# elizabethfong/SparkSmithWaterman

Hardware: AMD Instinct MI355X
Metric: GCUPS (higher is better)
Workload: dtype int32

## Files before the change

### include/swmi.h

```cpp
#ifndef SWMI_H
#define SWMI_H

#include <stddef.h>
#include <stdint.h>

#ifdef __cplusplus
extern "C" {
#endif

#define SWMI_ABI_VERSION 3

typedef enum swmi_status {
    SWMI_OK               =  0,
    SWMI_ERR_INVALID      = -1,
    SWMI_ERR_NO_DEVICE    = -2,
    SWMI_ERR_HIP          = -3,
    SWMI_ERR_NOMEM        = -4,
    SWMI_ERR_UNSUPPORTED  = -5,
    SWMI_ERR_RANGE        = -6
} swmi_status;

#define SWMI_ALIGN_LOCAL  0
#define SWMI_ALIGN_FIT    1
#define SWMI_ALIGN_GLOBAL 2

#define SWMI_TIE_SERIAL 0
#define SWMI_TIE_STRICT 1

typedef struct swmi_params {
    int32_t match;
    int32_t mismatch;
    int32_t gap;
    int32_t tie_mode;
    char    types[4];
} swmi_params;

typedef struct swmi_ctx    swmi_ctx;
typedef struct swmi_batch  swmi_batch;

int         swmi_abi_version(void);
const char *swmi_last_error(void);
int         swmi_device_count(int *count);
int         swmi_create(int device, swmi_ctx **out);
void        swmi_destroy(swmi_ctx *ctx);
void        swmi_default_params(swmi_params *p);

int         swmi_set_option(swmi_ctx *ctx, const char *name, int64_t value);

int         swmi_set_score_matrix(swmi_ctx *ctx, const uint8_t *alphabet, uint32_t n, const int32_t *scores);

int  swmi_batch_upload(swmi_ctx *ctx,
                       const uint8_t *ref_bytes, const uint64_t *ref_off, uint32_t n_refs,
                       const uint8_t *read_bytes, const uint64_t *read_off, uint32_t n_reads,
                       swmi_batch **out);
int  swmi_batch_run(swmi_ctx *ctx, swmi_batch *b, const swmi_params *p);
void swmi_batch_free(swmi_ctx *ctx, swmi_batch *b);
int  swmi_batch_run_async(swmi_ctx *ctx, swmi_batch *b, const swmi_params *p);
int  swmi_batch_wait(swmi_ctx *ctx);

typedef struct swmi_timing {
    float    fill_ms, traceback_ms, d2h_ms, total_ms;
    uint32_t fill_launches, rerun_pairs;
    uint64_t cells;
    uint64_t dir_bytes;
    uint32_t strip_fallbacks;
    uint32_t col_chunks;
    uint32_t resident_pairs;
    uint32_t tfused_pairs;
} swmi_timing;
int  swmi_batch_timing(const swmi_batch *b, swmi_timing *t);
int  swmi_batch_mode(const swmi_batch *b, int *mode);

#define SWMI_PAIR_DEGENERATE 0x1u
uint64_t swmi_batch_n_pairs(const swmi_batch *b);
int      swmi_pair_score(const swmi_batch *b, uint64_t pair, int32_t *score);
int      swmi_pair_n_alignments(const swmi_batch *b, uint64_t pair, uint64_t *n, uint32_t *flags);
int      swmi_pair_rows_swept(const swmi_batch *b, uint64_t pair, uint32_t *rows);
int      swmi_batch_pair_results(const swmi_batch *b, int32_t *scores, uint64_t *n_alignments, uint64_t n);
int      swmi_pair_alignment(swmi_batch *b, uint64_t pair, uint64_t k,
                             int32_t *begin, int32_t *end_i, int32_t *end_j,
                             const char **ref_aln, const char **read_aln, uint32_t *len);

int      swmi_batch_materialise_all(swmi_batch *b, uint64_t *n_alignments, uint64_t *n_chars);

int      swmi_ref_total(const swmi_batch *b, uint32_t ref, int32_t *total);
int      swmi_ref_totals(const swmi_batch *b, int32_t *totals, uint32_t n);
int      swmi_ref_n_match_sites(swmi_batch *b, uint32_t ref, uint64_t *n);
int      swmi_ref_match_site(swmi_batch *b, uint32_t ref, uint64_t k, int32_t *begin,
                             const char **ref_aln, const char **read_aln, uint32_t *len);

int      swmi_ref_sites_packed(swmi_batch *b, uint32_t ref_lo, uint32_t ref_hi,
                               int32_t *totals, uint64_t *degenerate, uint64_t *site_first,
                               int32_t *begins, uint32_t *lens, uint64_t *str_off, uint64_t sites_cap,
                               uint8_t *blob, uint64_t blob_cap, uint64_t *n_sites, uint64_t *blob_bytes);

int  swmi_align_batch(swmi_ctx *ctx, const swmi_params *p,
                      const uint8_t *ref_bytes, const uint64_t *ref_off, uint32_t n_refs,
                      const uint8_t *read_bytes, const uint64_t *read_off, uint32_t n_reads,
                      swmi_batch **out);

typedef struct swmi_stream swmi_stream;
typedef struct swmi_stream_stats {
    double   push_ms;
    double   parse_ms;
    double   upload_ms, run_ms;
    double   gpu_sweep_ms, gpu_traceback_ms;
    uint64_t bytes, cells;
    uint32_t chunks, pad;
} swmi_stream_stats;
int      swmi_stream_open(swmi_ctx *ctx, const swmi_params *p, const uint8_t *read_bytes, const uint64_t *read_off,
                          uint32_t n_reads, uint32_t slots, uint64_t chunk_bytes, swmi_stream **out);
int      swmi_stream_push(swmi_stream *s, const uint8_t *ref_bytes, const uint64_t *ref_off, uint32_t n_refs);
int      swmi_stream_push_file(swmi_stream *s, const char *path, const char *delimiter, uint32_t parse_threads);
int      swmi_stream_push_file_shard(swmi_stream *s, const char *path, const char *delimiter, uint32_t parse_threads,
                                     uint32_t shard, uint32_t n_shards);
int      swmi_stream_finish(swmi_stream *s);
uint64_t swmi_stream_n_refs(const swmi_stream *s);
uint32_t swmi_stream_n_chunks(const swmi_stream *s);
int      swmi_stream_chunk(swmi_stream *s, uint32_t k, swmi_batch **batch, uint64_t *first_ref);
int      swmi_stream_totals(const swmi_stream *s, int32_t *totals, uint64_t n);
int      swmi_stream_metadata(const swmi_stream *s, uint64_t ref, char *buf, size_t cap);
int      swmi_stream_ref_pos(const swmi_stream *s, uint64_t ref, uint64_t *pos);
int      swmi_stream_ref_sequence(const swmi_stream *s, uint64_t ref, uint8_t *buf, uint64_t cap, uint64_t *len);
int      swmi_stream_get_stats(const swmi_stream *s, swmi_stream_stats *st);
void     swmi_stream_close(swmi_stream *s);

#ifdef __cplusplus
}
#endif
#endif
```

### sparksmithwaterman_amd/_capi.py

```python
import ctypes as C
import os

_HERE = os.path.dirname(os.path.abspath(__file__))
LIB_PATH = os.environ.get("SWMI_LIB") or os.path.join(_HERE, "lib", "libswmi.so")

TIE_SERIAL = 0
TIE_STRICT = 1
ALIGN_LOCAL = 0
ALIGN_FIT = 1
ALIGN_GLOBAL = 2
BAND_MAX = 1 << 20
XDROP_MAX = (1 << 31) - 1
PAIR_DEGENERATE = 0x1


class SwmiError(RuntimeError):
    def __init__(self, code, msg):
        super().__init__("swmi error %d: %s" % (code, msg))
        self.code = code


class Params(C.Structure):
    _fields_ = [("match", C.c_int32), ("mismatch", C.c_int32), ("gap", C.c_int32),
                ("tie_mode", C.c_int32), ("types", C.c_char * 4)]


class Timing(C.Structure):
    _fields_ = [("fill_ms", C.c_float), ("traceback_ms", C.c_float), ("d2h_ms", C.c_float),
                ("total_ms", C.c_float), ("fill_launches", C.c_uint32), ("rerun_pairs", C.c_uint32),
                ("cells", C.c_uint64), ("dir_bytes", C.c_uint64),
                ("strip_fallbacks", C.c_uint32), ("col_chunks", C.c_uint32),
                ("resident_pairs", C.c_uint32), ("tfused_pairs", C.c_uint32)]


class StreamStats(C.Structure):
    _fields_ = [("push_ms", C.c_double), ("parse_ms", C.c_double), ("upload_ms", C.c_double), ("run_ms", C.c_double),
                ("gpu_sweep_ms", C.c_double), ("gpu_traceback_ms", C.c_double), ("bytes", C.c_uint64), ("cells", C.c_uint64),
                ("chunks", C.c_uint32), ("pad", C.c_uint32)]


_P = C.c_void_p
_u8p = C.POINTER(C.c_uint8)
_u64p = C.POINTER(C.c_uint64)
SYMBOLS = [
    ("swmi_abi_version", C.c_int, []),
    ("swmi_last_error", C.c_char_p, []),
    ("swmi_device_count", C.c_int, [C.POINTER(C.c_int)]),
    ("swmi_create", C.c_int, [C.c_int, C.POINTER(_P)]),
    ("swmi_destroy", None, [_P]),
    ("swmi_default_params", None, [C.POINTER(Params)]),
    ("swmi_set_option", C.c_int, [_P, C.c_char_p, C.c_int64]),
    ("swmi_set_score_matrix", C.c_int, [_P, C.c_char_p, C.c_uint32, C.POINTER(C.c_int32)]),
    ("swmi_batch_upload", C.c_int, [_P, C.c_char_p, _u64p, C.c_uint32, C.c_char_p, _u64p, C.c_uint32, C.POINTER(_P)]),
    ("swmi_batch_run", C.c_int, [_P, _P, C.POINTER(Params)]),
    ("swmi_batch_run_async", C.c_int, [_P, _P, C.POINTER(Params)]),
    ("swmi_batch_wait", C.c_int, [_P]),
    ("swmi_batch_free", None, [_P, _P]),
    ("swmi_batch_timing", C.c_int, [_P, C.POINTER(Timing)]),
    ("swmi_batch_mode", C.c_int, [_P, C.POINTER(C.c_int)]),
    ("swmi_batch_n_pairs", C.c_uint64, [_P]),
    ("swmi_pair_score", C.c_int, [_P, C.c_uint64, C.POINTER(C.c_int32)]),
    ("swmi_pair_n_alignments", C.c_int, [_P, C.c_uint64, _u64p, C.POINTER(C.c_uint32)]),
    ("swmi_pair_alignment", C.c_int, [_P, C.c_uint64, C.c_uint64, C.POINTER(C.c_int32), C.POINTER(C.c_int32),
                                      C.POINTER(C.c_int32), C.POINTER(C.c_char_p), C.POINTER(C.c_char_p),
                                      C.POINTER(C.c_uint32)]),
    ("swmi_pair_rows_swept", C.c_int, [_P, C.c_uint64, C.POINTER(C.c_uint32)]),
    ("swmi_batch_pair_results", C.c_int, [_P, C.POINTER(C.c_int32), _u64p, C.c_uint64]),
    ("swmi_batch_materialise_all", C.c_int, [_P, _u64p, _u64p]),
    ("swmi_ref_total", C.c_int, [_P, C.c_uint32, C.POINTER(C.c_int32)]),
    ("swmi_ref_totals", C.c_int, [_P, C.POINTER(C.c_int32), C.c_uint32]),
    ("swmi_ref_n_match_sites", C.c_int, [_P, C.c_uint32, _u64p]),
    ("swmi_ref_match_site", C.c_int, [_P, C.c_uint32, C.c_uint64, C.POINTER(C.c_int32), C.POINTER(C.c_char_p),
                                      C.POINTER(C.c_char_p), C.POINTER(C.c_uint32)]),
    ("swmi_ref_sites_packed", C.c_int, [_P, C.c_uint32, C.c_uint32, C.POINTER(C.c_int32), _u64p, _u64p, C.POINTER(C.c_int32),
                                        C.POINTER(C.c_uint32), _u64p, C.c_uint64, C.c_void_p, C.c_uint64, _u64p, _u64p]),
    ("swmi_stream_open", C.c_int, [_P, C.POINTER(Params), C.c_char_p, _u64p, C.c_uint32, C.c_uint32, C.c_uint64, C.POINTER(_P)]),
    ("swmi_stream_push", C.c_int, [_P, C.c_char_p, _u64p, C.c_uint32]),
    ("swmi_stream_push_file", C.c_int, [_P, C.c_char_p, C.c_char_p, C.c_uint32]),
    ("swmi_stream_push_file_shard", C.c_int, [_P, C.c_char_p, C.c_char_p, C.c_uint32, C.c_uint32, C.c_uint32]),
    ("swmi_stream_finish", C.c_int, [_P]),
    ("swmi_stream_n_refs", C.c_uint64, [_P]),
    ("swmi_stream_n_chunks", C.c_uint32, [_P]),
    ("swmi_stream_chunk", C.c_int, [_P, C.c_uint32, C.POINTER(_P), _u64p]),
    ("swmi_stream_totals", C.c_int, [_P, C.POINTER(C.c_int32), C.c_uint64]),
    ("swmi_stream_metadata", C.c_int, [_P, C.c_uint64, C.c_char_p, C.c_size_t]),
    ("swmi_stream_ref_pos", C.c_int, [_P, C.c_uint64, _u64p]),
    ("swmi_stream_ref_sequence", C.c_int, [_P, C.c_uint64, C.c_void_p, C.c_uint64, _u64p]),
    ("swmi_stream_get_stats", C.c_int, [_P, C.POINTER(StreamStats)]),
    ("swmi_stream_close", None, [_P]),
    ("swmi_align_batch", C.c_int, [_P, C.POINTER(Params), C.c_char_p, _u64p, C.c_uint32, C.c_char_p, _u64p,
                                   C.c_uint32, C.POINTER(_P)]),
]

_lib = None


def load():
    global _lib
    if _lib is None:
        if not os.path.exists(LIB_PATH):
            raise ImportError(
                "%s is missing: build it with `python -c 'import __graft_entry__ as g; g.build()'` "
                "(hipcc, gfx950).  There is no CPU fallback." % LIB_PATH)
        lib = C.CDLL(LIB_PATH)
        for name, res, args in SYMBOLS:
            f = getattr(lib, name)
            f.restype = res
            f.argtypes = args
        _lib = lib
    return _lib


def check(rc):
    if rc != 0:
        raise SwmiError(rc, load().swmi_last_error().decode("utf-8", "replace"))


def as_bytes(s):
    return bytes(s) if isinstance(s, (bytes, bytearray, memoryview)) else s.encode("latin-1")


def pack(seqs):
    bs = [as_bytes(s) for s in seqs]
    off = (C.c_uint64 * (len(bs) + 1))()
    t = 0
    for k, b in enumerate(bs):
        off[k] = t
        t += len(b)
    off[len(bs)] = t
    return b"".join(bs), off
```

### sparksmithwaterman_amd/csrc/swmi_ctx.cpp

```cpp
#include <cstdarg>
#include <cstdio>
#include <cstdlib>

#include "swmi_host.h"
#include "swmi_launch.h"

static thread_local std::string g_err;

int swmi_host::fail(int code, const char *fmt, ...) {
    char buf[512];
    va_list ap;
    va_start(ap, fmt);
    vsnprintf(buf, sizeof buf, fmt, ap);
    va_end(ap);
    g_err = buf;
    return code;
}

int swmi_io_fail(int code, const std::string &msg) { return fail(code, "%s", msg.c_str()); }

static const uint8_t *code_table();

extern "C" int swmi_abi_version(void) { return SWMI_ABI_VERSION; }

extern "C" const char *swmi_last_error(void) { return g_err.c_str(); }

extern "C" int swmi_device_count(int *count) {
    if (!count) return fail(SWMI_ERR_INVALID, "count is null");
    int n = 0;
    hipError_t e = hipGetDeviceCount(&n);
    if (e != hipSuccess) { *count = 0; return fail(SWMI_ERR_NO_DEVICE, "hipGetDeviceCount: %s", hipGetErrorString(e)); }
    *count = n;
    return SWMI_OK;
}

extern "C" void swmi_default_params(swmi_params *p) {
    if (!p) return;
    p->match = 5; p->mismatch = -3; p->gap = -4;
    p->tie_mode = SWMI_TIE_SERIAL;
    p->types[0] = 'a'; p->types[1] = 'i'; p->types[2] = 'd'; p->types[3] = '-';
}

static void ctx_release(swmi_ctx *c) {
    for (auto &ev : c->ev) if (ev) (void)hipEventDestroy(ev);
    if (c->stream) (void)hipStreamDestroy(c->stream);
    c->h_err.release();
    c->d_lut.release();
    c->d_hdr_ring.release();
    delete c;
}

extern "C" int swmi_create(int device, swmi_ctx **out) {
    if (!out) return fail(SWMI_ERR_INVALID, "out is null");
    *out = nullptr;
    int n = 0;
    hipError_t e = hipGetDeviceCount(&n);
    if (e != hipSuccess || n <= 0)
        return fail(SWMI_ERR_NO_DEVICE, "no HIP device available (%s); this library has no CPU fallback",
                    e != hipSuccess ? hipGetErrorString(e) : "device count 0");
    if (device < 0 || device >= n) return fail(SWMI_ERR_INVALID, "device %d out of range [0,%d)", device, n);
    hipDeviceProp_t prop;
    e = hipGetDeviceProperties(&prop, device);
    if (e != hipSuccess) return fail(SWMI_ERR_NO_DEVICE, "hipGetDeviceProperties: %s", hipGetErrorString(e));
    if (strncmp(prop.gcnArchName, "gfx950", 6) != 0)
        return fail(SWMI_ERR_NO_DEVICE, "device %d is %s; the kernels are built for gfx950 (MI355X) only",
                    device, prop.gcnArchName);
    e = hipSetDevice(device);
    if (e != hipSuccess) return fail(SWMI_ERR_NO_DEVICE, "hipSetDevice: %s", hipGetErrorString(e));
    swmi_ctx *c = new swmi_ctx;
    c->device = device;
    e = hipStreamCreateWithFlags(&c->stream, hipStreamNonBlocking);
    if (e != hipSuccess) { c->stream = nullptr; ctx_release(c); return fail(SWMI_ERR_HIP, "hipStreamCreate: %s", hipGetErrorString(e)); }
    for (auto &ev : c->ev) {
        e = hipEventCreate(&ev);
        if (e != hipSuccess) { ev = nullptr; ctx_release(c); return fail(SWMI_ERR_HIP, "hipEventCreate: %s", hipGetErrorString(e)); }
    }
    { int r = c->h_err.reserve(64); if (r) { ctx_release(c); return r; } }
    { static const char *ee = getenv("SWMI_EXT_EVENTS"); if (ee) c->ext_events = atoi(ee) != 0; }
    *(volatile uint32_t *)c->h_err.p = 0u;
    { int r = c->d_lut.reserve(256); if (r) { ctx_release(c); return r; } }
    e = hipMemcpy(c->d_lut.p, code_table(), 256, hipMemcpyHostToDevice);
    if (e != hipSuccess) { ctx_release(c); return fail(SWMI_ERR_HIP, "code table upload: %s", hipGetErrorString(e)); }
    *out = c;
    return SWMI_OK;
}

extern "C" void swmi_destroy(swmi_ctx *ctx) {
    if (!ctx) return;
    (void)hipSetDevice(ctx->device);
    if (ctx->worker.joinable()) {
        {
            std::unique_lock<std::mutex> lk(ctx->job_mu);
            ctx->job_cv.wait(lk, [&] { return ctx->job_state.load() != 1; });
            ctx->job_state.store(3);
        }
        ctx->job_cv.notify_all();
        ctx->worker.join();
    }
    ctx_release(ctx);
}

extern "C" int swmi_set_option(swmi_ctx *ctx, const char *name, int64_t value) {
    if (!ctx || !name) return fail(SWMI_ERR_INVALID, "null argument");
    std::lock_guard<std::mutex> g(ctx->mu);
    if (!strcmp(name, "cell_cap")) {
        if (value < 1 || value > (1 << 20)) return fail(SWMI_ERR_INVALID, "cell_cap out of range");
        ctx->cell_cap = (uint32_t)value;
        ctx->cell_cap_set = true;
    } else if (!strcmp(name, "max_workspace_bytes")) {
        if (value < (1 << 20)) return fail(SWMI_ERR_INVALID, "max_workspace_bytes too small");
        ctx->max_workspace_bytes = (uint64_t)value;
    } else if (!strcmp(name, "mode")) {
        if (value < -1 || value > 2) return fail(SWMI_ERR_INVALID, "mode must be -1 (automatic), 0, 1 or 2");
        ctx->mode = value < 0 ? 1u : (uint32_t)value;
    } else if (!strcmp(name, "auto_ties_x100")) {
        if (value < 100) return fail(SWMI_ERR_INVALID, "auto_ties_x100 out of range");
        ctx->auto_ties_x100 = (uint32_t)value;
    } else if (!strcmp(name, "spin_us")) {
        if (value < 0) return fail(SWMI_ERR_INVALID, "spin_us out of range");
        ctx->spin_us = value;
    } else if (!strcmp(name, "debug_strip_spins")) {
        ctx->dbg_strip_spins = (uint32_t)value;
    } else if (!strcmp(name, "debug_reverse_strips")) {
        ctx->dbg_reverse_strips = value != 0;
    } else if (!strcmp(name, "debug_async_delay_us")) {
        if (value < 0 || value > 10000000) return fail(SWMI_ERR_INVALID, "debug_async_delay_us out of range");
        ctx->dbg_async_delay_us = (uint32_t)value;
    } else if (!strcmp(name, "tfused")) {
        if (value < -1 || value > 1) return fail(SWMI_ERR_INVALID, "tfused must be -1 (automatic), 0 or 1");
        ctx->tfused = (int)value;
    } else if (!strcmp(name, "resident")) {
        if (value < -1 || value > 1) return fail(SWMI_ERR_INVALID, "resident must be -1 (automatic), 0 or 1");
        ctx->resident = (int)value;
    } else if (!strcmp(name, "scores_only")) {
        ctx->scores_only = value != 0;
    } else if (!strcmp(name, "stream_keep_records")) {
        ctx->stream_keep_records = value != 0;
    } else if (!strcmp(name, "device_strings")) {
        ctx->device_strings = value != 0;
    } else if (!strcmp(name, "tb_split")) {
        if (value < -1 || value > 1) return fail(SWMI_ERR_INVALID, "tb_split must be -1 (automatic), 0 or 1");
        ctx->tb_split = (int)value;
    } else if (!strcmp(name, "col_chunks")) {
        if (value < 0 || value > 4096) return fail(SWMI_ERR_INVALID, "col_chunks out of range");
        ctx->col_chunks = (uint32_t)value;
    } else if (!strcmp(name, "zero_copy")) {
        ctx->zero_copy = value != 0;
    } else if (!strcmp(name, "profiling")) {
        if (value < 0 || value > 2) return fail(SWMI_ERR_INVALID, "profiling must be 0, 1 (every stage) or 2 (the sweep only)");
        ctx->profiling = (int)value;
    } else if (!strcmp(name, "gap_open")) {
        if (value > 0) return fail(SWMI_ERR_INVALID, "gap_open must be <= 0 (a penalty), got %lld", (long long)value);
        if (value < INT32_MIN) return fail(SWMI_ERR_INVALID, "gap_open out of range");
        ctx->gap_open = (int32_t)value;
    } else if (!strcmp(name, "affine")) {
        if (value != -1 && value != 1) return fail(SWMI_ERR_INVALID, "affine must be -1 (when gap_open != 0) or 1 (always)");
        ctx->affine = (int)value;
    } else if (!strcmp(name, "align_mode")) {
        if (value != SWMI_ALIGN_LOCAL && value != SWMI_ALIGN_FIT && value != SWMI_ALIGN_GLOBAL)
            return fail(SWMI_ERR_INVALID, "align_mode must be 0 (local), 1 (fit) or 2 (global), got %lld", (long long)value);
        ctx->modes.align_mode = (int)value;
    } else if (!strcmp(name, "long_reads")) {
        if (value != 0 && value != 1) return fail(SWMI_ERR_INVALID, "long_reads must be 0 or 1, got %lld", (long long)value);
        ctx->modes.long_reads = (int)value;
    } else if (!strcmp(name, "band")) {
        if (value < 0 || value > (int64_t)SWMI_AFF_BAND_MAX)
            return fail(SWMI_ERR_INVALID, "band must be 0 (none) or a half-width of 1 .. %u columns, got %lld", SWMI_AFF_BAND_MAX, (long long)value);
        ctx->modes.band = (int)value;
    } else if (!strcmp(name, "extend")) {
        if (value != 0 && value != 1) return fail(SWMI_ERR_INVALID, "extend must be 0 or 1, got %lld", (long long)value);
        ctx->modes.extend = (int)value;
    } else if (!strcmp(name, "xdrop")) {
        if (value < 0 || value > 0x7FFFFFFFll)
            return fail(SWMI_ERR_INVALID, "xdrop must be 0 (off) or a threshold of 1 .. 2^31 - 1, got %lld", (long long)value);
        ctx->modes.xdrop = (int)value;
    } else if (!strcmp(name, "arena_words_per_pair")) {
        if (value < 1) return fail(SWMI_ERR_INVALID, "arena_words_per_pair out of range");
        ctx->arena_words_per_pair = (uint64_t)value;
    } else {
        return fail(SWMI_ERR_INVALID, "unknown option '%s'", name);
    }
    return SWMI_OK;
}

extern "C" int swmi_set_score_matrix(swmi_ctx *ctx, const uint8_t *alphabet, uint32_t n, const int32_t *scores) {
    if (!ctx) return fail(SWMI_ERR_INVALID, "null context");
    if (n == 0) {
        std::lock_guard<std::mutex> g(ctx->mat_mu);
        ctx->matrix.reset();
        return SWMI_OK;
    }
    if (n > SWMI_MAT_MAX_SYMBOLS) return fail(SWMI_ERR_INVALID, "a score matrix has at most %u symbols, got %u", SWMI_MAT_MAX_SYMBOLS, n);
    if (!alphabet || !scores) return fail(SWMI_ERR_INVALID, "alphabet or scores is null");
    const uint8_t *T = code_table();
    uint32_t cls[256];
    for (uint32_t c = 0; c < 256; c++) cls[c] = n;
    for (uint32_t i = 0; i < n; i++) {
        const uint8_t c = T[alphabet[i]];
        if (cls[c] != n)
            return fail(SWMI_ERR_INVALID, "score matrix symbols %u and %u are the same symbol (0x%02x, 0x%02x)", cls[c], i,
                        alphabet[cls[c]], alphabet[i]);
        cls[c] = i;
    }
    auto M = std::make_shared<ScoreMatrix>();
    M->n = n;
    M->max_entry = INT32_MIN;
    const uint32_t nn = n + 1;
    M->image.assign(swmi_aff_mat_words(nn), 0u);
    for (uint64_t x = 0; x < (uint64_t)n * n; x++) {
        if (std::llabs((int64_t)scores[x]) > (1 << 20))
            return fail(SWMI_ERR_INVALID, "score matrix entry [%u][%u] = %d: |entries| must be <= 2^20", (uint32_t)(x / n),
                        (uint32_t)(x % n), scores[x]);
        M->max_entry = std::max(M->max_entry, scores[x]);
        M->image[256 + (x / n) * nn + x % n] = (uint32_t)scores[x];
    }
    for (uint32_t c = 0; c < 256; c++) M->image[c] = cls[c] * 4u | ((cls[c] == n ? c : 0x1FFu) << 16);
    static std::atomic<uint64_t> gens{0};
    M->gen = ++gens;
    std::lock_guard<std::mutex> g(ctx->mat_mu);
    ctx->matrix = std::move(M);
    return SWMI_OK;
}

static const uint8_t *code_table() {
    static uint8_t T[256];
    static std::once_flag once;
    std::call_once(once, [] {
        uint8_t perm[256];
        for (int i = 0; i < 256; i++) perm[i] = (uint8_t)i;
        const uint8_t fast[8] = {'A', 'C', 'G', 'T', 'N', 'U', 'R', 'Y'};
        for (int k = 0; k < 8; k++) std::swap(perm[fast[k]], perm[4 * k]);
        for (int i = 0; i < 256; i++) {
            int u = i;
            if ((i >= 'a' && i <= 'z') || (i >= 0xE0 && i <= 0xFE && i != 0xF7)) u = i - 32;
            T[i] = perm[u];
        }
    });
    return T;
}

static uint64_t layout_sequences(const uint64_t *off, uint32_t n, uint64_t word0, std::vector<SeqDesc> &desc) {
    desc.resize(n);
    uint64_t at = word0;
    for (uint32_t s = 0; s < n; s++) {
        const uint64_t len = off[s + 1] - off[s];
        at = (at + 3) & ~(uint64_t)3;
        SeqDesc d{};
        d.len = (uint32_t)len;
        d.boff = (uint32_t)at;
        d.acgt = 0;
        desc[s] = d;
        at += (len + 3) / 4 + SWMI_SEQ_PAD_WORDS;
    }
    return at;
}

int swmi_host::check_offsets(const uint64_t *off, uint32_t n, const char *what) {
    if (!off) return fail(SWMI_ERR_INVALID, "%s offsets are null", what);
    if (off[0] != 0) return fail(SWMI_ERR_INVALID, "%s offsets must start at 0", what);
    for (uint32_t k = 0; k < n; k++) {
        if (off[k + 1] < off[k]) return fail(SWMI_ERR_INVALID, "%s offsets decrease at %u", what, k);
        if (off[k + 1] - off[k] >= (1ull << 30))
            return fail(SWMI_ERR_UNSUPPORTED, "%s %u is longer than 2^30-1 bases", what, k);
    }
    return SWMI_OK;
}

extern "C" void swmi_batch_free(swmi_ctx *ctx, swmi_batch *b) {
    if (!b) return;
    if (ctx) (void)hipSetDevice(ctx->device);
    b->d_raw.release(); b->d_raw_off.release();
    b->d_seqw.release(); b->d_refs.release(); b->d_reads.release(); b->d_pairs.release();
    b->d_dir.release(); b->d_seam.release(); b->d_result.release(); b->d_cells.release();
    b->d_cells_off.release(); b->d_cells_cap.release(); b->d_dbg.release(); b->d_dbg2.release();
    b->d_strip_items.release(); b->d_progress.release(); b->d_col_items.release(); b->d_win_off.release(); b->d_queue.release(); b->d_res_items.release();
    b->d_tf_items.release(); b->d_mat.release();
    b->h_result.release();
    delete b;
}

int swmi_host::upload_device(swmi_ctx *ctx, swmi_batch *b, hipStream_t st, const uint8_t *ref_src, const uint8_t *read_src) {
    const uint32_t n_refs = b->n_refs, n_reads = b->n_reads;
    const uint64_t ref_total = b->ref_off[n_refs], read_total = b->read_off[n_reads];
// ... 58 lines not shown
```

### sparksmithwaterman_amd/csrc/swmi_host.h

```cpp
#pragma once
#include <hip/hip_runtime.h>

#include <algorithm>
#include <atomic>
#include <condition_variable>
#include <cstdint>
#include <cstring>
#include <memory>
#include <mutex>
#include <string>
#include <thread>
#include <type_traits>
#include <unordered_map>
#include <vector>

#include "../../include/swmi.h"
#include "swmi_device.h"
#include "swmi_io_internal.h"

namespace swmi_host __attribute__((visibility("hidden"))) {
int fail(int code, const char *fmt, ...);
int check_offsets(const uint64_t *off, uint32_t n, const char *what);
int upload_device(swmi_ctx *ctx, swmi_batch *b, hipStream_t st, const uint8_t *ref_src, const uint8_t *read_src);
int settle_raw(swmi_batch *b);
int dump_traceback_diagnostics(swmi_batch *b, const TraceArgs &ta, size_t np, size_t n_tf);
int dump_fill_diagnostics(swmi_batch *b, const FillArgs &fa, size_t np);
void watchdog_wait(hipStream_t st, const swmi_batch *b, const char *limit_s);
}
using namespace swmi_host;

#define HIP_TRY(expr)                                                                         \
    do {                                                                                      \
        hipError_t e_ = (expr);                                                               \
        if (e_ != hipSuccess)                                                                 \
            return fail(e_ == hipErrorOutOfMemory ? SWMI_ERR_NOMEM : SWMI_ERR_HIP,            \
                        "%s failed: %s", #expr, hipGetErrorString(e_));                       \
    } while (0)

struct DevBuf {
    void *p = nullptr;
    size_t cap = 0;
    int reserve(size_t bytes) {
        if (bytes <= cap) return SWMI_OK;
        size_t want = bytes >= (256u << 20) ? bytes + bytes / 2 : bytes;
        if (p) { want = std::max(want, cap + cap / 4); (void)hipFree(p); p = nullptr; cap = 0; }
        hipError_t e = hipMalloc(&p, want);
        if (e != hipSuccess && want > bytes) { want = bytes; e = hipMalloc(&p, want); }
        if (e != hipSuccess) { p = nullptr; return fail(SWMI_ERR_NOMEM, "hipMalloc(%zu) failed: %s", bytes, hipGetErrorString(e)); }
        cap = want;
        return SWMI_OK;
    }
    void release() { if (p) (void)hipFree(p); p = nullptr; cap = 0; }
    template <class T> T *as() const { return (T *)p; }
    DevBuf() = default;
    DevBuf(const DevBuf &) = delete;
    DevBuf &operator=(const DevBuf &) = delete;
    ~DevBuf() { release(); }
};

struct PinnedBuf {
    void *p = nullptr;
    void *dp = nullptr;
    size_t cap = 0;
    int reserve(size_t bytes) {
        if (bytes <= cap) return SWMI_OK;
        if (p) { bytes = std::max(bytes, cap + cap / 4); (void)hipHostFree(p); p = nullptr; dp = nullptr; cap = 0; }
        hipError_t e = hipHostMalloc(&p, bytes, hipHostMallocMapped);
        if (e != hipSuccess) { p = nullptr; return fail(SWMI_ERR_NOMEM, "hipHostMalloc(%zu) failed: %s", bytes, hipGetErrorString(e)); }
        e = hipHostGetDevicePointer(&dp, p, 0);
        if (e != hipSuccess) { (void)hipHostFree(p); p = nullptr; return fail(SWMI_ERR_HIP, "hipHostGetDevicePointer: %s", hipGetErrorString(e)); }
        cap = bytes;
        return SWMI_OK;
    }
    void release() { if (p) (void)hipHostFree(p); p = nullptr; dp = nullptr; cap = 0; }
    PinnedBuf() = default;
    PinnedBuf(const PinnedBuf &) = delete;
    PinnedBuf &operator=(const PinnedBuf &) = delete;
    ~PinnedBuf() { release(); }
};

struct ScoreMatrix {
    uint64_t gen = 0;
    uint32_t n = 0;
    int32_t max_entry = 0;
    std::vector<uint32_t> image;
};

struct __attribute__((visibility("hidden"))) RunModes {
    int align_mode = SWMI_ALIGN_LOCAL;
    int long_reads = 0;
    int band = 0;
    int extend = 0;
    int xdrop = 0;
    uint32_t kernel_mode() const { return extend && align_mode == SWMI_ALIGN_GLOBAL ? 3u : (uint32_t)align_mode; }
    bool operator==(const RunModes &o) const { return memcmp(this, &o, sizeof(RunModes)) == 0; }
};
static_assert(std::has_unique_object_representations_v<RunModes>, "RunModes is compared bytewise: no padding, no floating point");
struct __attribute__((visibility("hidden"))) RunOptions {
    RunModes modes;
    std::shared_ptr<const ScoreMatrix> mat;
};

struct swmi_ctx {
    int device = 0;
    hipStream_t stream = nullptr;
    std::mutex mu;
    uint32_t cell_cap = 64;
    uint64_t max_workspace_bytes = 32ull << 30;
    int profiling = 0;
    uint32_t mode = 1;
    int zero_copy = 1;
    uint64_t arena_words_per_pair = 160;
    uint64_t arena_copy_wpp = 160;
    uint64_t recs_per_pair_x16 = 32;
    hipEvent_t ev[6] = {nullptr, nullptr, nullptr, nullptr, nullptr, nullptr};
    PinnedBuf h_err;
    DevBuf d_hdr_ring;
    uint32_t hdr_next = 0;
    DevBuf d_lut;
    int64_t spin_us = 2000;
    uint32_t dbg_strip_spins = 0;
    uint32_t dbg_reverse_strips = 0;
    uint32_t dbg_async_delay_us = 0;
    uint32_t auto_ties_x100 = 300;
    uint32_t col_chunks = 0;
    int tb_split = -1;
    bool ext_events = false;
    int tfused = -1;
    int resident = -1;
    int scores_only = 0;
    int stream_keep_records = 1;
    int device_strings = 1;
    bool cell_cap_set = false;
    int32_t gap_open = 0;
    int affine = -1;
    RunModes modes;
    std::mutex mat_mu;
    std::shared_ptr<const ScoreMatrix> matrix;
    std::thread worker;
    std::mutex job_mu;
    std::condition_variable job_cv;
    std::atomic<int> job_state{0};
    swmi_batch *job_batch = nullptr;
    swmi_params job_params{};
    RunOptions job_opt;
    uint32_t job_delay_us = 0;
    int job_rc = 0;
    std::string job_err;
};

static inline RunOptions run_options(swmi_ctx *ctx) {
    std::lock_guard<std::mutex> g(ctx->mat_mu);
    return RunOptions{ctx->modes, ctx->matrix};
}

struct HostAln {
    uint32_t rank;
    int32_t begin, end_i, end_j;
    uint32_t n_ops;
    const uint32_t *rec = nullptr;
    int64_t str_id = -1;
};

struct PairRes {
    int32_t score = 0;
    uint32_t flags = 0;
    uint64_t n_cells = 0;
    uint32_t strips = 0;
    uint64_t first = 0;
    uint64_t count = 0;
};

struct SiteRef { uint64_t pair; uint64_t k; int32_t begin; };

struct Work {
    uint32_t pair;
    uint64_t cells;
    uint64_t dir_words;
    uint64_t seam_words;
};

struct __attribute__((visibility("hidden"))) PlanKey {
    bool valid = false;
    size_t lo = 0, hi = 0;
    const void *work = nullptr;
    swmi_params params{};
    uint32_t eff_mode = 0;
    uint32_t col_chunks = 0;
    bool reverse_strips = false;
    int resident = -1, tfused = -1;
    bool exact = false;
    bool scores_only = false;
    uint64_t mat_gen = 0;
    RunModes modes;
    const void *d_pairs = nullptr;
    size_t pairs_bytes = 0;
    bool operator==(const PlanKey &o) const {
        return valid == o.valid && lo == o.lo && hi == o.hi && work == o.work && memcmp(&params, &o.params, sizeof(swmi_params)) == 0 &&
               eff_mode == o.eff_mode && col_chunks == o.col_chunks && reverse_strips == o.reverse_strips && resident == o.resident &&
               tfused == o.tfused && exact == o.exact && scores_only == o.scores_only && mat_gen == o.mat_gen &&
               modes == o.modes && d_pairs == o.d_pairs && pairs_bytes == o.pairs_bytes;
    }
};

struct __attribute__((visibility("hidden"))) ChunkPlan {
    uint64_t dir_words = 0, seam_words = 0;
    uint64_t seam_priv_words = 0;
    uint32_t max_path = 0, max_read = 0;
    size_t n_strip_items = 0;
    size_t n_strip_chunks = 0;
    size_t n_col_items = 0;
    uint64_t n_windows = 0;
    size_t n_res = 0;
    uint32_t res_lds_words = 0, res_ops_words = 0;
    size_t n_tf = 0;
    uint32_t tf_max_m = 0, tf_max_n = 0, tf_max_path = 0;
    uint32_t aff_r_min = 0xFFFFFFFFu, aff_r_max = 0;
    size_t aff_n_long = 0;
};

struct swmi_batch {
    uint32_t n_refs = 0, n_reads = 0;
    std::vector<uint8_t> ref_bytes, read_bytes;
    const uint8_t *src_map = nullptr;
    std::vector<swmi_io_recpos> src_recs;
    std::unordered_map<uint32_t, std::vector<uint8_t>> src_cache;
    std::vector<uint64_t> ref_off, read_off;
    std::vector<SeqDesc> ref_desc, read_desc;
    DevBuf d_raw, d_raw_off;
    DevBuf d_seqw, d_refs, d_reads, d_pairs, d_dir, d_seam, d_result, d_cells, d_cells_off, d_cells_cap, d_dbg, d_dbg2;
    DevBuf d_strip_items, d_progress;
    DevBuf d_col_items;
    DevBuf d_win_off, d_queue;
    DevBuf d_tf_items;
    DevBuf d_res_items;
    bool views_built = false;
    bool tb_split_used = false;
    bool acgt_known = false;
    PinnedBuf h_result;
    swmi_params params{};
    bool has_run = false;
    int auto_choice = -1;
    swmi_params auto_params{};
    std::vector<Work> work;
    int work_mode = -1;
    int work_band = 0;
    bool work_tfused = false;
    uint32_t eff_mode = 1;
    int32_t gap_open = 0;
    RunOptions opt;
    DevBuf d_mat;
    uint64_t d_mat_gen = 0;
    uint64_t work_cells = 0;
    std::vector<uint8_t> pairs_on_device;
    const void *pairs_dev_ptr = nullptr;
    PlanKey plan_key;
    ChunkPlan plan;
    std::vector<PairRes> pairs;
    struct RawChunk { size_t at, words; size_t tab_at, n_rec; size_t lo; std::vector<uint32_t> wpos; };
    std::vector<uint32_t> raw;
    std::vector<AlnRec> rtab;
    const uint32_t *raw_ext = nullptr;
    const AlnRec *rtab_ext = nullptr;
    uint64_t raw_ext_records = 0, raw_ext_cap = 0;
    std::vector<RawChunk> raw_chunks;
    bool indexed = false;
    bool rec_strings = false;
    bool scores_only = false;
    bool records_dropped = false;
    std::vector<HostAln> alns;
    std::vector<char> str_buf;
    std::vector<uint64_t> str_at;
    std::vector<int8_t> ref_view_ready;
    std::vector<std::vector<SiteRef>> ref_sites;
    std::vector<uint64_t> ref_degenerate;
    swmi_timing timing{};
};

struct RunState {
    swmi_ctx *ctx;
    swmi_batch *b;
    FillArgs fa{};
    TraceArgs ta{};
    float fill_ms = 0, tb_ms = 0, d2h_ms = 0;
    uint32_t launches = 0;
    double enqueue_us = 0, wait_us = 0, copyout_us = 0, prep_us = 0, prep_upload_us = 0;
    bool one_wave_sweep = false;
    bool tb_split = false;
    bool defer_copy = false;
    bool keep = true;
};

static inline size_t result_out_off() { return 64; }
static inline size_t result_tab_off(size_t np) { return (64 + np * sizeof(PairOut) + 255) & ~(size_t)255; }
static inline size_t result_arena_off(size_t np, uint64_t tab_cap) { return (result_tab_off(np) + tab_cap * sizeof(AlnRec) + 255) & ~(size_t)255; }
static inline uint64_t rec_words(uint32_t n_ops, bool strings) {
    return strings ? 2 * ((uint64_t)n_ops / 4 + 1) : ((uint64_t)n_ops + 15) / 16;
}
```

### sparksmithwaterman_amd/csrc/swmi_launch.h

```cpp
#pragma once
#include <hip/hip_runtime.h>
#include <stdint.h>
#include "swmi_device.h"

template <class K>
static inline void swmi_allow_big_lds(K kernel) {
    (void)hipFuncSetAttribute(reinterpret_cast<const void *>(kernel), hipFuncAttributeMaxDynamicSharedMemorySize, 160 * 1024);
}

extern "C" hipError_t swmi_launch_fill(const FillArgs *a, hipStream_t st, hipEvent_t ev_start, hipEvent_t ev_stop);
extern "C" hipError_t swmi_launch_traceback(const TraceArgs *a, hipStream_t st, hipEvent_t ev_start, hipEvent_t ev_stop);
extern "C" hipError_t swmi_launch_traceback_split(const TraceArgs *a, uint32_t n_windows, hipStream_t st);
extern "C" hipError_t swmi_launch_resident(const TraceArgs *a, const ResidentArgs *x, hipStream_t st);
extern "C" hipError_t swmi_launch_tfused(const TraceArgs *a, const TFusedArgs *x, hipStream_t st);
extern "C" hipError_t swmi_launch_affine_sweep(const FillArgs *a, int32_t gap_open, uint32_t align_mode, const uint32_t *mat, uint32_t nn,
                                               uint32_t r_min, uint32_t r_max, uint32_t long_reads, uint32_t band, uint32_t xdrop, hipStream_t st);
extern "C" hipError_t swmi_launch_affine_traceback(const TraceArgs *a, uint32_t align_mode, uint32_t long_reads, uint32_t band, uint32_t tile_words,
                                                   uint32_t ops_words, hipStream_t st);
extern "C" hipError_t swmi_launch_encode(const uint8_t *raw, const uint64_t *raw_off, SeqDesc *desc, uint32_t *seqw,
                                         const uint8_t *lut, uint32_t n_seq, hipStream_t st);
```

### sparksmithwaterman_amd/csrc/swmi_plan.h

```cpp
#pragma once
#include <chrono>
#include <cstdlib>

#include "swmi_host.h"

using Clock = std::chrono::steady_clock;
static inline double us_between(Clock::time_point a, Clock::time_point c) { return std::chrono::duration<double, std::micro>(c - a).count(); }

static uint64_t path_bound(uint64_t n_, uint64_t m_, const swmi_params &p, int32_t smax, int align_mode = 0) {
    uint64_t path = n_ + m_;
    if (align_mode != 0) return path;
    if (smax > 0 && p.gap < 0 && p.mismatch <= smax) {
        const uint64_t g = (uint64_t)(-(int64_t)p.gap), mt = (uint64_t)smax;
        path = std::min(path, std::min(m_ + std::min(n_, mt * m_ / g), n_ + std::min(m_, mt * n_ / g)));
    }
    return path;
}

static uint64_t traceback_lds_bytes(uint32_t mode, uint64_t max_path, uint64_t max_read) {
    const uint64_t lds_words = (max_path + 3) / 4 + 1, lds_read_words = (max_read + 3) / 4 + 1;
    const uint64_t win = (uint64_t)SWMI_RMAX * 64;
    const uint64_t tile_words = mode == 0 ? 4ull * SWMI_TB_BLOCKS * win : (mode == 1 ? 32 + 8ull * SWMI_CK_BLOCKS * win : 4ull * SWMI_CK_BLOCKS * win);
    return 4ull * (tile_words + 4ull * (lds_words + lds_read_words + SWMI_TB_REFWIN_WORDS));
}

static void longest_sequences(const swmi_batch *b, uint64_t &max_m, uint64_t &max_n) {
    max_m = max_n = 0;
    for (const auto &d : b->read_desc) max_m = std::max<uint64_t>(max_m, d.len);
    for (const auto &d : b->ref_desc) max_n = std::max<uint64_t>(max_n, d.len);
}


namespace {

struct PlanItems {
    std::vector<PairDesc> pd;
    std::vector<StripItem> strip_items;
    std::vector<ColItem> col_items;
    std::vector<uint32_t> win_off;
    std::vector<uint32_t> res_items, tf_items;
};

static const uint32_t CK_STEP_W = 16u * SWMI_CK_BLOCKS;
static inline uint32_t ck_windows(uint32_t n) {
    const uint64_t wblocks = ((uint64_t)n + 63u + 15u) / 16u;
    return (uint32_t)((wblocks + SWMI_CK_BLOCKS - 1u) / SWMI_CK_BLOCKS);
}
static inline uint64_t path_span(uint32_t m, const swmi_params &P) {
    return (uint64_t)m + (uint64_t)(P.match > 0 ? P.match : 0) * m / (uint64_t)(P.gap < 0 ? -(int64_t)P.gap : 1) + 1;
}

struct ColChunk { uint32_t g_lo, g_hi, col0; };
static ColChunk col_chunk(uint32_t g_lo, uint32_t wpc, uint32_t n_ck, uint32_t n, uint64_t span) {
    ColChunk c;
    c.g_lo = g_lo;
    c.g_hi = std::min(g_lo + wpc, n_ck);
    if (c.g_hi < n_ck && (uint64_t)c.g_hi * CK_STEP_W > n) c.g_hi = n_ck;
    const int64_t c0 = (int64_t)g_lo * CK_STEP_W - 64 - (int64_t)span - 1;
    c.col0 = g_lo == 0 || c0 <= 0 ? 0u : (uint32_t)(c0 / CK_STEP_W * CK_STEP_W);
    return c;
}

struct Planner {
    const swmi_ctx *ctx;
    const swmi_batch *b;
    const swmi_params &P;
    size_t np;
    ChunkPlan &plan;
    PlanItems &it;
    bool cols_possible = false;
    uint64_t chunk_budget = 1;
    bool res_possible = false, res_maybe = false;
    bool tf_possible = false;

    Planner(const swmi_ctx *ctx_, const swmi_batch *b_, size_t np_, bool exact, ChunkPlan &plan_, PlanItems &it_)
        : ctx(ctx_), b(b_), P(b_->params), np(np_), plan(plan_), it(it_) {
        const bool mode1 = b->eff_mode == 1, whole = mode1 && !exact && !ctx->scores_only;
        cols_possible = mode1 && P.match > 0 && P.gap < 0 && P.mismatch <= 0 && P.match <= 7 && P.mismatch >= -8 &&
                        (np <= 512 || ctx->col_chunks > 1) && ctx->col_chunks != 1;
        chunk_budget = ctx->col_chunks > 1 ? ctx->col_chunks : std::max<uint64_t>(1, 1024 / std::max<size_t>(np, 1));
        res_possible = whole && ctx->resident != 0 && (ctx->resident == 1 || np >= 256) &&
                       P.match <= 7 && P.match >= -8 && P.mismatch >= -8 && P.mismatch <= 0 && P.gap <= 0;
        tf_possible = whole && ctx->tfused == 1 &&
                      P.match > 0 && P.match <= 7 && P.mismatch >= -8 && P.mismatch <= P.match && P.gap < 0 && P.gap >= -64;
    }
    bool fast_symbols(const PairDesc &d) const { return b->read_desc[d.read_id].acgt && b->ref_desc[d.ref_id].acgt; }

    uint64_t res_need_words(uint32_t m, uint32_t n, uint32_t &opw) const {
        const uint32_t R_ = swmi_rows_per_lane(m), lact = (m + R_ - 1) / R_;
        const uint64_t nblk = ((uint64_t)n + lact - 1 + 15) / 16, n_ck = (nblk + SWMI_CK_BLOCKS - 1) / SWMI_CK_BLOCKS;
        opw = (uint32_t)((path_bound(n, m, P, P.match) + 15) / 16 + 1);
        return nblk * R_ * 64 + ((n_ck + 1) & ~1ull) + 2ull * SWMI_RES_CELL_CAP + 64ull * opw + (n + 3) / 4 + 1 + (m + 3) / 4 + 1 + 8 +
               SWMI_EMIT_SCRATCH_WORDS;
    }
    bool res_size_fits(uint32_t m, uint32_t n) const {
        uint32_t opw;
        return m <= 64u * SWMI_RMAX && (ctx->resident == 1 || (uint64_t)n <= 8ull * m) &&
               res_need_words(m, n, opw) * 4 <= (ctx->resident == 1 ? 40u : 20u) * 1024u;
    }
    bool tf_fits(const PairDesc &d, const Work &w, uint32_t m, uint32_t n) const {
        return tf_possible && m <= SWMI_TF_MAX_M && n <= 64u * SWMI_TF_BMAX && fast_symbols(d) && w.dir_words >= swmi_tf_ck_words(m);
    }
    bool cols_fit(const PairDesc &d, uint32_t m) const {
        return cols_possible && chunk_budget > 1 && m <= 64u * SWMI_RMAX && fast_symbols(d);
    }

    void take_tfused(size_t k, PairDesc &d, uint32_t m, uint32_t n) {
        d.pad = SWMI_PAD_RESIDENT;
        it.tf_items.push_back((uint32_t)k);
        plan.tf_max_m = std::max(plan.tf_max_m, m); plan.tf_max_n = std::max(plan.tf_max_n, n);
        plan.tf_max_path = std::max<uint32_t>(plan.tf_max_path, (uint32_t)path_bound(n, m, P, P.match));
    }
    void take_resident(size_t k, PairDesc &d, uint32_t m, uint32_t n) {
        d.pad = SWMI_PAD_RESIDENT;
        it.res_items.push_back((uint32_t)k);
        uint32_t opw;
        (void)res_need_words(m, n, opw);
        plan.res_ops_words = std::max(plan.res_ops_words, opw);
    }
    void take_strips(size_t k, PairDesc &d, uint32_t m, uint32_t n) {
        const uint32_t strips = (m + 64u * SWMI_RMAX - 1u) / (64u * SWMI_RMAX);
        d.pad = (uint32_t)it.strip_items.size();
        auto push_strips = [&](StripItem si) {
            si.pair = (uint32_t)k;
            si.prog = (uint32_t)it.strip_items.size();
            si.pad = 0;
            if (ctx->dbg_reverse_strips) for (uint32_t st = strips; st-- > 0;) { si.strip = st; it.strip_items.push_back(si); }
            else                         for (uint32_t st = 0; st < strips; st++) { si.strip = st; it.strip_items.push_back(si); }
        };
        uint64_t chunks = 1;
        const uint32_t n_ck = ck_windows(n);
        const uint64_t span = path_span(m, P);
        if (cols_possible) {
            const uint64_t budget = ctx->col_chunks > 1 ? ctx->col_chunks : chunk_budget / strips;
            chunks = std::min<uint64_t>(budget, n / std::max<uint64_t>((span + 64) / 4, 256));
            chunks = std::min<uint64_t>(chunks, n_ck);
            if (chunks < 2) chunks = 1;
        }
        if (chunks == 1) {
            StripItem si{};
            si.col0 = 0; si.g_lo = 0; si.g_hi = 0xFFFFFFFFu; si.priv_stride = 0; si.priv_off = 0;
            push_strips(si);
            return;
        }
        const uint32_t wpc = (uint32_t)((n_ck + chunks - 1) / chunks);
        for (uint32_t g_lo = 0; g_lo < n_ck; g_lo += wpc) {
            const ColChunk c = col_chunk(g_lo, wpc, n_ck, n, span);
            StripItem si{};
            si.g_lo = c.g_lo; si.g_hi = c.g_hi; si.col0 = c.col0;
            const uint64_t ext0 = (uint64_t)c.g_hi * CK_STEP_W - c.col0 + 64ull * (strips - 1u);
            const uint64_t n0 = c.g_hi < n_ck ? std::min<uint64_t>(n - c.col0, ext0) : n - c.col0;
            si.priv_stride = (uint32_t)((n0 + 1 + 15) & ~15ull);
            si.priv_off = plan.seam_priv_words;
            plan.seam_priv_words += (uint64_t)(strips - 1u) * si.priv_stride;
            if (c.g_hi == n_ck) si.g_hi = 0xFFFFFFFFu;
            push_strips(si);
            plan.n_strip_chunks++;
            if (c.g_hi == n_ck) break;
        }
    }
    void take_cols(size_t k, PairDesc &d, uint32_t m, uint32_t n) {
        const uint64_t span = path_span(m, P);
        const uint32_t n_ck = ck_windows(n);
        uint64_t chunks = std::min<uint64_t>(chunk_budget, n / std::max<uint64_t>(span + 64, 256));
        chunks = std::min<uint64_t>(chunks, n_ck);
        static const bool dbg_one = getenv("SWMI_DEBUG_ONE_CHUNK") != nullptr;
        if (dbg_one) chunks = 1;
        if (chunks < 2 && !dbg_one) return;
        const uint32_t wpc = (uint32_t)((n_ck + chunks - 1) / chunks);
        const size_t first = it.col_items.size();
        for (uint32_t g_lo = 0; g_lo < n_ck; g_lo += wpc) {
            const ColChunk c = col_chunk(g_lo, wpc, n_ck, n, span);
            ColItem ci;
            ci.pair = (uint32_t)k; ci.g_lo = c.g_lo; ci.g_hi = c.g_hi; ci.col0 = c.col0;
            it.col_items.push_back(ci);
            if (c.g_hi == n_ck) break;
        }
        d.pad = SWMI_PAD_COLS | (uint32_t)(it.col_items.size() - first);
    }

    void finish(const std::vector<Work> &work, size_t lo) {
        for (uint32_t k : it.res_items) {
            uint32_t opw;
            const uint64_t own = res_need_words(b->read_desc[it.pd[k].read_id].len, b->ref_desc[it.pd[k].ref_id].len, opw);
            plan.res_lds_words = std::max<uint32_t>(plan.res_lds_words, (uint32_t)(own + 64ull * (plan.res_ops_words - opw)));
        }
        if (16ull * plan.res_lds_words > SWMI_LDS_BYTES) {
            for (uint32_t k : it.res_items) it.pd[k].pad = 0;
            it.res_items.clear();
            plan.res_lds_words = 0; plan.res_ops_words = 0;
        }
        plan.n_strip_items = it.strip_items.size();
        plan.n_col_items = it.col_items.size();
        plan.n_res = it.res_items.size();
        plan.n_tf = it.tf_items.size();
        std::vector<uint8_t> is_res(np, 0);
        for (uint32_t k : it.res_items) is_res[k] = 1;
        for (size_t k = 0; k < np; k++) {
            it.pd[k].dir_off = plan.dir_words;
            it.pd[k].seam_off = plan.seam_words;
            if (!is_res[k]) { plan.dir_words += work[lo + k].dir_words; plan.seam_words += work[lo + k].seam_words; }
        }
        if (b->eff_mode == 1) it.win_off[np] = (uint32_t)std::min<uint64_t>(plan.n_windows, 0xFFFFFFFFu);
        for (StripItem &si : it.strip_items)
            if (si.priv_stride) si.priv_off += plan.seam_words;
    }
};

}

static int plan_chunk(swmi_ctx *ctx, swmi_batch *b, const std::vector<Work> &work, size_t lo, size_t np, bool exact, ChunkPlan &plan,
                      PlanItems &it) {
    const uint32_t n_reads = b->n_reads;
    plan = ChunkPlan{};
    Planner pl(ctx, b, np, exact, plan, it);
    if (pl.res_possible)
        for (size_t k = 0; k < np && !pl.res_maybe; k++)
            pl.res_maybe = pl.res_size_fits(b->read_desc[work[lo + k].pair % n_reads].len, b->ref_desc[work[lo + k].pair / n_reads].len);
    if ((pl.cols_possible || pl.res_maybe || pl.tf_possible) && !b->acgt_known) {
        if (b->n_refs) HIP_TRY(hipMemcpy(b->ref_desc.data(), b->d_refs.p, b->n_refs * sizeof(SeqDesc), hipMemcpyDeviceToHost));
        if (b->n_reads) HIP_TRY(hipMemcpy(b->read_desc.data(), b->d_reads.p, b->n_reads * sizeof(SeqDesc), hipMemcpyDeviceToHost));
        b->acgt_known = true;
    }
    it.pd.resize(np);
    if (b->eff_mode == 1) it.win_off.resize(np + 1);
    uint32_t pb_m = 0xFFFFFFFFu, pb_n = 0xFFFFFFFFu, pb_val = 0;
    const int32_t smax = b->opt.mat ? std::max(b->params.match, b->opt.mat->max_entry) : b->params.match;
    for (size_t k = 0; k < np; k++) {
        const Work &w = work[lo + k];
        PairDesc d{};
        d.ref_id = w.pair / n_reads;
        d.read_id = w.pair % n_reads;
        d.out_id = (uint32_t)k;
        const uint32_t m_ = b->read_desc[d.read_id].len, n_ = b->ref_desc[d.ref_id].len;
        if (b->eff_mode == 1) {
            const uint64_t rps = 64ull * swmi_rows_per_lane(m_);
            it.win_off[k] = (uint32_t)std::min<uint64_t>(plan.n_windows, 0xFFFFFFFFu);
            plan.n_windows += ((m_ + rps - 1) / rps) * ck_windows(n_);
        }
        const bool res_fit = pl.res_maybe && pl.fast_symbols(d) && pl.res_size_fits(m_, n_);
        if (!res_fit && pl.tf_fits(d, w, m_, n_)) pl.take_tfused(k, d, m_, n_);
        else if (res_fit) pl.take_resident(k, d, m_, n_);
        else if (b->eff_mode == 1 && m_ > 64u * SWMI_RMAX && it.strip_items.size() < (1u << 30)) pl.take_strips(k, d, m_, n_);
        else if (pl.cols_fit(d, m_)) pl.take_cols(k, d, m_, n_);
        it.pd[k] = d;
        if (m_ != pb_m || n_ != pb_n) { pb_m = m_; pb_n = n_; pb_val = (uint32_t)path_bound(n_, m_, b->params, smax, b->opt.modes.align_mode); }
        plan.max_path = std::max<uint32_t>(plan.max_path, pb_val);
        plan.max_read = std::max(plan.max_read, m_);
        if (m_ > SWMI_AFF_MAX_READ) { plan.aff_n_long++; continue; }
        plan.aff_r_min = std::min(plan.aff_r_min, swmi_aff_rows_per_lane(m_));
        plan.aff_r_max = std::max(plan.aff_r_max, swmi_aff_rows_per_lane(m_));
    }
    pl.finish(work, lo);
    if (b->eff_mode == 3 && plan.aff_n_long) {
        std::stable_partition(it.pd.begin(), it.pd.end(), [&](const PairDesc &d) { return b->read_desc[d.read_id].len <= SWMI_AFF_MAX_READ; });
    }
    return SWMI_OK;
}

template <class T>
static int upload_items(hipStream_t st, DevBuf &dst, const std::vector<T> &v) {
    int rc;
    if ((rc = dst.reserve(v.size() * sizeof(T)))) return rc;
    HIP_TRY(hipMemcpyAsync(dst.p, v.data(), v.size() * sizeof(T), hipMemcpyHostToDevice, st));
    HIP_TRY(hipStreamSynchronize(st));
    return SWMI_OK;
}

static int upload_plan(swmi_ctx *ctx, swmi_batch *b, size_t np, const ChunkPlan &plan, const PlanItems &it) {
    int rc;
    if (b->eff_mode == 1 && (rc = upload_items(ctx->stream, b->d_win_off, it.win_off))) return rc;
    if ((rc = b->d_pairs.reserve(np * sizeof(PairDesc)))) return rc;
    if (!it.strip_items.empty()) {
        if ((rc = b->d_progress.reserve(it.strip_items.size() * sizeof(uint32_t)))) return rc;
        if ((rc = upload_items(ctx->stream, b->d_strip_items, it.strip_items))) return rc;
    }
    if (!it.res_items.empty() && (rc = upload_items(ctx->stream, b->d_res_items, it.res_items))) return rc;
    if (!it.tf_items.empty() && (rc = upload_items(ctx->stream, b->d_tf_items, it.tf_items))) return rc;
    if (!it.col_items.empty() && (rc = upload_items(ctx->stream, b->d_col_items, it.col_items))) return rc;
    if ((rc = b->d_dir.reserve(std::max<uint64_t>(plan.dir_words, 1) * 4))) return rc;
    if ((rc = b->d_seam.reserve(std::max<uint64_t>(plan.seam_words + plan.seam_priv_words, 1) * 4))) return rc;
    const size_t bytes = np * sizeof(PairDesc);
    if (b->pairs_dev_ptr != b->d_pairs.p || b->pairs_on_device.size() != bytes || memcmp(b->pairs_on_device.data(), it.pd.data(), bytes) != 0) {
        HIP_TRY(hipMemcpyAsync(b->d_pairs.p, it.pd.data(), bytes, hipMemcpyHostToDevice, ctx->stream));
        HIP_TRY(hipStreamSynchronize(ctx->stream));
        b->pairs_on_device.assign((const uint8_t *)it.pd.data(), (const uint8_t *)it.pd.data() + bytes);
        b->pairs_dev_ptr = b->d_pairs.p;
    }
    return SWMI_OK;
}

static int prepare_chunk(RunState &rs, const std::vector<Work> &work, size_t lo, size_t hi, const std::vector<uint64_t> *cells_exact) {
    swmi_ctx *ctx = rs.ctx;
    swmi_batch *b = rs.b;
    const size_t np = hi - lo;
    const auto p0 = Clock::now();
    PlanKey key;
    key.valid = true;
    key.lo = lo; key.hi = hi; key.work = (const void *)work.data();
    key.params = b->params; key.eff_mode = b->eff_mode;
    key.col_chunks = ctx->col_chunks; key.reverse_strips = ctx->dbg_reverse_strips != 0;
    key.resident = ctx->resident; key.tfused = ctx->tfused;
    key.exact = cells_exact != nullptr; key.scores_only = ctx->scores_only != 0;
    key.mat_gen = b->opt.mat ? b->opt.mat->gen : 0u; key.modes = b->opt.modes;
    key.d_pairs = b->d_pairs.p; key.pairs_bytes = np * sizeof(PairDesc);
    auto p1 = p0;
    if (key == b->plan_key) {
        p1 = Clock::now();
    } else {
        b->plan_key = PlanKey{};
        PlanItems items;
        int rc;
        if ((rc = plan_chunk(ctx, b, work, lo, np, key.exact, b->plan, items))) return rc;
        p1 = Clock::now();
        if ((rc = upload_plan(ctx, b, np, b->plan, items))) return rc;
        key.d_pairs = b->pairs_dev_ptr;
        b->plan_key = key;
    }
    rs.prep_us += us_between(p0, p1);
    rs.prep_upload_us += us_between(p1, Clock::now());
    return SWMI_OK;
}
```

### sparksmithwaterman_amd/csrc/swmi_run.cpp

```cpp
#include <chrono>
#include <cstdio>
#include <cstdlib>
#include <functional>
#include <numeric>

#include "swmi_host.h"
#include "swmi_launch.h"
#include "swmi_plan.h"

static int keep_chunk_records(RunState &rs, const AlnRec *tab, uint64_t n_rec, const uint32_t *arena, uint64_t arena_cap, size_t lo) {
    swmi_batch *b = rs.b;
    if (rs.defer_copy && b->raw_chunks.empty()) {
        b->raw_ext = arena; b->rtab_ext = tab; b->raw_ext_records = n_rec; b->raw_ext_cap = arena_cap;
        b->raw_chunks.push_back(swmi_batch::RawChunk{0, 0, 0, (size_t)n_rec, lo, {}});
        return SWMI_OK;
    }
    uint64_t used = 0;
    for (uint64_t k = 0; k < n_rec; k++) {
        const uint64_t end = (((uint64_t)tab[k].off_hi << 32) | tab[k].off_lo) + rec_words(tab[k].n_ops, b->rec_strings);
        used = std::max(used, end);
    }
    if (used > arena_cap) return fail(SWMI_ERR_HIP, "record payloads overrun the arena");
    b->raw_chunks.push_back(swmi_batch::RawChunk{b->raw.size(), (size_t)used, b->rtab.size(), (size_t)n_rec, lo, {}});
    b->raw.insert(b->raw.end(), arena, arena + used);
// ... 91 lines not shown
    fa.err_host = (uint32_t *)ctx->h_err.dp;
    fa.pad3 = 0;
    if (L.attempt == 0) b->timing.col_chunks += (uint32_t)plan.n_col_items + (pipe ? (uint32_t)plan.n_strip_chunks : 0u);
    fa.col_items = plan.n_col_items ? b->d_col_items.as<ColItem>() : nullptr;
    fa.n_col_items = (uint32_t)plan.n_col_items;
    fa.strip_spins = ctx->dbg_strip_spins;
    L.q_cap = std::min<uint64_t>(std::max<uint64_t>(L.cells_total, 1), 1ull << 24);
    if (L.split && (rc = b->d_queue.reserve(256 + L.q_cap * sizeof(uint4)))) return rc;
    fa.q_reset = L.split ? b->d_queue.as<uint32_t>() : nullptr;
    return SWMI_OK;
}

static int build_trace_args(RunState &rs, Launch &L) {
    swmi_ctx *ctx = rs.ctx;
    swmi_batch *b = rs.b;
    const ChunkPlan &plan = b->plan;
    const FillArgs &fa = rs.fa;
    int rc;
    TraceArgs &ta = rs.ta;
    ta.seqw = fa.seqw; ta.refs = fa.refs; ta.reads = fa.reads; ta.pairs = fa.pairs;
    ta.dir = fa.dir; ta.out = fa.out; ta.cells = fa.cells;
    ta.cells_off = fa.cells_off; ta.cells_cap = fa.cells_cap;
    ta.hdr = (ArenaHdr *)L.res;
    ta.arena = (uint32_t *)(L.res + L.a_off);
    ta.arena_cap_words = L.arena_cap;
    ta.rec_tab = (AlnRec *)(L.res + L.t_off);
    ta.rec_tab_cap = (uint32_t)std::min<uint64_t>(L.tab_cap, 0xFFFFFFFFu);
    ta.n_pairs = fa.n_pairs; ta.cell_cap = fa.cell_cap;
    ta.match = fa.match; ta.mismatch = fa.mismatch; ta.gap = fa.gap; ta.strict = fa.strict;
    ta.lds_words = (plan.max_path + 3) / 4 + 1;
    ta.seam = fa.seam;
    ta.mode = b->eff_mode;
    ta.pad2 = 0;
    ta.lds_read_words = (plan.max_read + 3) / 4 + 1;
    ta.out_host = nullptr;
    ta.ovf_host = (uint32_t *)ctx->h_err.dp + 4;
    ((volatile uint32_t *)ctx->h_err.p)[4] = 0u; ((volatile uint32_t *)ctx->h_err.p)[5] = 0u;
    ta.win_off = nullptr; ta.q_count = nullptr; ta.q_items = nullptr; ta.q_cap = 0; ta.pad4 = 0;
    const bool strings = ctx->device_strings != 0 && b->d_raw.p != nullptr;
    ta.raw = strings ? b->d_raw.as<uint8_t>() : nullptr;
    ta.raw_off = strings ? b->d_raw_off.as<uint64_t>() : nullptr;
    ta.raw_reads_at = b->n_refs + 1u;
    b->rec_strings = strings;
    if (L.zc) {
        if ((rc = b->h_result.reserve(L.a_off + L.arena_cap * 4))) return rc;
        uint8_t *hd = (uint8_t *)b->h_result.dp;
        *(volatile uint32_t *)b->h_result.p = 0u;
        ((volatile uint32_t *)b->h_result.p)[1] = 0u;
        ta.ovf_host = (uint32_t *)hd;
        ta.out_host = (PairOut *)(hd + result_out_off());
        ta.arena = (uint32_t *)(hd + L.a_off);
        ta.rec_tab = (AlnRec *)(hd + L.t_off);
    }
    ta.dbg = nullptr;
    if (dbg_fill_on()) {
        if ((rc = b->d_dbg2.reserve(L.np * 32))) return rc;
        HIP_TRY(hipMemsetAsync(b->d_dbg2.p, 0, L.np * 32, ctx->stream));
        ta.dbg = b->d_dbg2.as<unsigned long long>();
    }
    L.whole_only = L.zc && plan.n_tf + plan.n_res == L.np;
    if (L.whole_only) {
        const uint32_t slots = 1024;
        if (!ctx->d_hdr_ring.p || ctx->hdr_next >= slots) {
            if ((rc = ctx->d_hdr_ring.reserve((size_t)slots * 64))) return rc;
            HIP_TRY(hipMemsetAsync(ctx->d_hdr_ring.p, 0, (size_t)slots * 64, ctx->stream));
            ctx->hdr_next = 0;
        }
        ta.hdr = (ArenaHdr *)(ctx->d_hdr_ring.as<uint8_t>() + (size_t)ctx->hdr_next++ * 64);
    }
    return SWMI_OK;
}

static ResidentArgs resident_args(const swmi_batch *b) {
    const ChunkPlan &plan = b->plan;
    ResidentArgs xa;
    xa.res_items = plan.n_res ? b->d_res_items.as<uint32_t>() : nullptr;
    xa.n_res = (uint32_t)plan.n_res; xa.res_lds_words = plan.res_lds_words; xa.res_cell_cap = SWMI_RES_CELL_CAP; xa.res_ops_words = plan.res_ops_words;
    return xa;
}

static TFusedArgs tfused_args(const swmi_batch *b) {
    const ChunkPlan &plan = b->plan;
    TFusedArgs xt{};
    xt.items = plan.n_tf ? b->d_tf_items.as<uint32_t>() : nullptr;
    xt.n_items = (uint32_t)plan.n_tf;
    xt.cell_cap = 16;
    xt.tile_words = ((plan.tf_max_m + 63u + 15u) / 16u) * 64u * SWMI_TF_BR;
    xt.ref_words = (plan.tf_max_n + 3u) / 4u + 1u;
    xt.read_words = (plan.tf_max_m + 3u) / 4u + 1u;
    xt.stage_words = (plan.tf_max_path + 3u) / 4u + 1u + SWMI_EMIT_SCRATCH_WORDS;
    static const bool tf_marks = getenv("SWMI_DEBUG_MARKS") != nullptr;
    xt.debug_marks = tf_marks ? 1u : 0u;
    xt.lds_words = (xt.tile_words + 2u * xt.cell_cap + xt.stage_words + xt.ref_words + xt.read_words + 3u) & ~3u;
    static const int tf_helpers = getenv("SWMI_TF_HELPERS") ? atoi(getenv("SWMI_TF_HELPERS")) : 2;
    const uint64_t region = 4ull * xt.lds_words, budget = SWMI_LDS_BYTES - 4ull * 1024;
    const uint64_t left = budget > 4 * region ? budget - 4 * region : 0;
    xt.n_helpers = (uint32_t)std::min<uint64_t>((uint64_t)std::max(0, std::min(tf_helpers, (int)SWMI_TF_HELPERS)), region ? left / region : 0);
    return xt;
}

static int enqueue_launches(RunState &rs, Launch &L, const ResidentArgs &xa, const TFusedArgs &xt) {
    swmi_ctx *ctx = rs.ctx;
    swmi_batch *b = rs.b;
    const ChunkPlan &plan = b->plan;
    FillArgs &fa = rs.fa;
    TraceArgs &ta = rs.ta;
    const size_t np = L.np, n_res = plan.n_res, n_tf = plan.n_tf;
    const bool first = L.attempt == 0;
    int rc;
    L.ext_timing = ctx->profiling == 1 && first && !L.whole_only && !n_res && !n_tf && !L.split && b->eff_mode == 1 &&
                   !fa.n_strip_items && !fa.n_col_items && ctx->ext_events;
    const bool ext = L.ext_timing;
    if (ctx->profiling && !ext) HIP_TRY(hipEventRecord(ctx->ev[0], ctx->stream));
    if (first && !L.whole_only) {
        if (fa.n_strip_items) HIP_TRY(hipMemsetAsync(fa.progress, 0, (size_t)fa.n_strip_items * sizeof(uint32_t), ctx->stream));
        if (b->eff_mode == 3) {
            FillArgs fs = fa, fl = fa;
            fs.n_pairs = (uint32_t)(np - plan.aff_n_long);
            fl.n_pairs = (uint32_t)plan.aff_n_long; fl.pairs = fa.pairs + fs.n_pairs;
            const uint32_t *mat = b->opt.mat ? b->d_mat.as<uint32_t>() : nullptr;
            const uint32_t nn = b->opt.mat ? b->opt.mat->n + 1u : 0u;
            HIP_TRY(swmi_launch_affine_sweep(&fs, b->gap_open, b->opt.modes.kernel_mode(), mat, nn, plan.aff_r_min, plan.aff_r_max, 0u, 0u, 0u, ctx->stream));
            HIP_TRY(swmi_launch_affine_sweep(&fl, b->gap_open, b->opt.modes.kernel_mode(), mat, nn, 0u, 0u, 1u, (uint32_t)b->opt.modes.band,
                                             (uint32_t)b->opt.modes.xdrop, ctx->stream));
        }
        else HIP_TRY(swmi_launch_fill(&fa, ctx->stream, ext ? ctx->ev[0] : nullptr, ext ? ctx->ev[1] : nullptr));
        rs.launches++;
    }
    if (n_tf) HIP_TRY(swmi_launch_tfused(&ta, &xt, ctx->stream));
    if (L.whole_only && n_tf) rs.launches++;
    if (ctx->profiling && !ext) HIP_TRY(hipEventRecord(ctx->ev[1], ctx->stream));
    if (n_res) HIP_TRY(swmi_launch_resident(&ta, &xa, ctx->stream));
    if (first) b->timing.resident_pairs += (uint32_t)n_res;
    if (first) b->timing.tfused_pairs += (uint32_t)n_tf;
    if (L.sweep_only) {
        if ((rc = b->h_result.reserve(L.a_off + L.arena_cap * 4))) return rc;
        HIP_TRY(hipMemcpyAsync((uint8_t *)b->h_result.p + result_out_off(), L.res + result_out_off(), np * sizeof(PairOut),
                               hipMemcpyDeviceToHost, ctx->stream));
    } else if (L.split) {
        ta.win_off = b->d_win_off.as<uint32_t>();
        ta.q_count = b->d_queue.as<uint32_t>();
        ta.q_items = (uint4 *)(b->d_queue.as<uint8_t>() + 256);
        ta.q_cap = (uint32_t)L.q_cap;
        if (!first || L.whole_only) HIP_TRY(hipMemsetAsync(ta.q_count, 0, 4, ctx->stream));
        HIP_TRY(swmi_launch_traceback_split(&ta, (uint32_t)plan.n_windows, ctx->stream));
    } else if (b->eff_mode == 3) {
        TraceArgs ts = ta, tl = ta;
        ts.n_pairs = (uint32_t)(np - plan.aff_n_long);
        tl.n_pairs = (uint32_t)plan.aff_n_long; tl.pairs = ta.pairs + ts.n_pairs;
        const uint32_t ops_words = (uint32_t)(((uint64_t)plan.max_path + 15) / 16 + 1);
        HIP_TRY(swmi_launch_affine_traceback(&ts, b->opt.modes.kernel_mode(), 0u, 0u, SWMI_AFF_TILE_WORDS, ops_words, ctx->stream));
        HIP_TRY(swmi_launch_affine_traceback(&tl, b->opt.modes.kernel_mode(), 1u, (uint32_t)b->opt.modes.band, SWMI_AFF_TILE_WORDS, ops_words, ctx->stream));
    } else if (n_res + n_tf < np) {
        HIP_TRY(swmi_launch_traceback(&ta, ctx->stream, ext ? ctx->ev[2] : nullptr, ext ? ctx->ev[3] : nullptr));
    }
    if (L.time_all && !ext) HIP_TRY(hipEventRecord(ctx->ev[3], ctx->stream));

    L.copy_words = std::min<uint64_t>(L.arena_cap, std::max<uint64_t>(256, np * ctx->arena_copy_wpp));
    L.copy_recs = std::min<uint64_t>(L.tab_cap, np * ctx->recs_per_pair_x16 / 16 + 64);
    if (!L.zc && !L.sweep_only) {
        if ((rc = b->h_result.reserve(L.a_off + L.arena_cap * 4))) return rc;
        HIP_TRY(hipMemcpyAsync(b->h_result.p, L.res, L.t_off + L.copy_recs * sizeof(AlnRec), hipMemcpyDeviceToHost, ctx->stream));
        HIP_TRY(hipMemcpyAsync((uint8_t *)b->h_result.p + L.a_off, L.res + L.a_off, L.copy_words * 4, hipMemcpyDeviceToHost, ctx->stream));
        if (L.time_all) HIP_TRY(hipEventRecord(ctx->ev[4], ctx->stream));
    }
    return SWMI_OK;
}

static int wait_for_stream(swmi_ctx *ctx) {
    const auto t0 = Clock::now();
    hipError_t q = hipErrorNotReady;
    while (ctx->spin_us > 0 && (q = hipStreamQuery(ctx->stream)) == hipErrorNotReady && us_between(t0, Clock::now()) < (double)ctx->spin_us)
        __builtin_ia32_pause();
    if (q != hipSuccess && q != hipErrorNotReady) return fail(SWMI_ERR_HIP, "hipStreamQuery: %s", hipGetErrorString(q));
    if (q != hipSuccess) HIP_TRY(hipStreamSynchronize(ctx->stream));
    return SWMI_OK;
}

static void collect_scores(const swmi_batch *b, const std::vector<Work> &work, const Launch &L, std::vector<PairOut> &outs) {
    const uint8_t *h = (const uint8_t *)b->h_result.p;
    outs.assign((const PairOut *)(h + result_out_off()), (const PairOut *)(h + result_out_off()) + L.np);
    for (size_t k = 0; k < L.np; k++) {
        PairOut &o = outs[k];
        if (o.score <= 0 && !(o.flags & SWMI_F_DEGENERATE) && b->opt.modes.align_mode == 0) {
            const uint32_t pair = work[L.lo + k].pair;
            o.score = 0; o.flags = SWMI_F_DEGENERATE;
            o.n_cells = (uint64_t)b->read_desc[pair % b->n_reads].len * b->ref_desc[pair / b->n_reads].len;
        }
        o.flags &= SWMI_F_DEGENERATE | SWMI_F_STRIPS_MASK;
    }
}

static int collect_launch(RunState &rs, Launch &L, Clock::time_point t_done, std::vector<uint8_t> &saved_outs, std::vector<PairOut> &outs,
                          bool &retry) {
    swmi_ctx *ctx = rs.ctx;
    swmi_batch *b = rs.b;
    const size_t np = L.np;
    const bool zc = L.zc;
    int rc;
    retry = false;
    const uint8_t *h = (const uint8_t *)b->h_result.p;
    ArenaHdr hdr_copy{};
    const ArenaHdr *hdr = (const ArenaHdr *)h;
    bool overflow = false;
    if (zc) {
        overflow = *(const volatile uint32_t *)h != 0u;
        if (overflow) {
            HIP_TRY(hipMemcpy(&hdr_copy, rs.ta.hdr, sizeof hdr_copy, hipMemcpyDeviceToHost));
            hdr = &hdr_copy;
        }
    }
    const uint64_t hdr_words = zc && !overflow ? 0 : hdr->reserved & SWMI_HDR_WORD_MASK;
    const uint64_t hdr_recs = zc && !overflow ? 0 : hdr->reserved >> SWMI_HDR_WORD_BITS;
    if (!zc) overflow = hdr_words > L.arena_cap || hdr_recs > L.tab_cap;
    if (overflow) {
        if (zc) {
            saved_outs.resize(np * sizeof(PairOut));
            HIP_TRY(hipMemcpy(saved_outs.data(), L.res + result_out_off(), saved_outs.size(), hipMemcpyDeviceToHost));
        } else {
            saved_outs.assign(h + result_out_off(), h + result_out_off() + np * sizeof(PairOut));
        }
        for (size_t k = 0; k < np; k++) {
            PairOut &so = ((PairOut *)saved_outs.data())[k];
            so.flags &= ~SWMI_F_ARENA_OVF;
            if (L.split && !(so.flags & SWMI_F_DEGENERATE)) { so.n_cells = 0; so.flags &= ~SWMI_F_CELL_OVF; }
        }
        L.arena_cap = std::max<uint64_t>(L.arena_cap, hdr_words + 1024);
        L.tab_cap = std::max<uint64_t>(L.tab_cap, hdr_recs + 64);
        if (L.arena_cap >= SWMI_HDR_WORD_MASK || L.tab_cap >= (1ull << (64u - SWMI_HDR_WORD_BITS)) - 1ull)
            return fail(SWMI_ERR_UNSUPPORTED, "one launch would hold %llu alignment records in %llu arena dwords: lower max_workspace_bytes so that the batch runs in smaller launches",
                        (unsigned long long)L.tab_cap, (unsigned long long)L.arena_cap);
        ctx->arena_words_per_pair = std::max<uint64_t>(ctx->arena_words_per_pair, L.arena_cap / np + 1);
        ctx->recs_per_pair_x16 = std::max<uint64_t>(ctx->recs_per_pair_x16, L.tab_cap * 16 / np + 1);
        retry = true;
        return SWMI_OK;
    }
    outs.assign((const PairOut *)(h + result_out_off()), (const PairOut *)(h + result_out_off()) + np);
    for (auto &o : outs) o.flags &= ~SWMI_F_ARENA_OVF;
    uint64_t n_rec = 0;
    if (zc) {
        for (auto &o : outs)
            if (!(o.flags & (SWMI_F_DEGENERATE | SWMI_F_CELL_OVF))) n_rec += o.n_cells;
    } else {
        n_rec = hdr_recs;
    }
    if (n_rec > L.tab_cap) return fail(SWMI_ERR_HIP, "more records than the table holds");
    const AlnRec *tab = (const AlnRec *)(h + L.t_off);
    const uint32_t *aw = (const uint32_t *)(h + L.a_off);
    if (!zc) {
        if (n_rec > L.copy_recs)
            HIP_TRY(hipMemcpy((uint8_t *)b->h_result.p + L.t_off + L.copy_recs * sizeof(AlnRec), L.res + L.t_off + L.copy_recs * sizeof(AlnRec),
                              (n_rec - L.copy_recs) * sizeof(AlnRec), hipMemcpyDeviceToHost));
        if (hdr_words > L.copy_words)
            HIP_TRY(hipMemcpy((uint8_t *)b->h_result.p + L.a_off + L.copy_words * 4, L.res + L.a_off + L.copy_words * 4,
                              (hdr_words - L.copy_words) * 4, hipMemcpyDeviceToHost));
        ctx->arena_copy_wpp = hdr_words * 5 / (4 * np) + 2;
        ctx->recs_per_pair_x16 = std::max<uint64_t>(ctx->recs_per_pair_x16, n_rec * 20 / np + 1);
    }
    if (rs.keep) {
        if ((rc = keep_chunk_records(rs, tab, n_rec, aw, L.arena_cap, L.lo))) return rc;
        rs.copyout_us += us_between(t_done, Clock::now());
    }
    return SWMI_OK;
}

static int run_chunk(RunState &rs, const std::vector<Work> &work, size_t lo, size_t hi,
                     const std::vector<uint64_t> *cells_exact, std::vector<PairOut> &outs) {
    swmi_ctx *ctx = rs.ctx;
    swmi_batch *b = rs.b;
    const size_t np = hi - lo;
    int rc;
    if ((rc = prepare_chunk(rs, work, lo, hi, cells_exact))) return rc;
    const ChunkPlan &plan = b->plan;
    if (plan.seam_words) HIP_TRY(hipMemsetAsync(b->d_seam.p, 0, plan.seam_words * 4, ctx->stream));

    Launch L;
    L.np = np; L.lo = lo; L.cells_exact = cells_exact;
    if ((rc = size_cell_lists(rs, L))) return rc;
    {
        const uint64_t need = b->eff_mode == 3 ? 4ull * (SWMI_AFF_TILE_WORDS + ((uint64_t)plan.max_path + 15) / 16 + 1 + SWMI_EMIT_SCRATCH_WORDS)
                                               : traceback_lds_bytes(b->eff_mode, plan.max_path, plan.max_read);
        if (need > SWMI_LDS_BYTES)
            return fail(SWMI_ERR_UNSUPPORTED, "a pair of %u bases in total needs %llu bytes of LDS for the traceback (limit %u)",
                        plan.max_path, (unsigned long long)need, SWMI_LDS_BYTES);
    }
    L.split = rs.tb_split && !cells_exact && b->eff_mode == 1 && plan.n_windows < 0xFFFFFFFFull;
    L.zc = ctx->zero_copy != 0;
    L.sweep_only = ctx->scores_only != 0 && !cells_exact;
    L.time_all = ctx->profiling == 1;

    const auto c0 = Clock::now();
    L.arena_cap = std::max<uint64_t>(np * ctx->arena_words_per_pair, 1024);
    L.tab_cap = std::max<uint64_t>(np * ctx->recs_per_pair_x16 / 16 + 64, 256);
    std::vector<uint8_t> saved_outs;
    for (L.attempt = 0;; L.attempt++) {
        if (L.attempt > 4) return fail(SWMI_ERR_HIP, "the record arena overflowed %d times in a row; results discarded", L.attempt);
        L.t_off = result_tab_off(np); L.a_off = result_arena_off(np, L.tab_cap);
        if ((rc = b->d_result.reserve(L.a_off + L.arena_cap * 4))) return rc;
        L.res = b->d_result.as<uint8_t>();
        if (L.attempt > 0) {
            HIP_TRY(hipMemsetAsync(L.res, 0, 64, ctx->stream));
            HIP_TRY(hipMemcpyAsync(L.res + result_out_off(), saved_outs.data(), saved_outs.size(), hipMemcpyHostToDevice, ctx->stream));
        }
        if ((rc = build_fill_args(rs, L))) return rc;
        if ((rc = build_trace_args(rs, L))) return rc;
        if ((rc = enqueue_launches(rs, L, resident_args(b), tfused_args(b)))) return rc;
        static const char *watchdog = getenv("SWMI_DEBUG_WATCHDOG");
// ... 440 lines not shown
```

### sparksmithwaterman_amd/csrc/swmi_stream.cpp

```cpp
#include <chrono>
#include <cstdio>
#include <cstdlib>
#include <deque>

#include "swmi_host.h"

struct StreamChunk {
    uint32_t id = 0;
    PinnedBuf *buf = nullptr;
    std::vector<uint64_t> off;
    std::vector<swmi_io_recpos> recs;
    std::vector<uint8_t> keep;
};

struct swmi_stream {
    swmi_ctx *owner = nullptr;
    swmi_params params{};
    std::vector<uint8_t> read_bytes;
    std::vector<uint64_t> read_off;
    uint32_t n_reads = 0;
    uint64_t chunk_bytes = 32ull << 20;
    bool keep_records = true;
    struct Slot { swmi_ctx *ctx = nullptr; swmi_batch *shell = nullptr; std::thread th; };
    std::vector<Slot> slots;
    std::vector<std::unique_ptr<PinnedBuf>> bufs;
    std::deque<PinnedBuf *> free_bufs;
    std::deque<StreamChunk *> ready;
    std::mutex mu;
    std::condition_variable cv_free, cv_ready;
    bool closing = false;
    std::atomic<int> err{0};
    std::string err_msg;
    uint32_t next_id = 0;
    uint32_t in_flight = 0;
    std::vector<swmi_batch *> results;
    std::vector<uint64_t> first_ref;
    bool finished = false;
    const uint8_t *map_p = nullptr; size_t map_n = 0; int map_fd = -1;
    swmi_stream_stats stats{};
};

static void stream_fail(swmi_stream *s, int rc, const std::string &msg) {
    std::lock_guard<std::mutex> g(s->mu);
    if (!s->err.load()) { s->err_msg = msg; s->err.store(rc); }
    s->cv_free.notify_all(); s->cv_ready.notify_all();
}

static int stream_process(swmi_stream *s, swmi_stream::Slot &sl, StreamChunk *c) {
    swmi_batch *b = sl.shell;
    const uint32_t n_refs = (uint32_t)(c->off.size() - 1);
    int rc;
    {
        std::lock_guard<std::mutex> g(sl.ctx->mu);
        HIP_TRY(hipSetDevice(sl.ctx->device));
        b->n_refs = n_refs; b->n_reads = s->n_reads;
        b->ref_off = c->off;
        b->read_off = s->read_off;
        if ((uint64_t)n_refs * s->n_reads >= (1ull << 32)) return fail(SWMI_ERR_UNSUPPORTED, "more than 2^32-1 pairs in one chunk");
        const auto t0 = std::chrono::steady_clock::now();
        if ((rc = upload_device(sl.ctx, b, sl.ctx->stream, (const uint8_t *)c->buf->p, s->read_bytes.data()))) return rc;
        const double up = std::chrono::duration<double, std::milli>(std::chrono::steady_clock::now() - t0).count();
        std::lock_guard<std::mutex> g2(s->mu);
        s->stats.upload_ms += up;
    }
    const auto t1 = std::chrono::steady_clock::now();
    if ((rc = swmi_batch_run(sl.ctx, b, &s->params))) return rc;
    const double run = std::chrono::duration<double, std::milli>(std::chrono::steady_clock::now() - t1).count();
    const auto t2 = std::chrono::steady_clock::now();
    std::unique_ptr<swmi_batch> r(new swmi_batch);
    r->n_refs = n_refs; r->n_reads = s->n_reads;
    r->ref_off = std::move(b->ref_off);
    r->read_off = s->read_off;
    r->read_bytes = s->read_bytes;
    r->ref_desc = b->ref_desc; r->read_desc = b->read_desc;
    r->params = b->params; r->has_run = true; r->eff_mode = b->eff_mode;
    r->work = std::move(b->work); b->work.clear(); b->work_mode = -1;
    r->work_mode = (int)r->eff_mode;
    r->pairs = std::move(b->pairs);
    if (s->keep_records) {
        (void)settle_raw(b);
        r->raw = std::move(b->raw);
        r->rtab = std::move(b->rtab);
        r->raw_chunks = std::move(b->raw_chunks);
    } else {
        r->records_dropped = true;
        b->raw_ext = nullptr; b->rtab_ext = nullptr;
    }
    r->rec_strings = b->rec_strings;
    r->scores_only = b->scores_only;
    r->indexed = false;
    r->ref_view_ready.assign(n_refs, 0);
    r->ref_sites.assign(n_refs, {});
    r->ref_degenerate.assign(n_refs, 0);
    r->timing = b->timing;
    if (!c->recs.empty()) { r->src_map = s->map_p; r->src_recs = std::move(c->recs); }
    else r->ref_bytes = std::move(c->keep);
    b->pairs.clear(); b->raw.clear(); b->rtab.clear(); b->raw_chunks.clear(); b->has_run = false;
    std::lock_guard<std::mutex> g(s->mu);
    {
        static const bool host_dbg = getenv("SWMI_DEBUG_HOST") != nullptr;
        if (host_dbg) fprintf(stderr, "[swmi stream] chunk %u: %u refs, run %.1f ms, results moved out of the slot in %.1f ms\n", c->id, n_refs, run,
                              std::chrono::duration<double, std::milli>(std::chrono::steady_clock::now() - t2).count());
    }
    if (s->results.size() <= c->id) s->results.resize(c->id + 1, nullptr);
    s->results[c->id] = r.release();
    s->stats.run_ms += run;
    s->stats.gpu_sweep_ms += b->timing.fill_ms;
    s->stats.gpu_traceback_ms += b->timing.traceback_ms;
    s->stats.cells += b->timing.cells;
    s->stats.chunks++;
    return SWMI_OK;
}

static void stream_worker(swmi_stream *s, size_t slot) {
    swmi_stream::Slot &sl = s->slots[slot];
    for (;;) {
        StreamChunk *c = nullptr;
        {
            std::unique_lock<std::mutex> lk(s->mu);
            s->cv_ready.wait(lk, [&] { return !s->ready.empty() || s->closing; });
            if (s->ready.empty()) return;
            c = s->ready.front();
            s->ready.pop_front();
        }
        int rc = s->err.load() ? s->err.load() : stream_process(s, sl, c);
        if (rc && !s->err.load()) stream_fail(s, rc, swmi_last_error());
        {
            std::lock_guard<std::mutex> g(s->mu);
            s->free_bufs.push_back(c->buf);
            s->in_flight--;
        }
        s->cv_free.notify_all();
        delete c;
    }
}

extern "C" int swmi_stream_open(swmi_ctx *ctx, const swmi_params *p, const uint8_t *read_bytes, const uint64_t *read_off,
                                uint32_t n_reads, uint32_t slots, uint64_t chunk_bytes, swmi_stream **out) {
    if (!ctx || !p || !out) return fail(SWMI_ERR_INVALID, "null argument");
    *out = nullptr;
    int rc;
    if ((rc = check_offsets(read_off, n_reads, "read"))) return rc;
    if (n_reads && read_off[n_reads] && !read_bytes) return fail(SWMI_ERR_INVALID, "sequence bytes are null");
    if (slots == 0) slots = 3;
    if (slots > 8) return fail(SWMI_ERR_INVALID, "at most 8 slots");
    std::unique_ptr<swmi_stream> s(new swmi_stream);
    s->owner = ctx;
    s->params = *p;
    s->n_reads = n_reads;
    s->read_off.assign(read_off, read_off + n_reads + 1);
    s->read_bytes.assign(read_bytes, read_bytes + read_off[n_reads]);
    if (chunk_bytes) s->chunk_bytes = std::max<uint64_t>(chunk_bytes, 1 << 16);
    s->keep_records = ctx->stream_keep_records != 0;
    s->slots.resize(slots);
    for (auto &sl : s->slots) {
        if ((rc = swmi_create(ctx->device, &sl.ctx))) { swmi_stream_close(s.release()); return rc; }
        sl.ctx->cell_cap = ctx->cell_cap; sl.ctx->cell_cap_set = ctx->cell_cap_set; sl.ctx->max_workspace_bytes = ctx->max_workspace_bytes;
        sl.ctx->profiling = ctx->profiling; sl.ctx->mode = ctx->mode; sl.ctx->zero_copy = ctx->zero_copy;
        sl.ctx->tb_split = ctx->tb_split; sl.ctx->col_chunks = ctx->col_chunks; sl.ctx->resident = ctx->resident; sl.ctx->tfused = ctx->tfused;
        sl.ctx->auto_ties_x100 = ctx->auto_ties_x100; sl.ctx->arena_words_per_pair = ctx->arena_words_per_pair;
        sl.ctx->device_strings = ctx->device_strings; sl.ctx->scores_only = ctx->scores_only;
        sl.ctx->gap_open = ctx->gap_open; sl.ctx->affine = ctx->affine;
        sl.ctx->modes = ctx->modes; sl.ctx->matrix = run_options(ctx).mat;
        sl.ctx->spin_us = 50;
        sl.shell = new swmi_batch;
    }
    const size_t n_bufs = slots + 8;
    for (size_t k = 0; k < n_bufs; k++) {
        std::unique_ptr<PinnedBuf> pb(new PinnedBuf);
        if ((rc = pb->reserve(s->chunk_bytes + (1 << 20)))) { swmi_stream_close(s.release()); return rc; }
        s->free_bufs.push_back(pb.get());
        s->bufs.push_back(std::move(pb));
    }
    for (size_t k = 0; k < s->slots.size(); k++) s->slots[k].th = std::thread(stream_worker, s.get(), k);
    *out = s.release();
    return SWMI_OK;
}

static PinnedBuf *stream_take_buf(swmi_stream *s, uint64_t bytes) {
    PinnedBuf *pb = nullptr;
    {
        std::unique_lock<std::mutex> lk(s->mu);
        s->cv_free.wait(lk, [&] { return !s->free_bufs.empty() || s->err; });
        if (s->err) return nullptr;
        pb = s->free_bufs.front();
        s->free_bufs.pop_front();
    }
    if (pb->reserve(bytes)) {
        stream_fail(s, SWMI_ERR_NOMEM, swmi_last_error());
        std::lock_guard<std::mutex> g(s->mu);
        s->free_bufs.push_back(pb);
        return nullptr;
    }
    return pb;
}

static void stream_submit(swmi_stream *s, StreamChunk *c) {
    {
        std::lock_guard<std::mutex> g(s->mu);
        auto it = s->ready.begin();
        while (it != s->ready.end() && (*it)->id < c->id) ++it;
        s->ready.insert(it, c);
        s->in_flight++;
    }
    s->cv_ready.notify_one();
}

extern "C" int swmi_stream_push(swmi_stream *s, const uint8_t *ref_bytes, const uint64_t *ref_off, uint32_t n_refs) {
    if (!s) return fail(SWMI_ERR_INVALID, "stream is null");
    if (s->finished) return fail(SWMI_ERR_INVALID, "the stream is finished");
    int rc;
    if ((rc = check_offsets(ref_off, n_refs, "reference"))) return rc;
    if (n_refs && ref_off[n_refs] && !ref_bytes) return fail(SWMI_ERR_INVALID, "sequence bytes are null");
    uint32_t lo = 0;
    while (lo < n_refs) {
        uint32_t hi = lo;
        while (hi < n_refs && (hi == lo || ref_off[hi + 1] - ref_off[lo] <= s->chunk_bytes)) hi++;
        const uint64_t bytes = ref_off[hi] - ref_off[lo];
        PinnedBuf *pb = stream_take_buf(s, std::max<uint64_t>(bytes, 16));
        if (!pb) return fail(s->err.load() ? s->err.load() : SWMI_ERR_NOMEM, "%s", s->err_msg.c_str());
        StreamChunk *c = new StreamChunk;
        c->buf = pb;
        c->off.resize(hi - lo + 1);
        for (uint32_t k = lo; k <= hi; k++) c->off[k - lo] = ref_off[k] - ref_off[lo];
        memcpy(pb->p, ref_bytes + ref_off[lo], bytes);
        c->keep.assign(ref_bytes + ref_off[lo], ref_bytes + ref_off[hi]);
        { std::lock_guard<std::mutex> g(s->mu); c->id = s->next_id++; }
        stream_submit(s, c);
        lo = hi;
    }
    return s->err ? fail(s->err, "%s", s->err_msg.c_str()) : SWMI_OK;
}

extern "C" int swmi_stream_push_file(swmi_stream *s, const char *path, const char *delimiter, uint32_t parse_threads) {
    return swmi_stream_push_file_shard(s, path, delimiter, parse_threads, 0, 1);
}

extern "C" int swmi_stream_push_file_shard(swmi_stream *s, const char *path, const char *delimiter, uint32_t parse_threads,
                                           uint32_t shard, uint32_t n_shards) {
    if (!s || !path || !delimiter) return fail(SWMI_ERR_INVALID, "null argument");
    if (s->finished) return fail(SWMI_ERR_INVALID, "the stream is finished");
    if (s->map_p) return fail(SWMI_ERR_UNSUPPORTED, "one file per stream");
    const auto t0 = std::chrono::steady_clock::now();
    int rc = swmi_io_map(path, &s->map_p, &s->map_n, &s->map_fd);
    if (rc) return rc;
    const uint8_t *p = s->map_p;
    const size_t n = s->map_n;
    size_t lo = 0, hi = 0;
    if ((rc = swmi_io_shard_range(p, n, delimiter, shard, n_shards, path, &lo, &hi))) return rc;
    std::vector<size_t> cut{lo};
    while (cut.back() < hi) {
        const size_t want = cut.back() + s->chunk_bytes;
        size_t nxt = want >= hi ? hi : swmi_io_next_record(p, n, want, delimiter);
        if (nxt <= cut.back() || nxt > hi) nxt = hi;
        cut.push_back(nxt);
    }
    const uint32_t n_seg = (uint32_t)(cut.size() - 1);
    uint32_t id0;
    { std::lock_guard<std::mutex> g(s->mu); id0 = s->next_id; s->next_id += n_seg; }
    if (parse_threads == 0) parse_threads = 6;
    parse_threads = std::min<uint32_t>(parse_threads, std::max<uint32_t>(1, n_seg));
    std::atomic<uint32_t> next{0};
    std::string delim(delimiter);
    auto parser = [&]() {
        for (;;) {
            const uint32_t k = next.fetch_add(1);
            if (k >= n_seg || s->err) return;
            const auto p0 = std::chrono::steady_clock::now();
            PinnedBuf *pb = stream_take_buf(s, std::max<uint64_t>(cut[k + 1] - cut[k], 16));
            if (!pb) return;
            StreamChunk *c = new StreamChunk;
            c->id = id0 + k;
            c->buf = pb;
            int prc = swmi_io_parse_segment(p, cut[k], cut[k + 1], delim.c_str(), (uint8_t *)pb->p, c->off, c->recs);
            if (prc) {
                stream_fail(s, prc, swmi_last_error());
                std::lock_guard<std::mutex> g(s->mu);
                s->free_bufs.push_back(pb);
                delete c;
                return;
            }
            const double ms = std::chrono::duration<double, std::milli>(std::chrono::steady_clock::now() - p0).count();
            { std::lock_guard<std::mutex> g(s->mu); s->stats.parse_ms += ms; s->stats.bytes += c->off.back(); }
            stream_submit(s, c);
        }
    };
    std::vector<std::thread> th;
    for (uint32_t k = 0; k < parse_threads; k++) th.emplace_back(parser);
    for (auto &t : th) t.join();
    s->stats.push_ms += std::chrono::duration<double, std::milli>(std::chrono::steady_clock::now() - t0).count();
    return s->err ? fail(s->err, "%s", s->err_msg.c_str()) : SWMI_OK;
}

extern "C" int swmi_stream_finish(swmi_stream *s) {
    if (!s) return fail(SWMI_ERR_INVALID, "stream is null");
    {
        std::unique_lock<std::mutex> lk(s->mu);
        s->cv_free.wait(lk, [&] { return s->in_flight == 0 || s->err; });
    }
    if (s->err) return fail(s->err, "%s", s->err_msg.c_str());
    if (!s->finished) {
        s->first_ref.assign(s->results.size() + 1, 0);
        for (size_t k = 0; k < s->results.size(); k++) {
            if (!s->results[k]) return fail(SWMI_ERR_HIP, "chunk %zu has no results", k);
            s->first_ref[k + 1] = s->first_ref[k] + s->results[k]->n_refs;
        }
        s->finished = true;
    }
    return SWMI_OK;
}

extern "C" uint64_t swmi_stream_n_refs(const swmi_stream *s) { return s && s->finished ? s->first_ref.back() : 0; }
// ... 106 lines not shown
```

### sparksmithwaterman_amd/csrc/swmi_traceback.hip

```cpp
#include <hip/hip_runtime.h>
#include <hip/hip_ext.h>
#include <stdint.h>
#include <stdlib.h>
#include "swmi_device.h"
#include "swmi_emit.h"
#include "swmi_launch.h"
#include "swmi_walk.h"

template <int R>
__device__ __forceinline__ void coop_helper(const TraceArgs &A, const PairDesc pd, const uint32_t lane, const uint32_t wave,
                                            const uint32_t nw, const uint32_t ts, const uint32_t n_waves_all,
                                            uint32_t *__restrict__ tiles, volatile uint32_t *__restrict__ shared) {
    const SeqDesc rd = A.refs[pd.ref_id];
    const SeqDesc qd = A.reads[pd.read_id];
    const uint32_t n = rd.len, m = qd.len;
    const uint32_t *__restrict__ refw = A.seqw + rd.boff;
    const uint32_t *__restrict__ readw = A.seqw + qd.boff;
    const StripGeom G = strip_geom<R>(m, n, 1u);
    const bool acgt = rd.acgt && qd.acgt && SWMI_SCORES_FIT(A);
    const uint32_t team = (wave - nw) % nw, q = 1u + (wave - nw) / nw;
    uint32_t last = 0;
    for (;;) {
        uint32_t seq;
        while ((seq = __hip_atomic_load(const_cast<uint32_t *>(&shared[7u + 4u * team]), __ATOMIC_RELAXED, __HIP_MEMORY_SCOPE_WORKGROUP)) == last)
            __builtin_amdgcn_s_sleep(SWMI_HELPER_SLEEP);
        if (seq == 0xFFFFFFFFu) break;
        last = seq;
        __builtin_amdgcn_fence(__ATOMIC_ACQUIRE, "workgroup");
        const uint32_t flags = shared[4u + 4u * team], wlo = shared[5u + 4u * team], nq = shared[6u + 4u * team];
        const uint32_t s = flags >> 2;
        const uint32_t win = (flags & 2u) ? q - 1u : q;
        if (q < ts && win < nq) {
            uint32_t *__restrict__ base = ((flags & 1u) ? tiles + n_waves_all * (SWMI_CK_BLOCKS * SWMI_RMAX * WAVE) : tiles) +
                                          team * ts * (SWMI_CK_BLOCKS * SWMI_RMAX * WAVE);
            (void)replay_any<R, false, false>(A, pd, n, m, acgt, refw, readw, G, s, wlo + win * SWMI_CK_BLOCKS, lane,
                                       base + win * SWMI_CK_BLOCKS * R * WAVE, 0, 0u, nullptr, 0u);
            __builtin_amdgcn_fence(__ATOMIC_RELEASE, "workgroup");
            if (lane == 0) atomicAdd(const_cast<uint32_t *>(&shared[20u + team]), 1u);
        }
    }
}

template <int TMODE>
__device__ __forceinline__ void traceback_entry(const TraceArgs &A, uint32_t *lds_all) {
    const uint32_t wave = threadIdx.x >> 6;
    const uint32_t pair = blockIdx.x * FILL_WAVES + wave;
    if (pair >= A.n_pairs) return;
    const uint32_t lane = threadIdx.x & 63u;
    const uint32_t slot = blockIdx.y;
    uint32_t *tb_lds = lds_all + wave * (A.lds_words + A.lds_read_words + SWMI_TB_REFWIN_WORDS +
                                         (TMODE == 0 ? SWMI_TB_BLOCKS : SWMI_CK_BLOCKS) * SWMI_RMAX * WAVE);
    uint32_t *tile = tb_lds + A.lds_words + A.lds_read_words + SWMI_TB_REFWIN_WORDS;
    const PairDesc pd = A.pairs[pair];
    const PairOut po = A.out[pd.out_id];
    if (A.out_host && slot == 0 && lane == 0) A.out_host[pd.out_id] = po;
    if (po.flags & (SWMI_F_DEGENERATE | SWMI_F_CELL_OVF)) return;
    if (po.n_cells <= slot) return;
    const uint32_t R = swmi_rows_per_lane(A.reads[pd.read_id].len);
    if (R == 1)      traceback_pair<1, TMODE, false>(A, pd, po, lane, slot, SWMI_TB_SLOTS, tb_lds, tile, nullptr, 1u);
    else if (R == 2) traceback_pair<2, TMODE, false>(A, pd, po, lane, slot, SWMI_TB_SLOTS, tb_lds, tile, nullptr, 1u);
    else if (R == 3) traceback_pair<3, TMODE, false>(A, pd, po, lane, slot, SWMI_TB_SLOTS, tb_lds, tile, nullptr, 1u);
    else             traceback_pair<4, TMODE, false>(A, pd, po, lane, slot, SWMI_TB_SLOTS, tb_lds, tile, nullptr, 1u);
}

template <int R>
__device__ __forceinline__ uint32_t winmax_detect(const TraceArgs &A, const PairDesc pd, PairOut &po, const uint32_t lane,
                                                  const uint32_t wave, const uint32_t n_waves, const uint32_t ccap,
                                                  uint32_t *__restrict__ tiles, uint32_t *__restrict__ walker_lds,
                                                  const uint32_t per_walker, volatile uint32_t *__restrict__ shared) {
    const SeqDesc rd = A.refs[pd.ref_id];
    const SeqDesc qd = A.reads[pd.read_id];
    const uint32_t n = rd.len, m = qd.len;
    const uint32_t *__restrict__ refw = A.seqw + rd.boff;
    const uint32_t *__restrict__ readw = A.seqw + qd.boff;
    const bool acgt = rd.acgt && qd.acgt && SWMI_SCORES_FIT(A);
    const StripGeom G = strip_geom<R>(m, n, 1u);
    constexpr uint32_t WIN_WORDS = SWMI_CK_BLOCKS * SWMI_RMAX * WAVE;
    uint32_t ncand = 0, gc[SWMI_TB_SLOTS] = {0u, 0u, 0u, 0u};
    if (G.n_strips == 1u) {
        const uint32_t *__restrict__ wm = A.dir + pd.dir_off + G.wmax_off;
        for (uint32_t g0 = 0; g0 < G.n_ck; g0 += WAVE) {
            const uint32_t g = g0 + lane;
            const int wv = g < G.n_ck ? (int)wm[g] : -1;
            uint64_t cand = BALLOT(wv == po.score);
            while (cand) {
                const uint32_t gg = g0 + (uint32_t)__builtin_ctzll(cand);
                cand &= cand - 1ull;
                if (ncand == 0u) gc[0] = gg; else if (ncand == 1u) gc[1] = gg; else if (ncand == 2u) gc[2] = gg; else if (ncand == 3u) gc[3] = gg;
                ++ncand;
            }
        }
    }
    auto stage_ref = [&](uint32_t *__restrict__ dst, uint32_t wlo, uint32_t nwin) {
        const int clo = (int)(16u * wlo) - 63;
        const uint32_t cw0 = clo > 0 ? (uint32_t)clo >> 2 : 0u;
        const uint32_t cw1 = (16u * (wlo + nwin * SWMI_CK_BLOCKS) - 1u) >> 2;
        for (uint32_t x = cw0 + lane; x <= cw1 && x < (n + 3u) / 4u; x += WAVE) dst[x - cw0] = refw[x];
    };
    auto publish = [&](uint32_t cnt, uint32_t staged) {
        if (lane == 0) {
            po.n_cells = cnt;
            if (cnt > ccap) po.flags |= SWMI_F_CELL_OVF;
            A.out[pd.out_id] = po;
            if (A.out_host) A.out_host[pd.out_id] = po;
            shared[0] = cnt;
            shared[3] = staged;
        }
        if (lane < SWMI_TB_SLOTS) { shared[7u + 4u * lane] = 0u; shared[20u + lane] = 0u; }
        asm volatile("s_waitcnt vmcnt(0)" ::: "memory");
    };
    const uint64_t cbase = A.cells_off ? A.cells_off[pd.out_id] : (uint64_t)pd.out_id * A.cell_cap;
    uint2 *__restrict__ cells = const_cast<uint2 *>(A.cells) + cbase;

    const uint32_t seg = ccap / SWMI_TB_SLOTS;
    if (ncand >= 2u && ncand <= SWMI_TB_SLOTS && ncand <= n_waves && seg >= 1u) {
        const uint32_t nw = ncand, ts = n_waves / nw;
        if (wave < nw) {
            const uint32_t g = wave == 0u ? gc[0] : wave == 1u ? gc[1] : wave == 2u ? gc[2] : gc[3];
            const uint32_t nq0 = g + 1u < ts ? g + 1u : ts;
            const uint32_t wlo0 = (g + 1u - nq0) * SWMI_CK_BLOCKS;
            uint32_t *my = walker_lds + wave * per_walker;
            for (uint32_t w = lane; w < (m + 3u) / 4u; w += WAVE) my[A.lds_words + w] = readw[w];
            stage_ref(my + A.lds_words + A.lds_read_words, wlo0, nq0);
            const uint32_t c = replay_any<R, true, false>(A, pd, n, m, acgt, refw, readw, G, 0u, g * SWMI_CK_BLOCKS, lane,
                                                   tiles + wave * ts * WIN_WORDS + (nq0 - 1u) * SWMI_CK_BLOCKS * R * WAVE,
                                                   po.score, 0u, cells + wave * seg, seg);
            if (lane == 0) { shared[24u + wave] = c; shared[28u + wave] = wlo0; }
            asm volatile("s_waitcnt vmcnt(0)" ::: "memory");
        } else {
            const uint32_t team = (wave - nw) % nw, q = 1u + (wave - nw) / nw;
            const uint32_t g = team == 0u ? gc[0] : team == 1u ? gc[1] : team == 2u ? gc[2] : gc[3];
            const uint32_t nq0 = g + 1u < ts ? g + 1u : ts;
            if (q < nq0)
                (void)replay_any<R, false, false>(A, pd, n, m, acgt, refw, readw, G, 0u, (g - q) * SWMI_CK_BLOCKS, lane,
                                           tiles + team * ts * WIN_WORDS + (nq0 - 1u - q) * SWMI_CK_BLOCKS * R * WAVE,
                                           0, 0u, nullptr, 0u);
        }
        __syncthreads();
        bool one_each = true;
        for (uint32_t w = 0; w < nw; ++w) one_each = one_each && shared[24u + w] == 1u;
        if (one_each) {
            if (wave == 0) {
                uint2 c = make_uint2(0, 0);
                if (lane < nw) { c.x = ld_l2(&cells[lane * seg].x); c.y = ld_l2(&cells[lane * seg].y); }
                if (lane < nw) cells[lane] = c;
                publish(nw, 1u);
            }
            __syncthreads();
            return wave < nw ? shared[28u + wave] : 0xFFFFFFFFu;
        }
        __syncthreads();
    }

    const bool pre = ncand == 1u;
    const uint32_t nq0 = gc[0] + 1u < n_waves ? gc[0] + 1u : n_waves;
    const uint32_t wlo0 = (gc[0] + 1u - nq0) * SWMI_CK_BLOCKS;
    if (wave == 0) {
        if (n_waves == 1u) {
            for (uint32_t w = lane; w < (m + 3u) / 4u; w += WAVE) walker_lds[A.lds_words + w] = readw[w];
            if (pre) stage_ref(walker_lds + A.lds_words + A.lds_read_words, wlo0, nq0);
        }
        const uint32_t cnt = detect_cells<R, false>(A, pd, po, lane, pre ? tiles + (nq0 - 1u) * SWMI_CK_BLOCKS * R * WAVE : tiles);
        publish(cnt, (pre && cnt == 1u) ? 1u : 0u);
    } else {
        if (wave < SWMI_TB_SLOTS)
            for (uint32_t w = lane; w < (m + 3u) / 4u; w += WAVE) walker_lds[wave * per_walker + A.lds_words + w] = readw[w];
        if (wave == n_waves - 1u)
            for (uint32_t w = lane; w < (m + 3u) / 4u; w += WAVE) walker_lds[A.lds_words + w] = readw[w];
        if (pre) {
            if (wave < nq0)
                (void)replay_any<R, false, false>(A, pd, n, m, acgt, refw, readw, G, 0u, wlo0 + (wave - 1u) * SWMI_CK_BLOCKS, lane,
                                           tiles + (wave - 1u) * SWMI_CK_BLOCKS * R * WAVE, 0, 0u, nullptr, 0u);
            if (wave == n_waves - 1u) stage_ref(walker_lds + A.lds_words + A.lds_read_words, wlo0, nq0);
        }
    }
    __syncthreads();
    return (pre && wave == 0) ? wlo0 : 0xFFFFFFFFu;
}

extern "C" __global__ void __launch_bounds__(WAVE * SWMI_TB_WAVES) __attribute__((amdgpu_waves_per_eu(4, 4)))
sw_traceback_winmax_kernel(const TraceArgs A) {
    extern __shared__ uint32_t wm_lds[];
    const uint32_t pair = blockIdx.x;
    if (pair >= A.n_pairs) return;
    const uint32_t wave = threadIdx.x >> 6, lane = threadIdx.x & 63u;
    const PairDesc pd = A.pairs[pair];
    PairOut po = A.out[pd.out_id];
    if (finish_pair(A, pd, po) && wave == 0 && lane == 0) A.out[pd.out_id] = po;
    if (po.flags & (SWMI_F_DEGENERATE | SWMI_F_DONE)) {
        if (A.out_host && wave == 0 && lane == 0) A.out_host[pd.out_id] = po;
        return;
    }
    const uint32_t n_waves = blockDim.x >> 6;
    const uint32_t per_walker = A.lds_words + A.lds_read_words + SWMI_TB_REFWIN_WORDS;
    constexpr uint32_t WIN_WORDS = SWMI_CK_BLOCKS * SWMI_RMAX * WAVE;
    uint32_t *shared = wm_lds;
    uint32_t *tiles = wm_lds + 32;
    const uint32_t R = swmi_rows_per_lane(A.reads[pd.read_id].len);
    const uint32_t ccap = A.cells_cap ? A.cells_cap[pd.out_id] : A.cell_cap;
    const uint32_t tile_sets = A.pad2 ? 2u : 1u;
    uint32_t *tiles2 = A.pad2 ? tiles + n_waves * WIN_WORDS : nullptr;
    uint32_t *walker_lds0 = tiles + tile_sets * n_waves * WIN_WORDS;
    if (!swmi_common_pair(A, A.refs[pd.ref_id], A.reads[pd.read_id])) {
        if (wave == 0) {
            uint32_t c;
            if (R == 1)      c = detect_cells<1>(A, pd, po, lane, tiles);
            else if (R == 2) c = detect_cells<2>(A, pd, po, lane, tiles);
            else if (R == 3) c = detect_cells<3>(A, pd, po, lane, tiles);
            else             c = detect_cells<4>(A, pd, po, lane, tiles);
            if (lane == 0) {
                po.n_cells = c;
                if (c > ccap) po.flags |= SWMI_F_CELL_OVF;
                A.out[pd.out_id] = po;
                if (A.out_host) A.out_host[pd.out_id] = po;
                shared[0] = c;
            }
            asm volatile("s_waitcnt vmcnt(0)" ::: "memory");
        }
        __syncthreads();
        const uint32_t c = shared[0];
        uint32_t nwr = c < SWMI_TB_SLOTS ? c : SWMI_TB_SLOTS;
        if (nwr > n_waves) nwr = n_waves;
        if (c > ccap || wave >= nwr) return;
        po.n_cells = c;
        uint32_t *lds = walker_lds0 + wave * per_walker;
        uint32_t *tile = tiles + wave * WIN_WORDS;
        if (R == 1)      traceback_pair<1, 1, false>(A, pd, po, lane, wave, nwr, lds, tile, nullptr, 1u);
        else if (R == 2) traceback_pair<2, 1, false>(A, pd, po, lane, wave, nwr, lds, tile, nullptr, 1u);
        else if (R == 3) traceback_pair<3, 1, false>(A, pd, po, lane, wave, nwr, lds, tile, nullptr, 1u);
        else             traceback_pair<4, 1, false>(A, pd, po, lane, wave, nwr, lds, tile, nullptr, 1u);
        return;
    }
    uint32_t pre_wlo;
    if (R == 1)      pre_wlo = winmax_detect<1>(A, pd, po, lane, wave, n_waves, ccap, tiles, walker_lds0, per_walker, shared);
    else if (R == 2) pre_wlo = winmax_detect<2>(A, pd, po, lane, wave, n_waves, ccap, tiles, walker_lds0, per_walker, shared);
    else if (R == 3) pre_wlo = winmax_detect<3>(A, pd, po, lane, wave, n_waves, ccap, tiles, walker_lds0, per_walker, shared);
    else             pre_wlo = winmax_detect<4>(A, pd, po, lane, wave, n_waves, ccap, tiles, walker_lds0, per_walker, shared);
    const uint32_t cnt = shared[0];
    if (shared[3] != 1u) pre_wlo = 0xFFFFFFFFu;
    if (cnt > ccap || cnt == 0u) return;
    po.n_cells = cnt;
    uint32_t nw = cnt < SWMI_TB_SLOTS ? cnt : SWMI_TB_SLOTS;
    if (nw > n_waves) nw = n_waves;
    const uint32_t ts = n_waves / nw;
    if (ts == 1u) {
        if (wave >= nw) return;
        uint32_t *lds = walker_lds0 + wave * per_walker;
        uint32_t *tile = tiles + wave * WIN_WORDS;
        if (R == 1)      traceback_pair<1, 1, false, false>(A, pd, po, lane, wave, nw, lds, tile, nullptr, 1u, pre_wlo, true);
        else if (R == 2) traceback_pair<2, 1, false, false>(A, pd, po, lane, wave, nw, lds, tile, nullptr, 1u, pre_wlo, true);
        else if (R == 3) traceback_pair<3, 1, false, false>(A, pd, po, lane, wave, nw, lds, tile, nullptr, 1u, pre_wlo, true);
        else             traceback_pair<4, 1, false, false>(A, pd, po, lane, wave, nw, lds, tile, nullptr, 1u, pre_wlo, true);
        return;
    }
    if (wave < nw) {
        uint32_t *lds = walker_lds0 + wave * per_walker;
        uint32_t *tile = tiles + wave * ts * WIN_WORDS;
        uint32_t *tile2 = tiles2 ? tiles2 + wave * ts * WIN_WORDS : nullptr;
        if (R == 1)      traceback_pair<1, 1, true, false>(A, pd, po, lane, wave, nw, lds, tile, shared, ts, pre_wlo, true, nullptr, tile2);
        else if (R == 2) traceback_pair<2, 1, true, false>(A, pd, po, lane, wave, nw, lds, tile, shared, ts, pre_wlo, true, nullptr, tile2);
        else if (R == 3) traceback_pair<3, 1, true, false>(A, pd, po, lane, wave, nw, lds, tile, shared, ts, pre_wlo, true, nullptr, tile2);
        else             traceback_pair<4, 1, true, false>(A, pd, po, lane, wave, nw, lds, tile, shared, ts, pre_wlo, true, nullptr, tile2);
    } else {
        if (R == 1)      coop_helper<1>(A, pd, lane, wave, nw, ts, n_waves, tiles, shared);
        else if (R == 2) coop_helper<2>(A, pd, lane, wave, nw, ts, n_waves, tiles, shared);
        else if (R == 3) coop_helper<3>(A, pd, lane, wave, nw, ts, n_waves, tiles, shared);
        else             coop_helper<4>(A, pd, lane, wave, nw, ts, n_waves, tiles, shared);
    }
}

extern "C" __global__ void __launch_bounds__(WAVE * FILL_WAVES)
sw_traceback_kernel(const TraceArgs A) {
    extern __shared__ uint32_t tb_lds[];
    traceback_entry<0>(A, tb_lds);
}

extern "C" __global__ void __launch_bounds__(WAVE * FILL_WAVES)
sw_traceback_replay_kernel(const TraceArgs A) {
    extern __shared__ uint32_t tb_lds[];
    traceback_entry<1>(A, tb_lds);
}

#define SWMI_SPLIT_WAVES 4u

extern "C" __global__ void __launch_bounds__(WAVE * SWMI_SPLIT_WAVES)
sw_detect_windows_kernel(const TraceArgs A) {
    extern __shared__ uint32_t dw_lds[];
    const uint32_t wave = threadIdx.x >> 6, lane = threadIdx.x & 63u;
    const uint32_t item = blockIdx.x * SWMI_SPLIT_WAVES + wave;
    const uint32_t n_items = A.win_off[A.n_pairs];
    if (item >= n_items) return;
    uint32_t lo = 0, hi = A.n_pairs;
    while (hi - lo > 1u) {
        const uint32_t mid = (lo + hi) >> 1;
        if (A.win_off[mid] <= item) lo = mid; else hi = mid;
    }
    const uint32_t pair = lo, wloc = item - A.win_off[pair];
    const PairDesc pd = A.pairs[pair];
    PairOut po = A.out[pd.out_id];
    if (finish_pair(A, pd, po) && wloc == 0u && lane == 0) A.out[pd.out_id] = po;
    if (po.flags & (SWMI_F_DEGENERATE | SWMI_F_DONE)) return;
    const SeqDesc rd = A.refs[pd.ref_id];
    const SeqDesc qd = A.reads[pd.read_id];
    const uint32_t n = rd.len, m = qd.len;
    const uint32_t R = swmi_rows_per_lane(m);
    const uint64_t wblocks = ((uint64_t)n + 63u + 15u) / 16u;
    const uint32_t n_ck = (uint32_t)((wblocks + SWMI_CK_BLOCKS - 1u) / SWMI_CK_BLOCKS);
    const uint32_t strip = wloc / n_ck, g = wloc - strip * n_ck;
    const uint64_t wmax_off = (uint64_t)n_ck * (R + 2) * WAVE;
    const uint64_t strip_words = wmax_off + (uint64_t)((n_ck + 63u) & ~63u);
    if ((int)A.dir[pd.dir_off + strip * strip_words + wmax_off + g] != po.score) return;

    constexpr uint32_t WIN_WORDS = SWMI_CK_BLOCKS * SWMI_RMAX * WAVE;
    uint32_t *tile = dw_lds + wave * (WIN_WORDS + 2u * SWMI_DETECT_LCAP);
    uint2 *found = reinterpret_cast<uint2 *>(tile + WIN_WORDS);
    const uint32_t *__restrict__ refw = A.seqw + rd.boff;
    const uint32_t *__restrict__ readw = A.seqw + qd.boff;
    const bool acgt = rd.acgt && qd.acgt && SWMI_SCORES_FIT(A);
    uint32_t cnt;
    if (R == 1)      { const StripGeom G = strip_geom<1>(m, n, 1u); cnt = replay_any<1, true>(A, pd, n, m, acgt, refw, readw, G, strip, g * SWMI_CK_BLOCKS, lane, tile, po.score, 0u, found, SWMI_DETECT_LCAP); }
    else if (R == 2) { const StripGeom G = strip_geom<2>(m, n, 1u); cnt = replay_any<2, true>(A, pd, n, m, acgt, refw, readw, G, strip, g * SWMI_CK_BLOCKS, lane, tile, po.score, 0u, found, SWMI_DETECT_LCAP); }
    else if (R == 3) { const StripGeom G = strip_geom<3>(m, n, 1u); cnt = replay_any<3, true>(A, pd, n, m, acgt, refw, readw, G, strip, g * SWMI_CK_BLOCKS, lane, tile, po.score, 0u, found, SWMI_DETECT_LCAP); }
    else             { const StripGeom G = strip_geom<4>(m, n, 1u); cnt = replay_any<4, true>(A, pd, n, m, acgt, refw, readw, G, strip, g * SWMI_CK_BLOCKS, lane, tile, po.score, 0u, found, SWMI_DETECT_LCAP); }
    if (cnt == 0u) return;
    WAVE_SYNC();
    const uint64_t cbase = A.cells_off ? A.cells_off[pd.out_id] : (uint64_t)pd.out_id * A.cell_cap;
    const uint32_t ccap = A.cells_cap ? A.cells_cap[pd.out_id] : A.cell_cap;
    unsigned long long base = 0;
    uint32_t qbase = 0;
    const uint32_t have = cnt < SWMI_DETECT_LCAP ? cnt : SWMI_DETECT_LCAP;
// ... 115 lines not shown
#endif
            {
                sweep_tail_block<R>(S, w, wnext.x, t0, lane_eff, n, one, gm);
            }
        }
        const int wm = wave_max_i32(lane < lact ? S.lmax : -1);
        if (lane == 0) wmaxs[(nblk - 1u) / SWMI_CK_BLOCKS] = (uint32_t)wm;
        pair_max = pair_max > wm ? pair_max : wm;
    }
    PairOut po;
    if (pair_max <= 0) {
        po.score = 0; po.flags = SWMI_F_DEGENERATE | SWMI_F_DONE; po.n_cells = (uint64_t)m * n;
        if (lane == 0) { A.out[pd.out_id] = po; if (A.out_host) A.out_host[pd.out_id] = po; }
        return;
    }
    WAVE_SYNC();

    uint32_t ncell;
    {
        FillState<R> S;
        S.thr = pair_max; S.cnt = 0; S.ev_prev = 0; S.events = 0; S.dbg_skip = false; S.lmax = -1;
        setup_rows<R, true>(S, readw, lane * R, m, A.match, A.mismatch);
        uint4 wnext = refq[0];
        for (uint32_t tb = 0; tb < nblk; ++tb) {
            const uint4 w = wnext;
            wnext = refq[tb + 1];
            const uint32_t t0 = 16u * tb;
            const bool steady = (t0 + 1u >= lact) && (t0 + 15u < n);
            const bool hot = (int)wmaxs[tb / SWMI_CK_BLOCKS] == pair_max;
            if (hot) {
                if (steady) fill_block16<R, true, STRICT, false, false, SWMI_MODE_DETECT>(S, w, t0, lane, lane_eff, n, m, lane * R, A.gap, A.match, A.mismatch,
                                                                                          0, false, false, nullptr, cells, X.res_cell_cap);
                else        fill_block16<R, true, STRICT, false, true, SWMI_MODE_DETECT>(S, w, t0, lane, lane_eff, n, m, lane * R, A.gap, A.match, A.mismatch,
                                                                                         0, false, false, nullptr, cells, X.res_cell_cap);
            } else {
                if (steady) fill_block16<R, true, STRICT, false, false, SWMI_MODE_REPLAY>(S, w, t0, lane, lane_eff, n, m, lane * R, A.gap, A.match, A.mismatch,
                                                                                          0, false, false, nullptr, nullptr, 0u);
                else        fill_block16<R, true, STRICT, false, true, SWMI_MODE_REPLAY>(S, w, t0, lane, lane_eff, n, m, lane * R, A.gap, A.match, A.mismatch,
                                                                                         0, false, false, nullptr, nullptr, 0u);
            }
            const int miss = (int)(t0 + 15u) - ((int)(lane + n) - 1);
#pragma unroll
            for (int k = 0; k < R; ++k) {
                uint32_t v = S.acc[k];
                if (miss > 0 && miss < 16) v <<= 2 * miss;
                field[(tb * R + k) * WAVE + lane] = v;
            }
        }
        ncell = S.cnt;
    }
    po.score = pair_max; po.flags = SWMI_F_DONE | (ncell > X.res_cell_cap ? SWMI_F_CELL_OVF : 0u); po.n_cells = ncell;
    if (lane == 0) { A.out[pd.out_id] = po; if (A.out_host) A.out_host[pd.out_id] = po; }
    if (ncell > X.res_cell_cap || ncell == 0u) return;
    WAVE_SYNC();

    const uint8_t *ref_b = reinterpret_cast<const uint8_t *>(refc);
    const uint8_t *read_b = reinterpret_cast<const uint8_t *>(readc);
    const uint32_t umat = (uint32_t)A.match, umis = (uint32_t)A.mismatch, ugap = (uint32_t)A.gap;
    const uint32_t max_ops = 16u * X.res_ops_words;
    for (uint32_t base = 0; base < ncell; base += WAVE) {
        const bool mine = base + lane < ncell;
        const uint2 c0 = mine ? cells[base + lane] : make_uint2(0u, 0u);
        uint32_t i = c0.x, j = c0.y, score = (uint32_t)pair_max, nops = 0, cur = 0;
        int begin = 0;
        bool active = mine;
        uint32_t *my_ops = opsb + lane * X.res_ops_words;
        while (BALLOT(active)) {
            if (active) {
                const uint32_t rho = i - 1u, l = rho / R, k = rho - l * R;
                const uint32_t t = j - 1u + l;
                const uint32_t dw = field[((t >> 4) * R + k) * WAVE + l];
                const uint32_t rc = ref_b[j - 1u], qc = read_b[i - 1u];
                const uint32_t d = (dw >> (2u * (15u - (t & 15u)))) & 3u;
                const bool isA = (d & 1u) != 0u, isI = d == 2u;
                begin = (int)j;
                score -= isA ? (rc == qc ? umat : umis) : ugap;
                const uint32_t op = isA ? SWMI_DIR_A : (isI ? SWMI_DIR_I : SWMI_DIR_D);
                cur |= op << (2u * (nops & 15u));
                ++nops;
                if ((nops & 15u) == 0u) { if (nops <= max_ops) my_ops[(nops >> 4) - 1u] = cur; cur = 0; }
                i -= (isA || isI) ? 1u : 0u;
                j -= (isA || !isI) ? 1u : 0u;
                active = (int)score > 0 && i != 0u && j != 0u;
            }
        }
        if ((nops & 15u) != 0u && nops <= max_ops) my_ops[nops >> 4] = cur;
        WAVE_SYNC();
        const uint32_t opw = A.raw ? 0u : (nops + 15u) / 16u;
        const uint32_t words = mine ? swmi_payload_words(nops, A.raw != nullptr) : 0u;
        const uint32_t incl = wave_scan_add_u32(words);
        const uint32_t total = (uint32_t)__builtin_amdgcn_readlane((int)incl, 63);
        const uint32_t nhere = ncell - base < WAVE ? ncell - base : WAVE;
        unsigned long long off;
        uint32_t rslot;
        const bool fits = swmi_reserve(A, lane, total, nhere, off, rslot);
        const bool too_long = BALLOT(mine && nops > max_ops) != 0ull;
        if (fits && !too_long) {
            if (mine) {
                uint32_t *dst = A.arena + off + (incl - words);
                swmi_write_rec(A, rslot + lane, pd.out_id, SWMI_RANK_BY_CELL, begin, c0.x, c0.y, nops, off + (incl - words));
                for (uint32_t w = 0; w < opw; ++w) dst[w] = my_ops[w];
            }
            if (A.raw) {
                const uint8_t *__restrict__ raw_ref = A.raw + A.raw_off[pd.ref_id];
                const uint8_t *__restrict__ raw_read = A.raw + A.raw_off[A.raw_reads_at + pd.read_id];
                for (uint32_t a = 0; a < nhere; ++a) {
                    const uint32_t na = (uint32_t)__builtin_amdgcn_readlane((int)nops, (int)a);
                    const uint32_t at = (uint32_t)__builtin_amdgcn_readlane((int)(incl - words), (int)a);
                    const uint32_t ai = (uint32_t)__builtin_amdgcn_readlane((int)c0.x, (int)a);
                    const uint32_t aj = (uint32_t)__builtin_amdgcn_readlane((int)c0.y, (int)a);
                    swmi_emit_strings(A.arena + off + at, SwmiOpsPacked{opsb + a * X.res_ops_words},
                                      na, ai, aj, raw_ref, raw_read, lane, scratch);
                }
            }
        } else if (lane == 0) {
            atomicOr(&A.out[pd.out_id].flags, SWMI_F_ARENA_OVF);
            if (A.ovf_host) *A.ovf_host = 1u;
        }
        WAVE_SYNC();
    }
}

extern "C" __global__ void __launch_bounds__(WAVE * FILL_WAVES)
sw_resident_pairs_kernel(const TraceArgs A, const ResidentArgs X) {
    extern __shared__ uint32_t rp_lds[];
    const uint32_t wave = threadIdx.x >> 6, lane = threadIdx.x & 63u;
    const uint32_t item = blockIdx.x * FILL_WAVES + wave;
    if (item >= X.n_res) return;
    const PairDesc pd = A.pairs[X.res_items[item]];
    uint32_t *lds = rp_lds + wave * X.res_lds_words;
    const uint32_t R = swmi_rows_per_lane(A.reads[pd.read_id].len);
    if (A.strict) {
        if (R == 1)      resident_pair<1, true>(A, X, pd, lane, lds);
        else if (R == 2) resident_pair<2, true>(A, X, pd, lane, lds);
        else if (R == 3) resident_pair<3, true>(A, X, pd, lane, lds);
        else             resident_pair<4, true>(A, X, pd, lane, lds);
    } else {
        if (R == 1)      resident_pair<1, false>(A, X, pd, lane, lds);
        else if (R == 2) resident_pair<2, false>(A, X, pd, lane, lds);
        else if (R == 3) resident_pair<3, false>(A, X, pd, lane, lds);
        else             resident_pair<4, false>(A, X, pd, lane, lds);
    }
}

extern "C" hipError_t swmi_launch_resident(const TraceArgs *a, const ResidentArgs *x, hipStream_t st) {
    if (x->n_res == 0) return hipSuccess;
    static const bool attr = [] { swmi_allow_big_lds(sw_resident_pairs_kernel); return true; }();
    (void)attr;
    hipLaunchKernelGGL(sw_resident_pairs_kernel, dim3((x->n_res + FILL_WAVES - 1) / FILL_WAVES), dim3(WAVE * FILL_WAVES),
                       (size_t)FILL_WAVES * x->res_lds_words * sizeof(uint32_t), st, *a, *x);
    return hipGetLastError();
}

extern "C" hipError_t swmi_launch_traceback(const TraceArgs *a, hipStream_t st, hipEvent_t ev_start, hipEvent_t ev_stop) {
    if (a->n_pairs == 0) return hipSuccess;
    const size_t tile = (size_t)(a->mode == 0 ? SWMI_TB_BLOCKS : SWMI_CK_BLOCKS) * SWMI_RMAX * WAVE;
    const size_t per_wave = (size_t)a->lds_words + a->lds_read_words + SWMI_TB_REFWIN_WORDS + tile;
    const dim3 block(WAVE * FILL_WAVES);
    if (a->mode == 1) {
        static int forced = getenv("SWMI_TB_WAVES") ? atoi(getenv("SWMI_TB_WAVES")) : 0;
        static int big = getenv("SWMI_TB_BIG") ? atoi(getenv("SWMI_TB_BIG")) : 10000;
        const uint32_t n_waves = forced ? (uint32_t)forced : (a->n_pairs <= 512u ? SWMI_TB_WAVES : a->n_pairs <= (uint32_t)big ? 4u : 1u);
        const size_t n_walkers = n_waves < SWMI_TB_SLOTS ? n_waves : SWMI_TB_SLOTS;
        const size_t tiles = (size_t)n_waves * SWMI_CK_BLOCKS * SWMI_RMAX * WAVE;
        size_t words = 32 + tiles + n_walkers * ((size_t)a->lds_words + a->lds_read_words + SWMI_TB_REFWIN_WORDS);
        static const int spec_opt = getenv("SWMI_TB_SPEC") ? atoi(getenv("SWMI_TB_SPEC")) : 1;
        TraceArgs t = *a;
        t.pad2 = (spec_opt && (spec_opt == 2 || a->n_pairs <= 384u) && n_waves > 1u && (words + tiles) * sizeof(uint32_t) <= 160u * 1024u) ? 1u : 0u;
        if (t.pad2) words += tiles;
        if (ev_start && ev_stop)
            hipExtLaunchKernelGGL(sw_traceback_winmax_kernel, dim3(a->n_pairs), dim3(WAVE * n_waves), (uint32_t)(words * sizeof(uint32_t)), st, ev_start, ev_stop, 0u, t);
        else
            hipLaunchKernelGGL(sw_traceback_winmax_kernel, dim3(a->n_pairs), dim3(WAVE * n_waves), words * sizeof(uint32_t), st, t);
    } else {
        const dim3 grid((a->n_pairs + FILL_WAVES - 1) / FILL_WAVES, SWMI_TB_SLOTS);
        if (a->mode == 0) hipLaunchKernelGGL(sw_traceback_kernel, grid, block, per_wave * FILL_WAVES * sizeof(uint32_t), st, *a);
        else              hipLaunchKernelGGL(sw_traceback_replay_kernel, grid, block, per_wave * FILL_WAVES * sizeof(uint32_t), st, *a);
    }
    return hipGetLastError();
}
```

### sparksmithwaterman_amd/csrc/swmi_walk.h

```cpp
#pragma once
#include <hip/hip_runtime.h>
#include <stdint.h>
#include "swmi_device.h"
#include "swmi_emit.h"
#include "swmi_cells.h"

#ifndef SWMI_HELPER_SLEEP
#define SWMI_HELPER_SLEEP 8
#endif

#define SWMI_TB_SLOTS 4u
#if SWMI_CK_BLOCKS > 2
#define SWMI_TB_WAVES 4u
#else
#define SWMI_TB_WAVES 8u
#endif

template <int R, bool STRICT>
__device__ __forceinline__ void replay_window_fast(const TraceArgs &A, const PairDesc pd, const uint32_t n, const uint32_t m,
                                                   const uint32_t *__restrict__ refw, const uint32_t *__restrict__ readw,
                                                   const uint32_t wlo, const uint32_t lane, uint32_t *__restrict__ lds_tile) {
    const uint32_t gm = (uint32_t)(-(int64_t)A.gap);
    const int one = 1;
    int h[R], g[R], hp[R], q[R];
    uint32_t acc[R];
    const uint32_t *__restrict__ ck = A.dir + pd.dir_off + (uint64_t)(wlo / SWMI_CK_BLOCKS) * (R + 2) * WAVE + lane;
    build_profiles<R>(q, readw, lane * R, m, A.match, A.mismatch);
#pragma unroll
    for (int k = 0; k < R; ++k) {
        h[k] = (int)ld_l2(ck + k * WAVE);
        hp[k] = (uint32_t)h[k] > gm ? (int)((uint32_t)h[k] - gm) : 0;
        g[k] = 0;
        acc[k] = 0;
    }
    const int nprev = (int)ld_l2(ck + R * WAVE);
    g[R - 1] = __builtin_amdgcn_update_dpp(0, nprev, 0x130 , 0xf, 0xf, true);
    const int rb_ck = (int)ld_l2(ck + (R + 1) * WAVE);
    const uint32_t lact = m >= WAVE * R ? WAVE : (m + R - 1) / R;
    const uint32_t T = n + lact - 1, nblk = (T + 15u) / 16u;
    const uint4 *__restrict__ refq = reinterpret_cast<const uint4 *>(refw);
    uint4 wv[SWMI_CK_BLOCKS + 1];
#pragma unroll
    for (uint32_t b = 0; b <= SWMI_CK_BLOCKS; ++b) wv[b] = refq[wlo + b];
    int rbx = wave_shr1((int)(1u << (wv[0].x & 31u)), rb_ck), rby = rb_ck;
#pragma unroll
    for (uint32_t b = 0; b < SWMI_CK_BLOCKS; ++b) {
        if (wlo + b >= nblk) break;
        const uint4 w = wv[b];
        DirStep4Asm<R, STRICT>::run(h, g, hp, acc, q, rbx, rby, w.x, w.y, one, gm);
        DirStep4Asm<R, STRICT>::run(h, g, hp, acc, q, rbx, rby, w.y, w.z, one, gm);
        DirStep4Asm<R, STRICT>::run(h, g, hp, acc, q, rbx, rby, w.z, w.w, one, gm);
        DirStep4Asm<R, STRICT>::run(h, g, hp, acc, q, rbx, rby, w.w, wv[b + 1].x, one, gm);
#pragma unroll
        for (int k = 0; k < R; ++k) lds_tile[(b * R + k) * WAVE + lane] = acc[k];
    }
}

template <int R, bool ACGT, bool STRICT, bool MULTI, bool DETECT>
__device__ __forceinline__ uint32_t replay_window(const TraceArgs &A, const PairDesc pd, const uint32_t n, const uint32_t m,
                                                  const uint32_t *__restrict__ refw, const uint32_t *__restrict__ readw,
                                                  const StripGeom G, const uint32_t s, const uint32_t wlo,
                                                  const uint32_t lane, uint32_t *__restrict__ lds_tile,
                                                  const int maxv, const uint32_t cnt_in, uint2 *__restrict__ cells, const uint32_t ccap) {
#ifndef SWMI_NO_ASM
    if constexpr (ACGT && !MULTI && !DETECT) {
        if (A.gap <= 0 && s == 0u) {
            replay_window_fast<R, STRICT>(A, pd, n, m, refw, readw, wlo, lane, lds_tile);
            return cnt_in;
        }
    }
#endif
    constexpr int BM = DETECT ? SWMI_MODE_DETECT : SWMI_MODE_REPLAY;
    FillState<R> S;
    S.thr = DETECT ? maxv : 0x7FFFFFFF; S.cnt = cnt_in; S.ev_prev = 0; S.events = 0; S.dbg_skip = false; S.lmax = -1;
    const uint32_t row0 = s * G.rps + lane * R;
    const uint32_t rows_left = m - s * G.rps;
    const uint32_t lact = rows_left >= G.rps ? WAVE : (rows_left + R - 1) / R;
    const uint32_t T = n + lact - 1;
    const uint32_t lane_eff = lane < lact ? lane : 0x40000000u;
    setup_rows<R, ACGT>(S, readw, row0, m, A.match, A.mismatch);
    const uint32_t *__restrict__ ck = A.dir + pd.dir_off + s * G.strip_words +
                                      (uint64_t)(wlo / SWMI_CK_BLOCKS) * (R + 2) * WAVE + lane;
#pragma unroll
    for (int k = 0; k < R; ++k) S.h[k] = (int)ld_l2(ck + k * WAVE);
    S.nprev = (int)ld_l2(ck + R * WAVE);
    S.rb = (int)ld_l2(ck + (R + 1) * WAVE);
    const int32_t *seam_in = nullptr;
    if (MULTI) seam_in = A.seam + pd.seam_off + (uint64_t)(s > 0 ? s - 1 : 0) * (n + 1);
    const bool reads_seam = MULTI && (s > 0);
    const uint32_t nblk = (T + 15u) / 16u;
    const uint4 *__restrict__ refq = reinterpret_cast<const uint4 *>(refw);
    uint4 wv[SWMI_CK_BLOCKS];
#pragma unroll
    for (uint32_t b = 0; b < SWMI_CK_BLOCKS; ++b) wv[b] = refq[wlo + b];
#pragma unroll
    for (uint32_t b = 0; b < SWMI_CK_BLOCKS; ++b) {
        const uint32_t tb = wlo + b;
        if (tb >= nblk) break;
        const uint4 w = wv[b];
        const uint32_t t0 = 16u * tb;
        int seamv = 0;
        if (reads_seam) {
            const uint32_t col = t0 + 1u + (lane & 15u);
            seamv = col <= n ? (int)ld_l2((const uint32_t *)seam_in + col) : 0;
        }
        const bool steady = (t0 + 1u >= lact) && (t0 + 15u < n);
        if (steady)
            fill_block16<R, ACGT, STRICT, MULTI, false, BM>(S, w, t0, lane, lane_eff, n, m, row0, A.gap, A.match, A.mismatch,
                                                            seamv, reads_seam, false, nullptr, cells, ccap);
        else
            fill_block16<R, ACGT, STRICT, MULTI, true, BM>(S, w, t0, lane, lane_eff, n, m, row0, A.gap, A.match, A.mismatch,
                                                           seamv, reads_seam, false, nullptr, cells, ccap);
        const int miss = (int)(t0 + 15u) - ((int)(lane + n) - 1);
#pragma unroll
        for (int k = 0; k < R; ++k) {
            uint32_t v = S.acc[k];
            if (miss > 0 && miss < 16) v <<= 2 * miss;
            lds_tile[(b * R + k) * WAVE + lane] = v;
        }
    }
    return S.cnt;
}

template <int R, bool MULTI, bool DETECT>
__device__ __forceinline__ uint32_t replay_dispatch(const TraceArgs &A, const PairDesc pd, uint32_t n, uint32_t m, bool acgt,
                                                    const uint32_t *__restrict__ refw, const uint32_t *__restrict__ readw,
                                                    const StripGeom G, uint32_t s, uint32_t wlo, uint32_t lane, uint32_t *lds_tile,
                                                    int maxv, uint32_t cnt_in, uint2 *__restrict__ cells, uint32_t ccap) {
    if (acgt) {
        if (A.strict) return replay_window<R, true, true, MULTI, DETECT>(A, pd, n, m, refw, readw, G, s, wlo, lane, lds_tile, maxv, cnt_in, cells, ccap);
        else          return replay_window<R, true, false, MULTI, DETECT>(A, pd, n, m, refw, readw, G, s, wlo, lane, lds_tile, maxv, cnt_in, cells, ccap);
    } else {
        if (A.strict) return replay_window<R, false, true, MULTI, DETECT>(A, pd, n, m, refw, readw, G, s, wlo, lane, lds_tile, maxv, cnt_in, cells, ccap);
        else          return replay_window<R, false, false, MULTI, DETECT>(A, pd, n, m, refw, readw, G, s, wlo, lane, lds_tile, maxv, cnt_in, cells, ccap);
    }
}

__device__ __forceinline__ bool finish_pair(const TraceArgs &A, const PairDesc pd, PairOut &po) {
    if (po.score > 0 || (po.flags & SWMI_F_DEGENERATE)) return false;
    po.score = 0;
    po.flags = SWMI_F_DEGENERATE;
    po.n_cells = (uint64_t)A.reads[pd.read_id].len * A.refs[pd.ref_id].len;
    return true;
}

__device__ __forceinline__ bool swmi_common_pair(const TraceArgs &A, const SeqDesc rd, const SeqDesc qd) {
    return rd.acgt && qd.acgt && SWMI_SCORES_FIT(A) && !A.strict;
}

template <int R, bool DETECT, bool FULL = true>
__device__ __forceinline__ uint32_t replay_any(const TraceArgs &A, const PairDesc pd, uint32_t n, uint32_t m, bool acgt,
                                               const uint32_t *__restrict__ refw, const uint32_t *__restrict__ readw,
                                               const StripGeom G, uint32_t s, uint32_t wlo, uint32_t lane, uint32_t *lds_tile,
                                               int maxv, uint32_t cnt_in, uint2 *__restrict__ cells, uint32_t ccap) {
    if constexpr (!FULL) {
        if constexpr (R == SWMI_RMAX) {
            if (m > WAVE * SWMI_RMAX)
                return replay_window<R, true, false, true, DETECT>(A, pd, n, m, refw, readw, G, s, wlo, lane, lds_tile, maxv, cnt_in, cells, ccap);
        }
        return replay_window<R, true, false, false, DETECT>(A, pd, n, m, refw, readw, G, s, wlo, lane, lds_tile, maxv, cnt_in, cells, ccap);
    }
    if constexpr (R == SWMI_RMAX) {
        if (m > WAVE * SWMI_RMAX)
            return replay_dispatch<R, true, DETECT>(A, pd, n, m, acgt, refw, readw, G, s, wlo, lane, lds_tile, maxv, cnt_in, cells, ccap);
    }
    return replay_dispatch<R, false, DETECT>(A, pd, n, m, acgt, refw, readw, G, s, wlo, lane, lds_tile, maxv, cnt_in, cells, ccap);
}

template <int R, bool FULL = true>
__device__ __forceinline__ uint32_t detect_cells(const TraceArgs &A, const PairDesc pd, const PairOut po,
                                                 const uint32_t lane, uint32_t *__restrict__ lds_tile) {
    const SeqDesc rd = A.refs[pd.ref_id];
    const SeqDesc qd = A.reads[pd.read_id];
    const uint32_t n = rd.len, m = qd.len;
    const uint32_t *__restrict__ refw = A.seqw + rd.boff;
    const uint32_t *__restrict__ readw = A.seqw + qd.boff;
    const StripGeom G = strip_geom<R>(m, n, 1u);
    const bool acgt = rd.acgt && qd.acgt && SWMI_SCORES_FIT(A);
    const uint64_t cbase = A.cells_off ? A.cells_off[pd.out_id] : (uint64_t)pd.out_id * A.cell_cap;
    const uint32_t ccap = A.cells_cap ? A.cells_cap[pd.out_id] : A.cell_cap;
    uint2 *__restrict__ cells = const_cast<uint2 *>(A.cells) + cbase;
    uint32_t cnt = 0;
    for (uint32_t s = 0; s < G.n_strips; ++s) {
        const uint32_t *__restrict__ wm = A.dir + pd.dir_off + s * G.strip_words + G.wmax_off;
        for (uint32_t g0 = 0; g0 < G.n_ck; g0 += WAVE) {
            const uint32_t g = g0 + lane;
            const int wv = g < G.n_ck ? (int)wm[g] : -1;
            uint64_t cand = BALLOT(wv == po.score);
            while (cand) {
                const uint32_t gg = g0 + (uint32_t)__builtin_ctzll(cand);
                cand &= cand - 1ull;
                cnt = replay_any<R, true, FULL>(A, pd, n, m, acgt, refw, readw, G, s, gg * SWMI_CK_BLOCKS, lane, lds_tile,
                                          po.score, cnt, cells, ccap);
            }
        }
    }
    return cnt;
}

#ifdef SWMI_TB_DIAG
#define TB_DBG (A.dbg != nullptr)
#else
#define TB_DBG false
#endif
template <int R, int TMODE, bool COOP, bool FULL = true>
__device__ __forceinline__ void traceback_pair(const TraceArgs &A, const PairDesc pd, const PairOut po,
                                               const uint32_t lane, const uint32_t slot, const uint32_t nslots,
                                               uint32_t *__restrict__ lds, uint32_t *__restrict__ lds_tile,
                                               volatile uint32_t *__restrict__ shared, const uint32_t ts,
                                               uint32_t pre_wlo = 0xFFFFFFFFu, const bool read_staged = false,
                                               const uint4 *__restrict__ one = nullptr, uint32_t *__restrict__ lds_tile_alt = nullptr) {
    const SeqDesc rd = A.refs[pd.ref_id];
    const SeqDesc qd = A.reads[pd.read_id];
    const uint32_t n = rd.len, m = qd.len;
    const uint32_t *__restrict__ refw = A.seqw + rd.boff;
    const uint32_t *__restrict__ readw = A.seqw + qd.boff;
    const StripGeom G = strip_geom<R>(m, n, A.mode);
    const uint32_t rps = G.rps;
    const uint32_t *__restrict__ dirp = A.dir + pd.dir_off;
    const uint32_t umat = (uint32_t)A.match, umis = (uint32_t)A.mismatch, ugap = (uint32_t)A.gap;
    const int dec0 = A.match > A.mismatch ? A.match : A.mismatch;
    const bool dec_fits = dec0 <= 0x7FFFFFFF / 23 && A.gap <= 0x7FFFFFFF / 23;
    const uint32_t udec = !dec_fits ? 0xFFFFFFFFu : dec0 > 0 ? (uint32_t)dec0 : 0u;
    const uint32_t ugdec = !dec_fits ? 0xFFFFFFFFu : A.gap > 0 ? (uint32_t)A.gap : 0u;
    (void)udec; (void)ugdec;
    const bool acgt = rd.acgt && qd.acgt && SWMI_SCORES_FIT(A);
    const uint8_t *__restrict__ raw_ref = A.raw ? A.raw + A.raw_off[pd.ref_id] : nullptr;
    const uint8_t *__restrict__ raw_read = A.raw ? A.raw + A.raw_off[A.raw_reads_at + pd.read_id] : nullptr;

    uint32_t *lds_ops = lds;
    uint32_t *lds_read = lds_ops + A.lds_words;
    uint32_t *lds_ref = lds_read + A.lds_read_words;
    uint8_t *ops_b = reinterpret_cast<uint8_t *>(lds_ops);
    const uint8_t *read_b = reinterpret_cast<const uint8_t *>(lds_read);
    const uint8_t *ref_b = reinterpret_cast<const uint8_t *>(lds_ref);
    uint32_t req_seq = 0, req_expected = 0;
    uint32_t *tile_cur = lds_tile, *tile_alt = lds_tile_alt;
    uint32_t spec_wlo = 0xFFFFFFFFu, spec_hi = 0u, spec_rv0 = 0u, spec_rv1 = 0u;
    auto team_wait = [&]() {
        while (__hip_atomic_load(const_cast<uint32_t *>(&shared[20u + slot]), __ATOMIC_RELAXED, __HIP_MEMORY_SCOPE_WORKGROUP) < req_expected)
            __builtin_amdgcn_s_sleep(1);
        __builtin_amdgcn_fence(__ATOMIC_ACQUIRE, "workgroup");
    };
    auto team_request = [&](uint32_t flags, uint32_t first_block, uint32_t nq, uint32_t delivered) {
        ++req_seq;
        req_expected += delivered;
        if (lane == 0) {
            shared[4u + 4u * slot] = flags; shared[5u + 4u * slot] = first_block; shared[6u + 4u * slot] = nq;
            __builtin_amdgcn_fence(__ATOMIC_RELEASE, "workgroup");
            __hip_atomic_store(const_cast<uint32_t *>(&shared[7u + 4u * slot]), req_seq, __ATOMIC_RELAXED, __HIP_MEMORY_SCOPE_WORKGROUP);
        }
    };

    const unsigned long long tk0 = TB_DBG ? __builtin_amdgcn_s_memtime() : 0ull;
    unsigned long long tk_walk = 0, tk_stage = 0, n_steps = 0, n_iters = 0;
    if (!read_staged)
        for (uint32_t w = lane; w < (m + 3u) / 4u; w += WAVE) lds_read[w] = readw[w];

    const uint64_t cbase = A.cells_off ? A.cells_off[pd.out_id] : (uint64_t)pd.out_id * A.cell_cap;
    const uint32_t ncell = one ? 1u : (uint32_t)po.n_cells;
    const uint2 *__restrict__ cells = A.cells + cbase;

    for (uint32_t base = 0; base < ncell; base += WAVE) {
        const uint32_t idx = base + lane;
        uint2 mine = make_uint2(0, 0);
        if (one) { mine.x = one->y; mine.y = one->z; }
        else if (idx < ncell) { mine.x = ld_l2(&cells[idx].x); mine.y = ld_l2(&cells[idx].y); }
        const uint64_t mykey = A.strict ? (((uint64_t)(mine.x + mine.y) << 32) | mine.y)
                                        : (((uint64_t)mine.x << 32) | mine.y);
        uint32_t rank = (one || ncell > WAVE) ? SWMI_RANK_BY_CELL : 0u;
        if (ncell > 1 && ncell <= WAVE) {
            for (uint32_t o = 0; o < ncell; ++o) {
                uint2 c; c.x = ld_l2(&cells[o].x); c.y = ld_l2(&cells[o].y);
                const uint64_t kk = A.strict ? (((uint64_t)(c.x + c.y) << 32) | c.y) : (((uint64_t)c.x << 32) | c.y);
                rank += (kk < mykey) ? 1u : 0u;
            }
        }
        const uint32_t nhere = ncell - base < WAVE ? ncell - base : WAVE;

        for (uint32_t a = slot; a < nhere; a += nslots) {
            const uint32_t ci = __builtin_amdgcn_readlane((int)mine.x, a);
            const uint32_t cj = __builtin_amdgcn_readlane((int)mine.y, a);
            const uint32_t crank = __builtin_amdgcn_readlane((int)rank, a);

            uint32_t i = ci, j = cj;
            uint32_t score = (uint32_t)po.score;
            uint32_t n_ops = 0;
            int begin = 0;
            while ((int)score > 0 && i != 0u && j != 0u) {
                const unsigned long long ts0 = TB_DBG ? __builtin_amdgcn_s_memtime() : 0ull;
                const uint32_t s = (i - 1u) / rps;
                int rho = (int)((i - 1u) - s * rps);
                const uint32_t t_cur = j - 1u + (uint32_t)rho / R;
                const uint32_t whi = t_cur >> 4;
                uint32_t wlo, nb;
                if (TMODE == 0) {
                    wlo = whi >= SWMI_TB_BLOCKS - 1u ? whi - (SWMI_TB_BLOCKS - 1u) : 0u;
                    nb = whi - wlo + 1u;
                } else if (COOP) {
                    const uint32_t wtop = whi - whi % SWMI_CK_BLOCKS;
                    wlo = wtop >= (ts - 1u) * SWMI_CK_BLOCKS ? wtop - (ts - 1u) * SWMI_CK_BLOCKS : 0u;
                    nb = wtop + SWMI_CK_BLOCKS - wlo;
                } else {
                    wlo = whi - whi % SWMI_CK_BLOCKS;
                    nb = SWMI_CK_BLOCKS;
                }
                bool use_spec = false;
                if (COOP && spec_wlo != 0xFFFFFFFFu) {
                    const uint32_t wtop = whi - whi % SWMI_CK_BLOCKS;
                    if (s == 0u && wtop + SWMI_CK_BLOCKS == spec_hi) { use_spec = true; wlo = spec_wlo; nb = spec_hi - spec_wlo; }
                }
                const bool prestaged = TMODE == 1 && pre_wlo == wlo && s == 0u && !use_spec;
                pre_wlo = 0xFFFFFFFFu;
                const int clo = (int)(16u * wlo) - 63;
                const uint32_t cw0 = clo > 0 ? (uint32_t)clo >> 2 : 0u;
                const uint32_t cw1 = (16u * (wlo + nb) - 1u) >> 2;
                WAVE_SYNC();
                if (use_spec) {
                    const unsigned long long tq0 = TB_DBG ? __builtin_amdgcn_s_memtime() : 0ull;
                    team_wait();
                    if (TB_DBG) tk_walk += (__builtin_amdgcn_s_memtime() - tq0) << 32;
                    uint32_t *t = tile_cur; tile_cur = tile_alt; tile_alt = t;
                    lds_ref[lane] = spec_rv0;
                    if (lane + WAVE < SWMI_TB_REFWIN_WORDS) lds_ref[lane + WAVE] = spec_rv1;
                    WAVE_SYNC();
                } else if (!prestaged) {
                    const uint32_t rx0 = cw0 + lane, rx1 = rx0 + WAVE, rlim = (n + 3u) / 4u;
                    const uint32_t rv0 = (rx0 <= cw1 && rx0 < rlim) ? refw[rx0] : 0u;
                    const uint32_t rv1 = (rx1 <= cw1 && rx1 < rlim) ? refw[rx1] : 0u;
                    if (TMODE == 0) {
                        const uint32_t *__restrict__ src = dirp + s * G.strip_words + (uint64_t)wlo * R * WAVE + lane;
                        for (uint32_t x = 0; x < nb * R; ++x) tile_cur[x * WAVE + lane] = src[(uint64_t)x * WAVE];
                    } else {
                        if (COOP) {
                            team_wait();
                            const uint32_t nq = nb / SWMI_CK_BLOCKS;
                            team_request((tile_cur == lds_tile ? 0u : 1u) | (s << 2), wlo, nq, nq - 1u);
                        }
                        (void)replay_any<R, false, FULL>(A, pd, n, m, acgt, refw, readw, G, s, wlo, lane, tile_cur, 0, 0u, nullptr, 0u);
                    }
                    lds_ref[lane] = rv0;
                    if (lane + WAVE < SWMI_TB_REFWIN_WORDS) lds_ref[lane + WAVE] = rv1;
                    if (COOP) {
                        const unsigned long long tq0 = TB_DBG ? __builtin_amdgcn_s_memtime() : 0ull;
                        team_wait();
                        if (TB_DBG) tk_walk += (__builtin_amdgcn_s_memtime() - tq0) << 32;
                    }
                    WAVE_SYNC();
                }
                spec_wlo = 0xFFFFFFFFu;
                if (COOP && tile_alt != nullptr && ts > 1u && wlo > 0u && s == 0u) {
                    const uint32_t have = wlo / SWMI_CK_BLOCKS, nq = have < ts - 1u ? have : ts - 1u;
                    spec_hi = wlo;
                    spec_wlo = wlo - nq * SWMI_CK_BLOCKS;
                    const int sclo = (int)(16u * spec_wlo) - 63;
                    const uint32_t scw0 = sclo > 0 ? (uint32_t)sclo >> 2 : 0u, scw1 = (16u * spec_hi - 1u) >> 2;
                    const uint32_t rx0 = scw0 + lane, rx1 = rx0 + WAVE, rlim = (n + 3u) / 4u;
                    spec_rv0 = (rx0 <= scw1 && rx0 < rlim) ? refw[rx0] : 0u;
                    spec_rv1 = (rx1 <= scw1 && rx1 < rlim) ? refw[rx1] : 0u;
                    team_request((tile_alt == lds_tile ? 0u : 1u) | 2u, spec_wlo, nq, nq);
                }
                const int tmin = (int)(16u * wlo);
                const unsigned long long tw0 = TB_DBG ? __builtin_amdgcn_s_memtime() : 0ull;
                if (TB_DBG) { tk_stage += tw0 - ts0; n_iters += 1ull << 32; }

#ifdef SWMI_WALK_CHASE
                for (;;) {
                    if (TB_DBG) ++n_iters;
                    const uint32_t na = lane >> 3, nb = lane & 7u;
                    const int rho_x = rho - (int)na;
                    const uint32_t rx = rho_x > 0 ? (uint32_t)rho_x : 0u;
                    const uint32_t lx = rx / R, kx = rx - lx * R;
                    const uint32_t jj = j - nb;
                    const int tx = (int)jj - 1 + (int)lx;
                    const bool valid = rho_x >= 0 && j > nb && tx >= tmin;
                    const uint32_t dw = tile_cur[valid ? (((uint32_t)tx >> 4) - wlo) * (R * WAVE) + kx * WAVE + lx : 0u];
                    const uint32_t rc = ref_b[valid ? (jj - 1u) - 4u * cw0 : 0u];
                    const uint32_t qc = read_b[valid ? i - 1u - na : 0u];
                    const uint32_t d = (dw >> (2u * (15u - ((uint32_t)tx & 15u)))) & 3u;
                    const uint32_t b0 = d & 1u, b1 = (d >> 1) & 1u;
                    const uint32_t di = b0 | b1, dj = b0 | (b1 ^ 1u);
                    const uint32_t op = (b0 << 1) | (b1 & (b0 ^ 1u));
                    const int delta = (int)(b0 ? (rc == qc ? umat : umis) : ugap);
                    const uint32_t last = (na + di > 7u || nb + dj > 7u) ? 1u : 0u;
                    const uint32_t edge = (i - na == di || j - nb == dj) ? 1u : 0u;
                    const int ctrl = valid ? (int)(0x80000000u | (edge << 9) | (last << 8) | (op << 4) | (di << 3) | dj) : 0;
                    const uint32_t si = uni(i), sj = uni(j);
                    uint32_t sscore = uni(score);
                    uint32_t idx = 0, sh = 0, opsacc = 0, lastc = 0, lastidx = 0;
                    bool done = false;
                    for (;;) {
                        const uint32_t c = (uint32_t)__builtin_amdgcn_readlane(ctrl, (int)idx);
                        if ((int)c >= 0) break;
                        sscore -= (uint32_t)__builtin_amdgcn_readlane(delta, (int)idx);
                        opsacc |= ((c >> 4) & 3u) << sh;
                        sh += 2u;
                        lastc = c; lastidx = idx;
                        idx += c & 15u;
                        if ((int)sscore <= 0) { done = true; break; }
                        if (c & 0x300u) {
                            if (c & 0x200u) { sscore = 0; done = true; }
                            break;
                        }
                    }
                    const uint32_t cnt = sh >> 1;
                    const uint32_t ca = cnt ? (lastidx >> 3) + ((lastc >> 3) & 1u) : 0u, cb = cnt ? (lastidx & 7u) + (lastc & 7u) : 0u;
                    score = sscore;
                    if (cnt) begin = (int)(sj - (lastidx & 7u));
                    if (lane < cnt && n_ops + lane < 4u * A.lds_words) ops_b[n_ops + lane] = (uint8_t)((opsacc >> (2u * lane)) & 3u);
                    n_ops += cnt; i = si - ca; j = sj - cb; rho -= (int)ca;
                    if (done || cnt == 0u || rho < 0) break;
                }
#else
                for (;;) {
                    if (TB_DBG) ++n_iters;
                    const uint32_t grp = lane / 21u, x = lane - grp * 21u;
                    const uint32_t di = grp == 1u ? 1u : 0u, dj = grp == 2u ? 1u : 0u;
                    const int rho_x = rho - (int)di - (int)x;
                    const uint32_t rx = rho_x > 0 ? (uint32_t)rho_x : 0u;
                    const uint32_t lx = rx / R, kx = rx - lx * R;
                    const uint32_t jj = j - dj - x;
                    const int tx = (int)jj - 1 + (int)lx;
                    const bool valid = grp < 3u && rho_x >= 0 && j > dj + x && tx >= tmin;
                    uint32_t dw = tile_cur[valid ? (((uint32_t)tx >> 4) - wlo) * (R * WAVE) + kx * WAVE + lx : 0u];
                    uint32_t rc = ref_b[valid ? (jj - 1u) - 4u * cw0 : 0u];
                    uint32_t qc = read_b[valid ? i - 1u - di - x : 0u];
                    asm volatile("" : "+v"(dw), "+v"(rc), "+v"(qc));
                    const uint32_t d = (dw >> (2u * (15u - ((uint32_t)tx & 15u)))) & 3u;
                    const bool mt = rc == qc;
                    const uint64_t vmask = BALLOT(valid);
                    if (!(vmask & 1ull)) break;
                    const uint64_t amask = BALLOT((d & 1u) != 0u) & vmask;
                    const uint64_t imask = BALLOT(d == 2u) & vmask;
                    const uint64_t mm = BALLOT(mt);
                    {
                        const uint32_t g1 = (uint32_t)(~amask & 1ull);
                        const uint32_t isI1 = (uint32_t)(imask & 1ull);
                        const uint32_t fb = g1 ? (isI1 ? 21u : 42u) : 0u;
                        const uint32_t vb = (uint32_t)(vmask >> fb) & 0x1FFFFFu;
                        const uint32_t frun = (uint32_t)__builtin_ctz(~((uint32_t)(amask >> fb) & 0x1FFFFFu));
                        const uint32_t has3 = (vb >> frun) & 1u;
                        if ((!g1 || (vb & 1u)) && score > (g1 + has3) * ugdec + frun * udec) {
                            const uint32_t isI3 = (uint32_t)(imask >> (fb + frun)) & 1u & has3;
                            const uint32_t nm = (uint32_t)__builtin_popcountll(mm & ((((1ull << frun) - 1ull)) << fb));
                            const uint32_t i1 = g1 & isI1, total = g1 + frun + has3;
                            score -= (g1 + has3) * ugap + nm * umat + (frun - nm) * umis;
                            const uint32_t j1 = j - (g1 - i1);
                            begin = has3 ? (int)(j1 - frun) : (frun ? (int)(j1 - frun + 1u) : (int)j);
                            if (lane < total && n_ops + lane < 4u * A.lds_words)
                                ops_b[n_ops + lane] = (uint8_t)(lane < g1 ? (isI1 ? SWMI_DIR_I : SWMI_DIR_D)
                                                               : lane < g1 + frun ? SWMI_DIR_A : (isI3 ? SWMI_DIR_I : SWMI_DIR_D));
                            n_ops += total;
                            const uint32_t dec_i = i1 + frun + isI3;
                            i -= dec_i; rho -= (int)dec_i;
                            j = j1 - frun - (has3 - isI3);
                            continue;
                        }
                    }
                    bool done = false;
                    uint32_t base = 0;
                    if (!(amask & 1ull)) {
                        begin = (int)j;
                        score -= ugap;
                        uint32_t op;
                        if (imask & 1ull) { --i; --rho; op = SWMI_DIR_I; base = 21u; } else { --j; op = SWMI_DIR_D; base = 42u; }
                        if (lane == 0 && n_ops < 4u * A.lds_words) ops_b[n_ops] = (uint8_t)op;
                        n_ops += 1u;
                        if ((int)score <= 0) break;
                        if (i == 0 || j == 0) { score = 0; break; }
                        if (rho < 0 || !((vmask >> base) & 1ull)) continue;
                    }
                    uint32_t run = (uint32_t)__builtin_ctzll(~((amask >> base) & 0x1FFFFFull));
                    if (run > 0) {
                        const uint64_t range = ((1ull << run) - 1ull) << base;
                        if (score > run * udec) {
                            const uint32_t nm = (uint32_t)__builtin_popcountll(mm & range);
                            score -= nm * umat + (run - nm) * umis;
                        } else {
                            const bool in_run = (range >> lane) & 1ull;
                            const uint32_t cm = lanemask_lt_count(mm & range) + (mt ? 1u : 0u);
                            const uint32_t after = score - (cm * umat + (lane - base + 1u - cm) * umis);
                            const uint64_t z = BALLOT(in_run && (int)after <= 0);
                            if (z) { run = (uint32_t)__builtin_ctzll(z) - base + 1u; done = true; }
                            score = (uint32_t)__builtin_amdgcn_readlane((int)after, base + run - 1u);
                        }
                        begin = (int)(j - (run - 1u));
                        if (lane >= base && lane < base + run && n_ops + (lane - base) < 4u * A.lds_words)
                            ops_b[n_ops + (lane - base)] = (uint8_t)SWMI_DIR_A;
                        n_ops += run; i -= run; j -= run; rho -= (int)run;
                        if (done || (int)score <= 0) break;
                        if (i == 0 || j == 0) { score = 0; break; }
                        if (rho < 0) break;
// ... 70 lines not shown
```

Measured before the change: 2566.

## Add specialized single-strip traceback kernel for uniform-R ACGT batches

Adds a fast traceback path that is selected when every pair in a chunk is single-strip, shares one rows-per-lane value, uses ACGT symbols and non-strict ties. The new kernel is templated per R with a ONE_STRIP flag that removes the multi-strip window-replay branch, and it uses an occupancy hint of five waves per EU. The winmax detect and cooperative helper code moves into a shared header. This should cut instruction overhead and register pressure in the common case, at the price of more kernel instances to compile and an extra planner pass over the pairs.

```diff
diff --git a/include/swmi.h b/include/swmi.h
--- a/include/swmi.h
+++ b/include/swmi.h
@@ -67,6 +67,7 @@
     uint32_t col_chunks;
     uint32_t resident_pairs;
     uint32_t tfused_pairs;
+    uint32_t tb_fast_pairs;
 } swmi_timing;
 int  swmi_batch_timing(const swmi_batch *b, swmi_timing *t);
 int  swmi_batch_mode(const swmi_batch *b, int *mode);
diff --git a/sparksmithwaterman_amd/_capi.py b/sparksmithwaterman_amd/_capi.py
--- a/sparksmithwaterman_amd/_capi.py
+++ b/sparksmithwaterman_amd/_capi.py
@@ -30,7 +30,7 @@
                 ("total_ms", C.c_float), ("fill_launches", C.c_uint32), ("rerun_pairs", C.c_uint32),
                 ("cells", C.c_uint64), ("dir_bytes", C.c_uint64),
                 ("strip_fallbacks", C.c_uint32), ("col_chunks", C.c_uint32),
-                ("resident_pairs", C.c_uint32), ("tfused_pairs", C.c_uint32)]
+                ("resident_pairs", C.c_uint32), ("tfused_pairs", C.c_uint32), ("tb_fast_pairs", C.c_uint32)]
 
 
 class StreamStats(C.Structure):
diff --git a/sparksmithwaterman_amd/csrc/swmi_ctx.cpp b/sparksmithwaterman_amd/csrc/swmi_ctx.cpp
--- a/sparksmithwaterman_amd/csrc/swmi_ctx.cpp
+++ b/sparksmithwaterman_amd/csrc/swmi_ctx.cpp
@@ -129,6 +129,9 @@
     } else if (!strcmp(name, "tfused")) {
         if (value < -1 || value > 1) return fail(SWMI_ERR_INVALID, "tfused must be -1 (automatic), 0 or 1");
         ctx->tfused = (int)value;
+    } else if (!strcmp(name, "tb_fast")) {
+        if (value < -1 || value > 1) return fail(SWMI_ERR_INVALID, "tb_fast must be -1 (automatic), 0 or 1");
+        ctx->tb_fast = (int)value;
     } else if (!strcmp(name, "resident")) {
         if (value < -1 || value > 1) return fail(SWMI_ERR_INVALID, "resident must be -1 (automatic), 0 or 1");
         ctx->resident = (int)value;
diff --git a/sparksmithwaterman_amd/csrc/swmi_host.h b/sparksmithwaterman_amd/csrc/swmi_host.h
--- a/sparksmithwaterman_amd/csrc/swmi_host.h
+++ b/sparksmithwaterman_amd/csrc/swmi_host.h
@@ -127,6 +127,7 @@
     int tb_split = -1;
     bool ext_events = false;
     int tfused = -1;
+    int tb_fast = -1;
     int resident = -1;
     int scores_only = 0;
     int stream_keep_records = 1;
@@ -188,7 +189,7 @@
     uint32_t eff_mode = 0;
     uint32_t col_chunks = 0;
     bool reverse_strips = false;
-    int resident = -1, tfused = -1;
+    int resident = -1, tfused = -1, tb_fast = -1;
     bool exact = false;
     bool scores_only = false;
     uint64_t mat_gen = 0;
@@ -198,7 +199,7 @@
     bool operator==(const PlanKey &o) const {
         return valid == o.valid && lo == o.lo && hi == o.hi && work == o.work && memcmp(&params, &o.params, sizeof(swmi_params)) == 0 &&
                eff_mode == o.eff_mode && col_chunks == o.col_chunks && reverse_strips == o.reverse_strips && resident == o.resident &&
-               tfused == o.tfused && exact == o.exact && scores_only == o.scores_only && mat_gen == o.mat_gen &&
+               tfused == o.tfused && tb_fast == o.tb_fast && exact == o.exact && scores_only == o.scores_only && mat_gen == o.mat_gen &&
                modes == o.modes && d_pairs == o.d_pairs && pairs_bytes == o.pairs_bytes;
     }
 };
@@ -215,6 +216,7 @@
     uint32_t res_lds_words = 0, res_ops_words = 0;
     size_t n_tf = 0;
     uint32_t tf_max_m = 0, tf_max_n = 0, tf_max_path = 0;
+    uint32_t tb_fast_r = 0;
     uint32_t aff_r_min = 0xFFFFFFFFu, aff_r_max = 0;
     size_t aff_n_long = 0;
 };
diff --git a/sparksmithwaterman_amd/csrc/swmi_launch.h b/sparksmithwaterman_amd/csrc/swmi_launch.h
--- a/sparksmithwaterman_amd/csrc/swmi_launch.h
+++ b/sparksmithwaterman_amd/csrc/swmi_launch.h
@@ -9,7 +9,9 @@
 }
 
 extern "C" hipError_t swmi_launch_fill(const FillArgs *a, hipStream_t st, hipEvent_t ev_start, hipEvent_t ev_stop);
-extern "C" hipError_t swmi_launch_traceback(const TraceArgs *a, hipStream_t st, hipEvent_t ev_start, hipEvent_t ev_stop);
+extern "C" hipError_t swmi_launch_traceback(const TraceArgs *a, uint32_t fast_r, hipStream_t st, hipEvent_t ev_start, hipEvent_t ev_stop);
+extern "C" hipError_t swmi_launch_traceback_fast(const TraceArgs *t, uint32_t R, uint32_t n_waves, size_t lds_bytes, hipStream_t st,
+                                                 hipEvent_t ev_start, hipEvent_t ev_stop);
 extern "C" hipError_t swmi_launch_traceback_split(const TraceArgs *a, uint32_t n_windows, hipStream_t st);
 extern "C" hipError_t swmi_launch_resident(const TraceArgs *a, const ResidentArgs *x, hipStream_t st);
 extern "C" hipError_t swmi_launch_tfused(const TraceArgs *a, const TFusedArgs *x, hipStream_t st);
diff --git a/sparksmithwaterman_amd/csrc/swmi_plan.h b/sparksmithwaterman_amd/csrc/swmi_plan.h
--- a/sparksmithwaterman_amd/csrc/swmi_plan.h
+++ b/sparksmithwaterman_amd/csrc/swmi_plan.h
@@ -72,6 +72,7 @@
     uint64_t chunk_budget = 1;
     bool res_possible = false, res_maybe = false;
     bool tf_possible = false;
+    bool fast_possible = false;
 
     Planner(const swmi_ctx *ctx_, const swmi_batch *b_, size_t np_, bool exact, ChunkPlan &plan_, PlanItems &it_)
         : ctx(ctx_), b(b_), P(b_->params), np(np_), plan(plan_), it(it_) {
@@ -83,6 +84,8 @@
                        P.match <= 7 && P.match >= -8 && P.mismatch >= -8 && P.mismatch <= 0 && P.gap <= 0;
         tf_possible = whole && ctx->tfused == 1 &&
                       P.match > 0 && P.match <= 7 && P.mismatch >= -8 && P.mismatch <= P.match && P.gap < 0 && P.gap >= -64;
+        fast_possible = mode1 && !ctx->scores_only && ctx->tb_fast != 0 && P.tie_mode != SWMI_TIE_STRICT && P.gap <= 0 &&
+                        P.match >= -8 && P.match <= 7 && P.mismatch >= -8 && P.mismatch <= 7;
     }
     bool fast_symbols(const PairDesc &d) const { return b->read_desc[d.read_id].acgt && b->ref_desc[d.ref_id].acgt; }
 
@@ -217,7 +220,7 @@
     if (pl.res_possible)
         for (size_t k = 0; k < np && !pl.res_maybe; k++)
             pl.res_maybe = pl.res_size_fits(b->read_desc[work[lo + k].pair % n_reads].len, b->ref_desc[work[lo + k].pair / n_reads].len);
-    if ((pl.cols_possible || pl.res_maybe || pl.tf_possible) && !b->acgt_known) {
+    if ((pl.cols_possible || pl.res_maybe || pl.tf_possible || pl.fast_possible) && !b->acgt_known) {
         if (b->n_refs) HIP_TRY(hipMemcpy(b->ref_desc.data(), b->d_refs.p, b->n_refs * sizeof(SeqDesc), hipMemcpyDeviceToHost));
         if (b->n_reads) HIP_TRY(hipMemcpy(b->read_desc.data(), b->d_reads.p, b->n_reads * sizeof(SeqDesc), hipMemcpyDeviceToHost));
         b->acgt_known = true;
@@ -225,6 +228,8 @@
     it.pd.resize(np);
     if (b->eff_mode == 1) it.win_off.resize(np + 1);
     uint32_t pb_m = 0xFFFFFFFFu, pb_n = 0xFFFFFFFFu, pb_val = 0;
+    uint32_t fast_r = 0;
+    bool fast_all = pl.fast_possible && np > 0;
     const int32_t smax = b->opt.mat ? std::max(b->params.match, b->opt.mat->max_entry) : b->params.match;
     for (size_t k = 0; k < np; k++) {
         const Work &w = work[lo + k];
@@ -244,6 +249,11 @@
         else if (b->eff_mode == 1 && m_ > 64u * SWMI_RMAX && it.strip_items.size() < (1u << 30)) pl.take_strips(k, d, m_, n_);
         else if (pl.cols_fit(d, m_)) pl.take_cols(k, d, m_, n_);
         it.pd[k] = d;
+        if (fast_all) {
+            const uint32_t r = swmi_rows_per_lane(m_);
+            fast_all = m_ <= 64u * SWMI_RMAX && (fast_r == 0 || fast_r == r) && pl.fast_symbols(d);
+            fast_r = r;
+        }
         if (m_ != pb_m || n_ != pb_n) { pb_m = m_; pb_n = n_; pb_val = (uint32_t)path_bound(n_, m_, b->params, smax, b->opt.modes.align_mode); }
         plan.max_path = std::max<uint32_t>(plan.max_path, pb_val);
         plan.max_read = std::max(plan.max_read, m_);
@@ -252,6 +262,7 @@
         plan.aff_r_max = std::max(plan.aff_r_max, swmi_aff_rows_per_lane(m_));
     }
     pl.finish(work, lo);
+    plan.tb_fast_r = fast_all ? fast_r : 0u;
     if (b->eff_mode == 3 && plan.aff_n_long) {
         std::stable_partition(it.pd.begin(), it.pd.end(), [&](const PairDesc &d) { return b->read_desc[d.read_id].len <= SWMI_AFF_MAX_READ; });
     }
@@ -300,7 +311,7 @@
     key.lo = lo; key.hi = hi; key.work = (const void *)work.data();
     key.params = b->params; key.eff_mode = b->eff_mode;
     key.col_chunks = ctx->col_chunks; key.reverse_strips = ctx->dbg_reverse_strips != 0;
-    key.resident = ctx->resident; key.tfused = ctx->tfused;
+    key.resident = ctx->resident; key.tfused = ctx->tfused; key.tb_fast = ctx->tb_fast;
     key.exact = cells_exact != nullptr; key.scores_only = ctx->scores_only != 0;
     key.mat_gen = b->opt.mat ? b->opt.mat->gen : 0u; key.modes = b->opt.modes;
     key.d_pairs = b->d_pairs.p; key.pairs_bytes = np * sizeof(PairDesc);
diff --git a/sparksmithwaterman_amd/csrc/swmi_run.cpp b/sparksmithwaterman_amd/csrc/swmi_run.cpp
--- a/sparksmithwaterman_amd/csrc/swmi_run.cpp
+++ b/sparksmithwaterman_amd/csrc/swmi_run.cpp
@@ -267,7 +267,8 @@
         HIP_TRY(swmi_launch_affine_traceback(&ts, b->opt.modes.kernel_mode(), 0u, 0u, SWMI_AFF_TILE_WORDS, ops_words, ctx->stream));
         HIP_TRY(swmi_launch_affine_traceback(&tl, b->opt.modes.kernel_mode(), 1u, (uint32_t)b->opt.modes.band, SWMI_AFF_TILE_WORDS, ops_words, ctx->stream));
     } else if (n_res + n_tf < np) {
-        HIP_TRY(swmi_launch_traceback(&ta, ctx->stream, ext ? ctx->ev[2] : nullptr, ext ? ctx->ev[3] : nullptr));
+        HIP_TRY(swmi_launch_traceback(&ta, plan.tb_fast_r, ctx->stream, ext ? ctx->ev[2] : nullptr, ext ? ctx->ev[3] : nullptr));
+        if (first && plan.tb_fast_r) b->timing.tb_fast_pairs += (uint32_t)(np - n_res - n_tf);
     }
     if (L.time_all && !ext) HIP_TRY(hipEventRecord(ctx->ev[3], ctx->stream));
 
diff --git a/sparksmithwaterman_amd/csrc/swmi_stream.cpp b/sparksmithwaterman_amd/csrc/swmi_stream.cpp
--- a/sparksmithwaterman_amd/csrc/swmi_stream.cpp
+++ b/sparksmithwaterman_amd/csrc/swmi_stream.cpp
@@ -157,7 +157,7 @@
         if ((rc = swmi_create(ctx->device, &sl.ctx))) { swmi_stream_close(s.release()); return rc; }
         sl.ctx->cell_cap = ctx->cell_cap; sl.ctx->cell_cap_set = ctx->cell_cap_set; sl.ctx->max_workspace_bytes = ctx->max_workspace_bytes;
         sl.ctx->profiling = ctx->profiling; sl.ctx->mode = ctx->mode; sl.ctx->zero_copy = ctx->zero_copy;
-        sl.ctx->tb_split = ctx->tb_split; sl.ctx->col_chunks = ctx->col_chunks; sl.ctx->resident = ctx->resident; sl.ctx->tfused = ctx->tfused;
+        sl.ctx->tb_split = ctx->tb_split; sl.ctx->col_chunks = ctx->col_chunks; sl.ctx->resident = ctx->resident; sl.ctx->tfused = ctx->tfused; sl.ctx->tb_fast = ctx->tb_fast;
         sl.ctx->auto_ties_x100 = ctx->auto_ties_x100; sl.ctx->arena_words_per_pair = ctx->arena_words_per_pair;
         sl.ctx->device_strings = ctx->device_strings; sl.ctx->scores_only = ctx->scores_only;
         sl.ctx->gap_open = ctx->gap_open; sl.ctx->affine = ctx->affine;
diff --git a/sparksmithwaterman_amd/csrc/swmi_team.h b/sparksmithwaterman_amd/csrc/swmi_team.h
--- /dev/null
+++ b/sparksmithwaterman_amd/csrc/swmi_team.h
@@ -0,0 +1,151 @@
+#pragma once
+#include "swmi_walk.h"
+
+template <int R, bool ONE_STRIP = false>
+__device__ __forceinline__ void coop_helper(const TraceArgs &A, const PairDesc pd, const uint32_t lane, const uint32_t wave,
+                                            const uint32_t nw, const uint32_t ts, const uint32_t n_waves_all,
+                                            uint32_t *__restrict__ tiles, volatile uint32_t *__restrict__ shared) {
+    const SeqDesc rd = A.refs[pd.ref_id];
+    const SeqDesc qd = A.reads[pd.read_id];
+    const uint32_t n = rd.len, m = qd.len;
+    const uint32_t *__restrict__ refw = A.seqw + rd.boff;
+    const uint32_t *__restrict__ readw = A.seqw + qd.boff;
+    const StripGeom G = strip_geom<R>(m, n, 1u);
+    const bool acgt = rd.acgt && qd.acgt && SWMI_SCORES_FIT(A);
+    const uint32_t team = (wave - nw) % nw, q = 1u + (wave - nw) / nw;
+    uint32_t last = 0;
+    for (;;) {
+        uint32_t seq;
+        while ((seq = __hip_atomic_load(const_cast<uint32_t *>(&shared[7u + 4u * team]), __ATOMIC_RELAXED, __HIP_MEMORY_SCOPE_WORKGROUP)) == last)
+            __builtin_amdgcn_s_sleep(SWMI_HELPER_SLEEP);
+        if (seq == 0xFFFFFFFFu) break;
+        last = seq;
+        __builtin_amdgcn_fence(__ATOMIC_ACQUIRE, "workgroup");
+        const uint32_t flags = shared[4u + 4u * team], wlo = shared[5u + 4u * team], nq = shared[6u + 4u * team];
+        const uint32_t s = flags >> 2;
+        const uint32_t win = (flags & 2u) ? q - 1u : q;
+        if (q < ts && win < nq) {
+            uint32_t *__restrict__ base = ((flags & 1u) ? tiles + n_waves_all * (SWMI_CK_BLOCKS * SWMI_RMAX * WAVE) : tiles) +
+                                          team * ts * (SWMI_CK_BLOCKS * SWMI_RMAX * WAVE);
+            (void)replay_any<R, false, false, ONE_STRIP>(A, pd, n, m, acgt, refw, readw, G, s, wlo + win * SWMI_CK_BLOCKS, lane,
+                                       base + win * SWMI_CK_BLOCKS * R * WAVE, 0, 0u, nullptr, 0u);
+            __builtin_amdgcn_fence(__ATOMIC_RELEASE, "workgroup");
+            if (lane == 0) atomicAdd(const_cast<uint32_t *>(&shared[20u + team]), 1u);
+        }
+    }
+}
+
+template <int R, bool ONE_STRIP = false>
+__device__ __forceinline__ uint32_t winmax_detect(const TraceArgs &A, const PairDesc pd, PairOut &po, const uint32_t lane,
+                                                  const uint32_t wave, const uint32_t n_waves, const uint32_t ccap,
+                                                  uint32_t *__restrict__ tiles, uint32_t *__restrict__ walker_lds,
+                                                  const uint32_t per_walker, volatile uint32_t *__restrict__ shared) {
+    const SeqDesc rd = A.refs[pd.ref_id];
+    const SeqDesc qd = A.reads[pd.read_id];
+    const uint32_t n = rd.len, m = qd.len;
+    const uint32_t *__restrict__ refw = A.seqw + rd.boff;
+    const uint32_t *__restrict__ readw = A.seqw + qd.boff;
+    const bool acgt = rd.acgt && qd.acgt && SWMI_SCORES_FIT(A);
+    const StripGeom G = strip_geom<R>(m, n, 1u);
+    constexpr uint32_t WIN_WORDS = SWMI_CK_BLOCKS * SWMI_RMAX * WAVE;
+    uint32_t ncand = 0, gc[SWMI_TB_SLOTS] = {0u, 0u, 0u, 0u};
+    if (G.n_strips == 1u) {
+        const uint32_t *__restrict__ wm = A.dir + pd.dir_off + G.wmax_off;
+        for (uint32_t g0 = 0; g0 < G.n_ck; g0 += WAVE) {
+            const uint32_t g = g0 + lane;
+            const int wv = g < G.n_ck ? (int)wm[g] : -1;
+            uint64_t cand = BALLOT(wv == po.score);
+            while (cand) {
+                const uint32_t gg = g0 + (uint32_t)__builtin_ctzll(cand);
+                cand &= cand - 1ull;
+                if (ncand == 0u) gc[0] = gg; else if (ncand == 1u) gc[1] = gg; else if (ncand == 2u) gc[2] = gg; else if (ncand == 3u) gc[3] = gg;
+                ++ncand;
+            }
+        }
+    }
+    auto stage_ref = [&](uint32_t *__restrict__ dst, uint32_t wlo, uint32_t nwin) {
+        const int clo = (int)(16u * wlo) - 63;
+        const uint32_t cw0 = clo > 0 ? (uint32_t)clo >> 2 : 0u;
+        const uint32_t cw1 = (16u * (wlo + nwin * SWMI_CK_BLOCKS) - 1u) >> 2;
+        for (uint32_t x = cw0 + lane; x <= cw1 && x < (n + 3u) / 4u; x += WAVE) dst[x - cw0] = refw[x];
+    };
+    auto publish = [&](uint32_t cnt, uint32_t staged) {
+        if (lane == 0) {
+            po.n_cells = cnt;
+            if (cnt > ccap) po.flags |= SWMI_F_CELL_OVF;
+            A.out[pd.out_id] = po;
+            if (A.out_host) A.out_host[pd.out_id] = po;
+            shared[0] = cnt;
+            shared[3] = staged;
+        }
+        if (lane < SWMI_TB_SLOTS) { shared[7u + 4u * lane] = 0u; shared[20u + lane] = 0u; }
+        asm volatile("s_waitcnt vmcnt(0)" ::: "memory");
+    };
+    const uint64_t cbase = A.cells_off ? A.cells_off[pd.out_id] : (uint64_t)pd.out_id * A.cell_cap;
+    uint2 *__restrict__ cells = const_cast<uint2 *>(A.cells) + cbase;
+
+    const uint32_t seg = ccap / SWMI_TB_SLOTS;
+    if (ncand >= 2u && ncand <= SWMI_TB_SLOTS && ncand <= n_waves && seg >= 1u) {
+        const uint32_t nw = ncand, ts = n_waves / nw;
+        if (wave < nw) {
+            const uint32_t g = wave == 0u ? gc[0] : wave == 1u ? gc[1] : wave == 2u ? gc[2] : gc[3];
+            const uint32_t nq0 = g + 1u < ts ? g + 1u : ts;
+            const uint32_t wlo0 = (g + 1u - nq0) * SWMI_CK_BLOCKS;
+            uint32_t *my = walker_lds + wave * per_walker;
+            for (uint32_t w = lane; w < (m + 3u) / 4u; w += WAVE) my[A.lds_words + w] = readw[w];
+            stage_ref(my + A.lds_words + A.lds_read_words, wlo0, nq0);
+            const uint32_t c = replay_any<R, true, false, ONE_STRIP>(A, pd, n, m, acgt, refw, readw, G, 0u, g * SWMI_CK_BLOCKS, lane,
+                                                   tiles + wave * ts * WIN_WORDS + (nq0 - 1u) * SWMI_CK_BLOCKS * R * WAVE,
+                                                   po.score, 0u, cells + wave * seg, seg);
+            if (lane == 0) { shared[24u + wave] = c; shared[28u + wave] = wlo0; }
+            asm volatile("s_waitcnt vmcnt(0)" ::: "memory");
+        } else {
+            const uint32_t team = (wave - nw) % nw, q = 1u + (wave - nw) / nw;
+            const uint32_t g = team == 0u ? gc[0] : team == 1u ? gc[1] : team == 2u ? gc[2] : gc[3];
+            const uint32_t nq0 = g + 1u < ts ? g + 1u : ts;
+            if (q < nq0)
+                (void)replay_any<R, false, false, ONE_STRIP>(A, pd, n, m, acgt, refw, readw, G, 0u, (g - q) * SWMI_CK_BLOCKS, lane,
+                                           tiles + team * ts * WIN_WORDS + (nq0 - 1u - q) * SWMI_CK_BLOCKS * R * WAVE,
+                                           0, 0u, nullptr, 0u);
+        }
+        __syncthreads();
+        bool one_each = true;
+        for (uint32_t w = 0; w < nw; ++w) one_each = one_each && shared[24u + w] == 1u;
+        if (one_each) {
+            if (wave == 0) {
+                uint2 c = make_uint2(0, 0);
+                if (lane < nw) { c.x = ld_l2(&cells[lane * seg].x); c.y = ld_l2(&cells[lane * seg].y); }
+                if (lane < nw) cells[lane] = c;
+                publish(nw, 1u);
+            }
+            __syncthreads();
+            return wave < nw ? shared[28u + wave] : 0xFFFFFFFFu;
+        }
+        __syncthreads();
+    }
+
+    const bool pre = ncand == 1u;
+    const uint32_t nq0 = gc[0] + 1u < n_waves ? gc[0] + 1u : n_waves;
+    const uint32_t wlo0 = (gc[0] + 1u - nq0) * SWMI_CK_BLOCKS;
+    if (wave == 0) {
+        if (n_waves == 1u) {
+            for (uint32_t w = lane; w < (m + 3u) / 4u; w += WAVE) walker_lds[A.lds_words + w] = readw[w];
+            if (pre) stage_ref(walker_lds + A.lds_words + A.lds_read_words, wlo0, nq0);
+        }
+        const uint32_t cnt = detect_cells<R, false, ONE_STRIP>(A, pd, po, lane, pre ? tiles + (nq0 - 1u) * SWMI_CK_BLOCKS * R * WAVE : tiles);
+        publish(cnt, (pre && cnt == 1u) ? 1u : 0u);
+    } else {
+        if (wave < SWMI_TB_SLOTS)
+            for (uint32_t w = lane; w < (m + 3u) / 4u; w += WAVE) walker_lds[wave * per_walker + A.lds_words + w] = readw[w];
+        if (wave == n_waves - 1u)
+            for (uint32_t w = lane; w < (m + 3u) / 4u; w += WAVE) walker_lds[A.lds_words + w] = readw[w];
+        if (pre) {
+            if (wave < nq0)
+                (void)replay_any<R, false, false, ONE_STRIP>(A, pd, n, m, acgt, refw, readw, G, 0u, wlo0 + (wave - 1u) * SWMI_CK_BLOCKS, lane,
+                                           tiles + (wave - 1u) * SWMI_CK_BLOCKS * R * WAVE, 0, 0u, nullptr, 0u);
+            if (wave == n_waves - 1u) stage_ref(walker_lds + A.lds_words + A.lds_read_words, wlo0, nq0);
+        }
+    }
+    __syncthreads();
+    return (pre && wave == 0) ? wlo0 : 0xFFFFFFFFu;
+}
diff --git a/sparksmithwaterman_amd/csrc/swmi_traceback.hip b/sparksmithwaterman_amd/csrc/swmi_traceback.hip
--- a/sparksmithwaterman_amd/csrc/swmi_traceback.hip
+++ b/sparksmithwaterman_amd/csrc/swmi_traceback.hip
@@ -6,40 +6,7 @@
 #include "swmi_emit.h"
 #include "swmi_launch.h"
 #include "swmi_walk.h"
-
-template <int R>
-__device__ __forceinline__ void coop_helper(const TraceArgs &A, const PairDesc pd, const uint32_t lane, const uint32_t wave,
-                                            const uint32_t nw, const uint32_t ts, const uint32_t n_waves_all,
-                                            uint32_t *__restrict__ tiles, volatile uint32_t *__restrict__ shared) {
-    const SeqDesc rd = A.refs[pd.ref_id];
-    const SeqDesc qd = A.reads[pd.read_id];
-    const uint32_t n = rd.len, m = qd.len;
-    const uint32_t *__restrict__ refw = A.seqw + rd.boff;
-    const uint32_t *__restrict__ readw = A.seqw + qd.boff;
-    const StripGeom G = strip_geom<R>(m, n, 1u);
-    const bool acgt = rd.acgt && qd.acgt && SWMI_SCORES_FIT(A);
-    const uint32_t team = (wave - nw) % nw, q = 1u + (wave - nw) / nw;
-    uint32_t last = 0;
-    for (;;) {
-        uint32_t seq;
-        while ((seq = __hip_atomic_load(const_cast<uint32_t *>(&shared[7u + 4u * team]), __ATOMIC_RELAXED, __HIP_MEMORY_SCOPE_WORKGROUP)) == last)
-            __builtin_amdgcn_s_sleep(SWMI_HELPER_SLEEP);
-        if (seq == 0xFFFFFFFFu) break;
-        last = seq;
-        __builtin_amdgcn_fence(__ATOMIC_ACQUIRE, "workgroup");
-        const uint32_t flags = shared[4u + 4u * team], wlo = shared[5u + 4u * team], nq = shared[6u + 4u * team];
-        const uint32_t s = flags >> 2;
-        const uint32_t win = (flags & 2u) ? q - 1u : q;
-        if (q < ts && win < nq) {
-            uint32_t *__restrict__ base = ((flags & 1u) ? tiles + n_waves_all * (SWMI_CK_BLOCKS * SWMI_RMAX * WAVE) : tiles) +
-                                          team * ts * (SWMI_CK_BLOCKS * SWMI_RMAX * WAVE);
-            (void)replay_any<R, false, false>(A, pd, n, m, acgt, refw, readw, G, s, wlo + win * SWMI_CK_BLOCKS, lane,
-                                       base + win * SWMI_CK_BLOCKS * R * WAVE, 0, 0u, nullptr, 0u);
-            __builtin_amdgcn_fence(__ATOMIC_RELEASE, "workgroup");
-            if (lane == 0) atomicAdd(const_cast<uint32_t *>(&shared[20u + team]), 1u);
-        }
-    }
-}
+#include "swmi_team.h"
 
 template <int TMODE>
 __device__ __forceinline__ void traceback_entry(const TraceArgs &A, uint32_t *lds_all) {
@@ -61,121 +28,6 @@
     else if (R == 2) traceback_pair<2, TMODE, false>(A, pd, po, lane, slot, SWMI_TB_SLOTS, tb_lds, tile, nullptr, 1u);
     else if (R == 3) traceback_pair<3, TMODE, false>(A, pd, po, lane, slot, SWMI_TB_SLOTS, tb_lds, tile, nullptr, 1u);
     else             traceback_pair<4, TMODE, false>(A, pd, po, lane, slot, SWMI_TB_SLOTS, tb_lds, tile, nullptr, 1u);
-}
-
-template <int R>
-__device__ __forceinline__ uint32_t winmax_detect(const TraceArgs &A, const PairDesc pd, PairOut &po, const uint32_t lane,
-                                                  const uint32_t wave, const uint32_t n_waves, const uint32_t ccap,
-                                                  uint32_t *__restrict__ tiles, uint32_t *__restrict__ walker_lds,
-                                                  const uint32_t per_walker, volatile uint32_t *__restrict__ shared) {
-    const SeqDesc rd = A.refs[pd.ref_id];
-    const SeqDesc qd = A.reads[pd.read_id];
-    const uint32_t n = rd.len, m = qd.len;
-    const uint32_t *__restrict__ refw = A.seqw + rd.boff;
-    const uint32_t *__restrict__ readw = A.seqw + qd.boff;
-    const bool acgt = rd.acgt && qd.acgt && SWMI_SCORES_FIT(A);
-    const StripGeom G = strip_geom<R>(m, n, 1u);
-    constexpr uint32_t WIN_WORDS = SWMI_CK_BLOCKS * SWMI_RMAX * WAVE;
-    uint32_t ncand = 0, gc[SWMI_TB_SLOTS] = {0u, 0u, 0u, 0u};
-    if (G.n_strips == 1u) {
-        const uint32_t *__restrict__ wm = A.dir + pd.dir_off + G.wmax_off;
-        for (uint32_t g0 = 0; g0 < G.n_ck; g0 += WAVE) {
-            const uint32_t g = g0 + lane;
-            const int wv = g < G.n_ck ? (int)wm[g] : -1;
-            uint64_t cand = BALLOT(wv == po.score);
-            while (cand) {
-                const uint32_t gg = g0 + (uint32_t)__builtin_ctzll(cand);
-                cand &= cand - 1ull;
-                if (ncand == 0u) gc[0] = gg; else if (ncand == 1u) gc[1] = gg; else if (ncand == 2u) gc[2] = gg; else if (ncand == 3u) gc[3] = gg;
-                ++ncand;
-            }
-        }
-    }
-    auto stage_ref = [&](uint32_t *__restrict__ dst, uint32_t wlo, uint32_t nwin) {
-        const int clo = (int)(16u * wlo) - 63;
-        const uint32_t cw0 = clo > 0 ? (uint32_t)clo >> 2 : 0u;
-        const uint32_t cw1 = (16u * (wlo + nwin * SWMI_CK_BLOCKS) - 1u) >> 2;
-        for (uint32_t x = cw0 + lane; x <= cw1 && x < (n + 3u) / 4u; x += WAVE) dst[x - cw0] = refw[x];
-    };
-    auto publish = [&](uint32_t cnt, uint32_t staged) {
-        if (lane == 0) {
-            po.n_cells = cnt;
-            if (cnt > ccap) po.flags |= SWMI_F_CELL_OVF;
-            A.out[pd.out_id] = po;
-            if (A.out_host) A.out_host[pd.out_id] = po;
-            shared[0] = cnt;
-            shared[3] = staged;
-        }
-        if (lane < SWMI_TB_SLOTS) { shared[7u + 4u * lane] = 0u; shared[20u + lane] = 0u; }
-        asm volatile("s_waitcnt vmcnt(0)" ::: "memory");
-    };
-    const uint64_t cbase = A.cells_off ? A.cells_off[pd.out_id] : (uint64_t)pd.out_id * A.cell_cap;
-    uint2 *__restrict__ cells = const_cast<uint2 *>(A.cells) + cbase;
-
-    const uint32_t seg = ccap / SWMI_TB_SLOTS;
-    if (ncand >= 2u && ncand <= SWMI_TB_SLOTS && ncand <= n_waves && seg >= 1u) {
-        const uint32_t nw = ncand, ts = n_waves / nw;
-        if (wave < nw) {
-            const uint32_t g = wave == 0u ? gc[0] : wave == 1u ? gc[1] : wave == 2u ? gc[2] : gc[3];
-            const uint32_t nq0 = g + 1u < ts ? g + 1u : ts;
-            const uint32_t wlo0 = (g + 1u - nq0) * SWMI_CK_BLOCKS;
-            uint32_t *my = walker_lds + wave * per_walker;
-            for (uint32_t w = lane; w < (m + 3u) / 4u; w += WAVE) my[A.lds_words + w] = readw[w];
-            stage_ref(my + A.lds_words + A.lds_read_words, wlo0, nq0);
-            const uint32_t c = replay_any<R, true, false>(A, pd, n, m, acgt, refw, readw, G, 0u, g * SWMI_CK_BLOCKS, lane,
-                                                   tiles + wave * ts * WIN_WORDS + (nq0 - 1u) * SWMI_CK_BLOCKS * R * WAVE,
-                                                   po.score, 0u, cells + wave * seg, seg);
-            if (lane == 0) { shared[24u + wave] = c; shared[28u + wave] = wlo0; }
-            asm volatile("s_waitcnt vmcnt(0)" ::: "memory");
-        } else {
-            const uint32_t team = (wave - nw) % nw, q = 1u + (wave - nw) / nw;
-            const uint32_t g = team == 0u ? gc[0] : team == 1u ? gc[1] : team == 2u ? gc[2] : gc[3];
-            const uint32_t nq0 = g + 1u < ts ? g + 1u : ts;
-            if (q < nq0)
-                (void)replay_any<R, false, false>(A, pd, n, m, acgt, refw, readw, G, 0u, (g - q) * SWMI_CK_BLOCKS, lane,
-                                           tiles + team * ts * WIN_WORDS + (nq0 - 1u - q) * SWMI_CK_BLOCKS * R * WAVE,
-                                           0, 0u, nullptr, 0u);
-        }
-        __syncthreads();
-        bool one_each = true;
-        for (uint32_t w = 0; w < nw; ++w) one_each = one_each && shared[24u + w] == 1u;
-        if (one_each) {
-            if (wave == 0) {
-                uint2 c = make_uint2(0, 0);
-                if (lane < nw) { c.x = ld_l2(&cells[lane * seg].x); c.y = ld_l2(&cells[lane * seg].y); }
-                if (lane < nw) cells[lane] = c;
-                publish(nw, 1u);
-            }
-            __syncthreads();
-            return wave < nw ? shared[28u + wave] : 0xFFFFFFFFu;
-        }
-        __syncthreads();
-    }
-
-    const bool pre = ncand == 1u;
-    const uint32_t nq0 = gc[0] + 1u < n_waves ? gc[0] + 1u : n_waves;
-    const uint32_t wlo0 = (gc[0] + 1u - nq0) * SWMI_CK_BLOCKS;
-    if (wave == 0) {
-        if (n_waves == 1u) {
-            for (uint32_t w = lane; w < (m + 3u) / 4u; w += WAVE) walker_lds[A.lds_words + w] = readw[w];
-            if (pre) stage_ref(walker_lds + A.lds_words + A.lds_read_words, wlo0, nq0);
-        }
-        const uint32_t cnt = detect_cells<R, false>(A, pd, po, lane, pre ? tiles + (nq0 - 1u) * SWMI_CK_BLOCKS * R * WAVE : tiles);
-        publish(cnt, (pre && cnt == 1u) ? 1u : 0u);
-    } else {
-        if (wave < SWMI_TB_SLOTS)
-            for (uint32_t w = lane; w < (m + 3u) / 4u; w += WAVE) walker_lds[wave * per_walker + A.lds_words + w] = readw[w];
-        if (wave == n_waves - 1u)
-            for (uint32_t w = lane; w < (m + 3u) / 4u; w += WAVE) walker_lds[A.lds_words + w] = readw[w];
-        if (pre) {
-            if (wave < nq0)
-                (void)replay_any<R, false, false>(A, pd, n, m, acgt, refw, readw, G, 0u, wlo0 + (wave - 1u) * SWMI_CK_BLOCKS, lane,
-                                           tiles + (wave - 1u) * SWMI_CK_BLOCKS * R * WAVE, 0, 0u, nullptr, 0u);
-            if (wave == n_waves - 1u) stage_ref(walker_lds + A.lds_words + A.lds_read_words, wlo0, nq0);
-        }
-    }
-    __syncthreads();
-    return (pre && wave == 0) ? wlo0 : 0xFFFFFFFFu;
 }
 
 extern "C" __global__ void __launch_bounds__(WAVE * SWMI_TB_WAVES) __attribute__((amdgpu_waves_per_eu(4, 4)))
@@ -597,7 +449,7 @@
     return hipGetLastError();
 }
 
-extern "C" hipError_t swmi_launch_traceback(const TraceArgs *a, hipStream_t st, hipEvent_t ev_start, hipEvent_t ev_stop) {
+extern "C" hipError_t swmi_launch_traceback(const TraceArgs *a, uint32_t fast_r, hipStream_t st, hipEvent_t ev_start, hipEvent_t ev_stop) {
     if (a->n_pairs == 0) return hipSuccess;
     const size_t tile = (size_t)(a->mode == 0 ? SWMI_TB_BLOCKS : SWMI_CK_BLOCKS) * SWMI_RMAX * WAVE;
     const size_t per_wave = (size_t)a->lds_words + a->lds_read_words + SWMI_TB_REFWIN_WORDS + tile;
@@ -613,6 +465,8 @@
         TraceArgs t = *a;
         t.pad2 = (spec_opt && (spec_opt == 2 || a->n_pairs <= 384u) && n_waves > 1u && (words + tiles) * sizeof(uint32_t) <= 160u * 1024u) ? 1u : 0u;
         if (t.pad2) words += tiles;
+        if (fast_r && words * sizeof(uint32_t) <= 64u * 1024u)
+            return swmi_launch_traceback_fast(&t, fast_r, n_waves, words * sizeof(uint32_t), st, ev_start, ev_stop);
         if (ev_start && ev_stop)
             hipExtLaunchKernelGGL(sw_traceback_winmax_kernel, dim3(a->n_pairs), dim3(WAVE * n_waves), (uint32_t)(words * sizeof(uint32_t)), st, ev_start, ev_stop, 0u, t);
         else
diff --git a/sparksmithwaterman_amd/csrc/swmi_traceback_fast.hip b/sparksmithwaterman_amd/csrc/swmi_traceback_fast.hip
--- /dev/null
+++ b/sparksmithwaterman_amd/csrc/swmi_traceback_fast.hip
@@ -0,0 +1,75 @@
+#include <hip/hip_runtime.h>
+#include <hip/hip_ext.h>
+#include <stdint.h>
+#include "swmi_device.h"
+#include "swmi_emit.h"
+#include "swmi_launch.h"
+#include "swmi_walk.h"
+#include "swmi_team.h"
+
+template <int R>
+__device__ __forceinline__ void traceback_winmax_fast(const TraceArgs &A, uint32_t *wm_lds) {
+    const uint32_t pair = blockIdx.x;
+    if (pair >= A.n_pairs) return;
+    const uint32_t wave = threadIdx.x >> 6, lane = threadIdx.x & 63u;
+    const PairDesc pd = A.pairs[pair];
+    PairOut po = A.out[pd.out_id];
+    if (finish_pair(A, pd, po) && wave == 0 && lane == 0) A.out[pd.out_id] = po;
+    if (po.flags & (SWMI_F_DEGENERATE | SWMI_F_DONE)) {
+        if (A.out_host && wave == 0 && lane == 0) A.out_host[pd.out_id] = po;
+        return;
+    }
+    const uint32_t n_waves = blockDim.x >> 6;
+    const uint32_t per_walker = A.lds_words + A.lds_read_words + SWMI_TB_REFWIN_WORDS;
+    constexpr uint32_t WIN_WORDS = SWMI_CK_BLOCKS * SWMI_RMAX * WAVE;
+    uint32_t *shared = wm_lds;
+    uint32_t *tiles = wm_lds + 32;
+    const uint32_t ccap = A.cells_cap ? A.cells_cap[pd.out_id] : A.cell_cap;
+    const uint32_t tile_sets = A.pad2 ? 2u : 1u;
+    uint32_t *tiles2 = A.pad2 ? tiles + n_waves * WIN_WORDS : nullptr;
+    uint32_t *walker_lds0 = tiles + tile_sets * n_waves * WIN_WORDS;
+    uint32_t pre_wlo = winmax_detect<R, true>(A, pd, po, lane, wave, n_waves, ccap, tiles, walker_lds0, per_walker, shared);
+    const uint32_t cnt = shared[0];
+    if (shared[3] != 1u) pre_wlo = 0xFFFFFFFFu;
+    if (cnt > ccap || cnt == 0u) return;
+    po.n_cells = cnt;
+    uint32_t nw = cnt < SWMI_TB_SLOTS ? cnt : SWMI_TB_SLOTS;
+    if (nw > n_waves) nw = n_waves;
+    const uint32_t ts = n_waves / nw;
+    if (ts == 1u) {
+        if (wave >= nw) return;
+        traceback_pair<R, 1, false, false, true>(A, pd, po, lane, wave, nw, walker_lds0 + wave * per_walker, tiles + wave * WIN_WORDS, nullptr, 1u,
+                                           pre_wlo, true);
+        return;
+    }
+    if (wave < nw) {
+        traceback_pair<R, 1, true, false, true>(A, pd, po, lane, wave, nw, walker_lds0 + wave * per_walker, tiles + wave * ts * WIN_WORDS, shared, ts,
+                                          pre_wlo, true, nullptr, tiles2 ? tiles2 + wave * ts * WIN_WORDS : nullptr);
+    } else {
+        coop_helper<R, true>(A, pd, lane, wave, nw, ts, n_waves, tiles, shared);
+    }
+}
+
+#define SWMI_TB_FAST_KERNEL(R)                                                                                              \
+    extern "C" __global__ void __launch_bounds__(WAVE * SWMI_TB_WAVES) __attribute__((amdgpu_waves_per_eu(5, 5)))          \
+    sw_traceback_winmax_fast_r##R##_kernel(const TraceArgs A) {                                                             \
+        extern __shared__ uint32_t wf_lds[];                                                                                \
+        traceback_winmax_fast<R>(A, wf_lds);                                                                                \
+    }
+SWMI_TB_FAST_KERNEL(1)
+SWMI_TB_FAST_KERNEL(2)
+SWMI_TB_FAST_KERNEL(3)
+SWMI_TB_FAST_KERNEL(4)
+
+extern "C" hipError_t swmi_launch_traceback_fast(const TraceArgs *t, uint32_t R, uint32_t n_waves, size_t lds_bytes, hipStream_t st,
+                                                 hipEvent_t ev_start, hipEvent_t ev_stop) {
+    if (t->n_pairs == 0) return hipSuccess;
+    void (*kernel)(const TraceArgs) = R == 1u ? sw_traceback_winmax_fast_r1_kernel : R == 2u ? sw_traceback_winmax_fast_r2_kernel
+                                    : R == 3u ? sw_traceback_winmax_fast_r3_kernel : R == 4u ? sw_traceback_winmax_fast_r4_kernel : nullptr;
+    if (!kernel || lds_bytes > 64u * 1024u) return hipErrorInvalidValue;
+    if (ev_start && ev_stop)
+        hipExtLaunchKernelGGL(kernel, dim3(t->n_pairs), dim3(WAVE * n_waves), (uint32_t)lds_bytes, st, ev_start, ev_stop, 0u, *t);
+    else
+        hipLaunchKernelGGL(kernel, dim3(t->n_pairs), dim3(WAVE * n_waves), lds_bytes, st, *t);
+    return hipGetLastError();
+}
diff --git a/sparksmithwaterman_amd/csrc/swmi_walk.h b/sparksmithwaterman_amd/csrc/swmi_walk.h
--- a/sparksmithwaterman_amd/csrc/swmi_walk.h
+++ b/sparksmithwaterman_amd/csrc/swmi_walk.h
@@ -148,13 +148,13 @@
     return rd.acgt && qd.acgt && SWMI_SCORES_FIT(A) && !A.strict;
 }
 
-template <int R, bool DETECT, bool FULL = true>
+template <int R, bool DETECT, bool FULL = true, bool ONE_STRIP = false>
 __device__ __forceinline__ uint32_t replay_any(const TraceArgs &A, const PairDesc pd, uint32_t n, uint32_t m, bool acgt,
                                                const uint32_t *__restrict__ refw, const uint32_t *__restrict__ readw,
                                                const StripGeom G, uint32_t s, uint32_t wlo, uint32_t lane, uint32_t *lds_tile,
                                                int maxv, uint32_t cnt_in, uint2 *__restrict__ cells, uint32_t ccap) {
     if constexpr (!FULL) {
-        if constexpr (R == SWMI_RMAX) {
+        if constexpr (R == SWMI_RMAX && !ONE_STRIP) {
             if (m > WAVE * SWMI_RMAX)
                 return replay_window<R, true, false, true, DETECT>(A, pd, n, m, refw, readw, G, s, wlo, lane, lds_tile, maxv, cnt_in, cells, ccap);
         }
@@ -167,7 +167,7 @@
     return replay_dispatch<R, false, DETECT>(A, pd, n, m, acgt, refw, readw, G, s, wlo, lane, lds_tile, maxv, cnt_in, cells, ccap);
 }
 
-template <int R, bool FULL = true>
+template <int R, bool FULL = true, bool ONE_STRIP = false>
 __device__ __forceinline__ uint32_t detect_cells(const TraceArgs &A, const PairDesc pd, const PairOut po,
                                                  const uint32_t lane, uint32_t *__restrict__ lds_tile) {
     const SeqDesc rd = A.refs[pd.ref_id];
@@ -190,7 +190,7 @@
             while (cand) {
                 const uint32_t gg = g0 + (uint32_t)__builtin_ctzll(cand);
                 cand &= cand - 1ull;
-                cnt = replay_any<R, true, FULL>(A, pd, n, m, acgt, refw, readw, G, s, gg * SWMI_CK_BLOCKS, lane, lds_tile,
+                cnt = replay_any<R, true, FULL, ONE_STRIP>(A, pd, n, m, acgt, refw, readw, G, s, gg * SWMI_CK_BLOCKS, lane, lds_tile,
                                           po.score, cnt, cells, ccap);
             }
         }
@@ -203,7 +203,7 @@
 #else
 #define TB_DBG false
 #endif
-template <int R, int TMODE, bool COOP, bool FULL = true>
+template <int R, int TMODE, bool COOP, bool FULL = true, bool ONE_STRIP = false>
 __device__ __forceinline__ void traceback_pair(const TraceArgs &A, const PairDesc pd, const PairOut po,
                                                const uint32_t lane, const uint32_t slot, const uint32_t nslots,
                                                uint32_t *__restrict__ lds, uint32_t *__restrict__ lds_tile,
@@ -337,7 +337,7 @@
                             const uint32_t nq = nb / SWMI_CK_BLOCKS;
                             team_request((tile_cur == lds_tile ? 0u : 1u) | (s << 2), wlo, nq, nq - 1u);
                         }
-                        (void)replay_any<R, false, FULL>(A, pd, n, m, acgt, refw, readw, G, s, wlo, lane, tile_cur, 0, 0u, nullptr, 0u);
+                        (void)replay_any<R, false, FULL, ONE_STRIP>(A, pd, n, m, acgt, refw, readw, G, s, wlo, lane, tile_cur, 0, 0u, nullptr, 0u);
                     }
                     lds_ref[lane] = rv0;
                     if (lane + WAVE < SWMI_TB_REFWIN_WORDS) lds_ref[lane + WAVE] = rv1;
```

After: 2565. Within noise of the previous version (-0.0%).
